# HBioquant/DiffBindFR

Hardware: AMD Instinct MI355X
Metric: poses_per_sec (higher is better)
Workload: dtype f32

## Files before the change

diffbindfr_amd/csrc/api.cpp:

```cpp
#include <cmath>
#include <cstdio>
#include <cstring>
#include <algorithm>
#include <atomic>
#include <map>

#include "common.h"

void launch_conv(const ConvArgs& a, hipStream_t st);
void launch_conv_layer(const ConvArgs* c4, hipStream_t st);
void launch_conv2(const Conv2Args& a, hipStream_t st);
void launch_conv2h(const Conv2Args& a, hipStream_t st);
void launch_convz(const ConvZArgs& a, hipStream_t st);
void launch_reduce_ln(const float* msg, const int* row_start, const int* row_cnt, int N, int D, const LNDesc& ln,
                      const float* old, int D_old, float* out, int ldo, int mode, hipStream_t st, const uint8_t* first = nullptr, unsigned long long sc_lanes = 0);
struct ReduceLayerArgs {
  const float* msg[4]; const int* row_start[4]; const int* row_cnt[4]; LNDesc ln[4];
  int NL, NA, D, D_old;
  const float* old_l; const float* old_a; float* out_l; float* out_a;
  const uint8_t* first[4]; unsigned long long sc_lanes[4];
};
static unsigned long long convz_sc_lanes(const ConvZ& z) {
  unsigned long long m = 0;
  for (int i = 0; i < z.n_io; ++i) m |= 0xfffull << (z.out_off[i] / 4);
  return m;
}
void launch_reduce_ln_layer(const ReduceLayerArgs& a, hipStream_t st);
enum SetKind { SET_LL = 0, SET_AA = 1, SET_AL = 2, SET_LA = 3, SET_TOR = 4, SET_SC = 5, N_SETS = 6 };
struct GraphArgs {
  dbfr_batch b;
  const int* lig_batch; const int* atm_batch; const uint8_t* is_cab; const int* n_cab; const float* tr_sigma;
  float lig_cut2, atom_cut2, cross_cut2;
  int lig_cap, atom_cap, dynamic_cross;
  EdgeSet set[N_SETS];
  int* err;
  int step, lds_nl, lds_na, n_chunk, lanes;
};
void dbfr_edge_form(const dbfr_batch& b, int* n_chunk, int* lanes);
void launch_edges(const GraphArgs& A, bool heads_only, hipStream_t st);
void launch_edge_log(const GraphArgs& A, int* log_row, int stride, hipStream_t st);
void launch_edge_ties(const GraphArgs& A, int* log_row, int stride, float tol, hipStream_t st);
void launch_graph_chunks(const GraphArgs& A, hipStream_t st);
void launch_flat_chunks(const int* tgt, const int* n_edges, int max_edges, int span, int n_span, int* cnt0, int cap, int* chunk_es, int* chunk_gl, hipStream_t st);
void launch_row_absmax(const float* lx, const int* lig_ptr, float* out_l, const float* ax, const int* atm_ptr, float* out_a, int ld, int D, int G, int n_rows_a, hipStream_t st);
void launch_batch_vectors(const dbfr_batch& b, int* lig_batch, int* atm_batch, uint8_t* is_cab, int* n_cab,
                          int* tor_batch, int* sc_batch, hipStream_t st);
void launch_time_embed(const float* t, int G, float emb_scale, float* temb, hipStream_t st);
enum MlpIn { IN_LIGNODE = 0, IN_LIGEDGE = 1, IN_TG = 2, IN_G = 3 };
struct MlpArgs {
  Mlp2 w; int mode; const int* n_rows_dev; int n_rows_max; const float* temb; const int* row_graph_tab; const int* tgt;
  const int* aux; const float* dist; const float* bond_feat; int nfeat; const float* lig_node; int nnode;
  const float* gs_offset; const float* gs_coeff; float* out;
};
void launch_mlp(const MlpArgs& a, hipStream_t st);
struct AtomEncArgs {
  const float* pocket_feat; const int* atm_batch; const float* temb; const float* emb[5]; int dims[5];
  const float* lin_t; int NA; float* out;
};
void launch_atom_encoder(const AtomEncArgs& a, hipStream_t st);
void launch_center_edges(const dbfr_batch& b, int* tgt, int* gth, float* dist, float* sh, int* row_start, int* row_cnt,
                         hipStream_t st);
struct TrRotArgs {
  const float* gp; const float* temb; const float* tr_sigma; const float* rot_norm; Mlp2 tr, rot; int G;
  int scale_by_sigma; float* tr_out; float* rot_out; int* err;
};
void launch_trrot(const TrRotArgs& a, hipStream_t st);
void launch_bond_attr(const float* x, int ldx, const int* b0, const int* b1, const int* bsel, int stride, int n,
                      float* out, hipStream_t st);
void launch_tor_final(const float* feat, const Mlp2& w, const float* norm2, int scale, int n, float* out, hipStream_t st);
struct SdeLigArgs {
  dbfr_batch b; const float* tr_score; const float* rot_score; const float* tor_score; const float* z_tr;
  const float* z_rot; const float* z_tor; float dt, tr_g2, tr_gsdt, rot_g2, rot_gsdt, tor_g2, tor_gsdt; float* traj;
  int* err;
};
void launch_sde_ligand(const SdeLigArgs& a, hipStream_t st);
void launch_sidechain(const dbfr_batch& b, const float* score, const float* z, float dt, float g2, float gsdt,
                      const int* a14_group, float* atom14_out, float* traj14, const int* err, hipStream_t st);
void launch_fill(float* p, float v, int n, hipStream_t st);
void launch_set_int(int* p, int v, hipStream_t st);
void launch_init_poses(const dbfr_batch& b, const dbfr_init_tape& z, const int* a14_group, float* atom14_out, hipStream_t st);
void launch_extract_templates(int n_res, const int* aatype, const float* pos14, float* transl, float* rots, float* frames,
                              float* rigid, float* angle, hipStream_t st);
void launch_select_pocket(int n_prot, int n_res_total, const int* res_ptr, int m, const float* pos, const float* mask, const int* ref_ptr,
                          const float* ref, float cut2, int max_neighbors, float* d2, unsigned char* out, hipStream_t st);
void launch_acc_flops(const int* n_edges, double flops_per_edge, double bytes_per_edge, double fused_bytes_per_edge, double* counter, hipStream_t st);
void launch_acc_executed(const int* n_edges, double flops_per_edge, double* counter, hipStream_t st);
struct AccBatch { const int* n[32]; double coef[32]; double* dst[32]; int count; };
void launch_acc_batch(const AccBatch& b, hipStream_t st);
static inline double fused_bytes(int D_in, int D_out) { return 4.0 * (48 + 9 + 3 + 48 + 48 + D_in + D_out); }

#define RT_TABLE static const
#include "residue_tables.inc"
#undef RT_TABLE

static thread_local std::string g_err;
void dbfr_set_error(const std::string& s) { g_err = s; }
// ... 270 lines not shown
      }
  }
  o->K = K; o->D_in = sp.D_in; o->D_out = sp.D_out; o->n_tiles = n_tiles; o->W = sp.W;
  for (int v = 0; v < 5; ++v) { o->wave_tile0[v] = wave_tile0[v]; o->wave_run0[v] = wave_run0[v]; }
  o->W1p = upload(m, w1p, &rc);
  o->b1 = upload(m, std::vector<float>(B1, B1 + K), &rc);
  o->W2p = upload(m, w2p, &rc);
  o->b2p = upload(m, b2p, &rc);
  o->runs = upload(m, runs, &rc);
  LNDesc& ln = o->ln;
  memset(&ln, 0, sizeof ln);
  ln.nblk = (int)sp.out.size();
  int off = 0;
  for (int i = 0; i < ln.nblk; ++i) {
    ln.mul[i] = sp.out[i].mul; ln.dim[i] = sp.out[i].dim(); ln.off[i] = off;
    ln.is0e[i] = sp.out[i].l == 0 && sp.out[i].p == 1;
    off += ln.mul[i] * ln.dim[i];
  }
  ln.mean_shift = upload(m, std::vector<float>(ms, ms + nirr), &rc);
  ln.weight = upload(m, std::vector<float>(aw, aw + nirr), &rc);
  ln.bias = upload(m, std::vector<float>(ab, ab + std::max(n0e, 0)), &rc);
  return rc;
}

#define CH_TILE_BYTES_HOST 9280
#define F16_ROW_DEPTH_OK 17
static int pack_f16_tiles(const float* frag, const float* bias16, int tile0, int nt, uint16_t* out, int* depth = nullptr, float* rinv = nullptr) {
  constexpr int KT = 9;
  const size_t tile_h = CH_TILE_BYTES_HOST / 2, tail_off = 8192 / 2, bias_off = 9216 / 2;
  auto h16 = [](float v) { const _Float16 h = (_Float16)v; uint16_t u; memcpy(&u, &h, 2); return u; };
  float mx = 0.f;
  for (size_t i = (size_t)tile0 * KT * 256; i < (size_t)(tile0 + nt) * KT * 256; ++i) mx = std::max(mx, fabsf(frag[i]));
  int e = 0;
  if (mx > 0.f) (void)frexpf(mx, &e);
  int k = mx > 0.f ? std::max(-120, std::min(120, 15 - e)) : 0;
  float bmx = 0.f;
  for (int i = 16 * tile0; i < 16 * (tile0 + nt); ++i) bmx = std::max(bmx, fabsf(bias16[i]));
  if (bmx > 0.f) { int eb = 0; (void)frexpf(bmx, &eb); k = std::min(k, 48 - eb); }
  const float sc = ldexpf(1.f, k);
  std::vector<int> rowd((size_t)nt * 16, 0);
  int dmax = 0;
  for (int t = tile0; t < tile0 + nt; ++t)
    for (int row = 0; row < 16; ++row) {
      float rm = 0.f;
      for (int s4 = 0; s4 < KT; ++s4)
        for (int gq = 0; gq < 4; ++gq)
          for (int q = 0; q < 4; ++q) rm = std::max(rm, fabsf(frag[(((size_t)t * KT + s4) * 64 + 16 * gq + row) * 4 + q]));
      if (rm <= 0.f) continue;
      int er = 0;
      (void)frexpf(rm, &er);
      int d = 15 - (er + k);
      if (rinv) {
        int up = std::max(d, 0);
        const float br = fabsf(bias16[16 * t + row]);
        if (br > 0.f) { int eb = 0; (void)frexpf(br, &eb); up = std::max(0, std::min(up, 48 - eb - k)); }
        up = std::min(up, 100);
        rowd[(size_t)(t - tile0) * 16 + row] = up;
        d -= up;
      }
      dmax = std::max(dmax, d);
    }
  if (depth) *depth = dmax;
  if (rinv)
    for (int i = 0; i < nt * 16; ++i) rinv[(size_t)tile0 * 16 + i] = ldexpf(1.f, -rowd[i]);
  for (int t = tile0; t < tile0 + nt; ++t) {
    float b[16];
    for (int i = 0; i < 16; ++i) b[i] = bias16[16 * t + i] * ldexpf(sc, rowd[(size_t)(t - tile0) * 16 + i]);
    memcpy(&out[t * tile_h + bias_off], b, 64);
    for (int s4 = 0; s4 < KT; ++s4)
      for (int lane = 0; lane < 64; ++lane)
        for (int q = 0; q < 4; ++q) {
          const float v = frag[(((size_t)t * KT + s4) * 64 + lane) * 4 + q] * ldexpf(sc, rowd[(size_t)(t - tile0) * 16 + (lane & 15)]);
          const _Float16 hi = (_Float16)v;
          const uint16_t pc[2] = {h16(v), h16(v - (float)hi)};
          for (int i = 0; i < 2; ++i) {
            if (s4 < 8) out[t * tile_h + ((size_t)(i * 4 + (s4 >> 1)) * 64 + lane) * 8 + 4 * (s4 & 1) + q] = pc[i];
            else out[t * tile_h + tail_off + (size_t)lane * 8 + 4 * i + q] = pc[i];
          }
        }
  }
  return k;
}

static int pack_conv2(dbfr_model* m, const TMap& tm, const std::string& name, int kind, const ConvW& base, ConvW2* o, bool vector_only = false) {
  ConvSpec sp = make_conv_spec(kind);
  const int K = sp.K;
  if (K != 144) return fail(DBFR_ERR_ARG, "k_conv2 layout is for the K=144 convs");
  int rc = 0;
  const float* W2 = need(tm, name + ".fc.lin.3.weight", (int64_t)sp.W * K, &rc);
  const float* B2 = need(tm, name + ".fc.lin.3.bias", sp.W, &rc);
  if (rc) return rc;
  const int KT = K / 16;
  struct Pair { int io, w; std::vector<const PathDesc*> paths; };
  std::vector<Pair> pairs;
  for (int io = 0; io < (int)sp.out.size(); ++io)
    for (int w = 0; w < sp.out[io].mul; ++w) {
      if (vector_only && sp.out[io].l == 0) continue;
      Pair pr{io, w, {}};
      for (auto& p : sp.paths) if (p.io == io) pr.paths.push_back(&p);
      std::stable_sort(pr.paths.begin(), pr.paths.end(),
                       [](const PathDesc* a, const PathDesc* b) { return a->type != b->type ? a->type < b->type : a->mul1 > b->mul1; });
      pairs.push_back(pr);
    }
  auto sig = [](const Pair& a) {
    std::string k;
    for (auto* p : a.paths) k += std::to_string(p->type) + ":" + std::to_string(p->mul1) + ":" + std::to_string(p->in_off) + ",";
    return k;
  };
  struct Group { std::vector<int> pair_idx; int tiles; int xph; };
  std::vector<Group> groups;
  {
    std::map<std::string, std::vector<int>> cls;
    std::vector<std::string> order;
    for (int i = 0; i < (int)pairs.size(); ++i) {
      std::string k = sig(pairs[i]);
      if (!cls.count(k)) order.push_back(k);
      cls[k].push_back(i);
    }
    for (auto& k : order) {
      auto& v = cls[k];
      for (size_t i = 0; i < v.size(); i += 4) {
        Group g;
        for (size_t j = i; j < i + 4; ++j) g.pair_idx.push_back(j < v.size() ? v[j] : -1);
        g.tiles = 0;
        bool hi = false, lo = false;
        for (auto* p : pairs[v[i]].paths) {
          if (p->mul1 % 4) return fail(DBFR_ERR_ARG, "input multiplicity not a multiple of 4 in " + name);
          g.tiles += p->mul1 / 4;
          if (p->in_off >= 120) hi = true;
          if (p->in_off < 48) lo = true;
        }
        if (hi && lo) return fail(DBFR_ERR_ARG, "channel group reads both scalar input blocks in " + name);
        g.xph = hi ? 1 : 0;
        groups.push_back(g);
      }
    }
  }
  std::stable_sort(groups.begin(), groups.end(), [](const Group& a, const Group& b) { return a.xph < b.xph; });
  std::vector<int> rows_orig; std::vector<float> rows_scale;
  std::vector<RunDesc> runs;
  std::vector<int> group_run0, group_tiles;
  for (const Group& G : groups) {
    group_run0.push_back((int)runs.size());
    group_tiles.push_back(G.tiles);
    const Pair& lead = pairs[G.pair_idx[0]];
    for (size_t pi = 0; pi < lead.paths.size(); ++pi) {
      const PathDesc* lp = lead.paths[pi];
      RunDesc rd;
      const uint32_t flags = (pi == 0 ? 1u : 0u) | (pi + 1 == lead.paths.size() ? 2u : 0u);
      const uint32_t tile0 = (uint32_t)rows_orig.size() / 16, nt = (uint32_t)lp->mul1 / 4, x_step = 4u * (2 * lp->l1 + 1);
      if (tile0 >= (1u << 20) || nt >= (1u << 12)) return fail(DBFR_ERR_ARG, "conv too large for the run descriptor");
      rd.tile0_n = tile0 | (nt << 20);
      rd.meta = (uint32_t)lp->type | (flags << 4) | ((uint32_t)lp->sh_off << 8) | (x_step << 12) | ((uint32_t)G.xph << 20);
      rd.x_off4 = rd.o_off4 = 0;
      for (int g = 0; g < 4; ++g) {
        const int pidx = G.pair_idx[g];
        const PathDesc* p = pidx >= 0 ? pairs[pidx].paths[pi] : lp;
        if (p->type != lp->type || p->sh_off != lp->sh_off || p->mul1 != lp->mul1 || p->in_off != lp->in_off)
          return fail(DBFR_ERR_ARG, "channel group with non-uniform paths in " + name);
        const int d_o = 2 * p->lo + 1;
        const uint32_t xo = p->in_off >= 120 ? p->in_off - 120 : p->in_off;
        const uint32_t oo = pidx >= 0 ? p->out_off + pairs[pidx].w * d_o : 255u;
        if (xo + 4 * (2 * p->l1 + 1) * (p->mul1 / 4) > 120 || (oo != 255u && (int)oo >= sp.D_out))
          return fail(DBFR_ERR_ARG, "irreps do not fit the k_conv2 row layout in " + name);
        rd.x_off4 |= xo << (8 * g);
        rd.o_off4 |= oo << (8 * g);
      }
      runs.push_back(rd);
      for (int u0 = 0; u0 < lp->mul1; u0 += 4)
        for (int g = 0; g < 4; ++g) {
          const int pidx = G.pair_idx[g];
          const PathDesc* p = pidx >= 0 ? pairs[pidx].paths[pi] : lp;
          for (int r = 0; r < 4; ++r) {
            rows_orig.push_back(pidx >= 0 ? p->w_off + (u0 + r) * p->mulo + pairs[pidx].w : -1);
            rows_scale.push_back(pidx >= 0 ? p->fold : 0.f);
          }
        }
    }
  }
  const int n_tiles = (int)rows_orig.size() / 16;
  std::vector<float> w2q((size_t)n_tiles * KT * 64 * 4), b2q((size_t)n_tiles * 16);
  for (int t = 0; t < n_tiles; ++t) {
    for (int i = 0; i < 16; ++i) { const int ro = rows_orig[16 * t + i]; b2q[16 * t + i] = ro >= 0 ? rows_scale[16 * t + i] * B2[ro] : 0.f; }
    for (int s4 = 0; s4 < KT; ++s4)
      for (int lane = 0; lane < 64; ++lane) {
        const int ro = rows_orig[16 * t + (lane & 15)];
        const float sc = rows_scale[16 * t + (lane & 15)];
        for (int q = 0; q < 4; ++q)
          w2q[(((size_t)t * KT + s4) * 64 + lane) * 4 + q] = ro >= 0 ? sc * W2[(size_t)ro * K + 16 * s4 + 4 * (lane >> 4) + q] : 0.f;
      }
  }
  memset(o, 0, sizeof *o);
  o->D_in = sp.D_in; o->D_out = sp.D_out; o->n_tiles = n_tiles; o->n_runs = (int)runs.size();
  o->W1p = base.W1p; o->b1 = base.b1;
  if (!vector_only) {
  o->W2q = upload(m, w2q, &rc);
  o->b2q = upload(m, b2q, &rc);
  }
  {
    const int rowscale = getenv("DBFR_F16_ROWSCALE") ? atoi(getenv("DBFR_F16_ROWSCALE")) : 1;
    std::vector<uint16_t> w2h((size_t)n_tiles * (CH_TILE_BYTES_HOST / 2) + 512, 0);
    std::vector<float> w2rinv((size_t)std::max(n_tiles, 1) * 16, 1.f);
    int depth_max = 0, depth_run = 0;
    for (int pass = 0; pass < 2; ++pass) {
      const bool rowf = pass == 1;
      if (rowf && !(rowscale == 2 || (rowscale == 1 && depth_max > F16_ROW_DEPTH_OK))) break;
      if (rowf) depth_run = depth_max;
      depth_max = 0;
      for (RunDesc& rd : runs) {
        const int tile0 = rd.tile0_n & 0xfffff, nt = rd.tile0_n >> 20;
        int depth = 0;
        const int k = pack_f16_tiles(w2q.data(), b2q.data(), tile0, nt, w2h.data(), &depth, rowf ? w2rinv.data() : nullptr);
        depth_max = std::max(depth_max, depth);
        rd.meta = (rd.meta & 0x00ffffffu) | ((uint32_t)(k & 0xff) << 24);
      }
      if (!rowf) depth_run = depth_max;
      else o->W2rinv = upload(m, w2rinv, &rc);
    }
    o->W2h = upload(m, w2h, &rc);
    const float* W1 = need(tm, name + ".fc.lin.0.weight", (int64_t)K * K, &rc);
    const float* B1 = need(tm, name + ".fc.lin.0.bias", K, &rc);
    if (rc) return rc;
    std::vector<float> w1q((size_t)KT * KT * 256);
    for (int mt = 0; mt < KT; ++mt)
      for (int s4 = 0; s4 < KT; ++s4)
        for (int lane = 0; lane < 64; ++lane)
          for (int q = 0; q < 4; ++q)
            w1q[(((size_t)mt * KT + s4) * 64 + lane) * 4 + q] = W1[(size_t)(16 * mt + (lane & 15)) * K + 16 * s4 + 4 * (lane >> 4) + q];
    std::vector<uint16_t> w1h((size_t)KT * (CH_TILE_BYTES_HOST / 2) + 512, 0);
    int depth1 = 0;
    o->k1 = pack_f16_tiles(w1q.data(), B1, 0, KT, w1h.data(), &depth1);
    depth_run = std::max(depth_run, depth1);
    if (rowscale == 2 || (rowscale == 1 && depth1 > F16_ROW_DEPTH_OK)) {
      std::vector<float> w1rinv((size_t)KT * 16, 1.f);
      o->k1 = pack_f16_tiles(w1q.data(), B1, 0, KT, w1h.data(), &depth1, w1rinv.data());
      o->W1rinv = upload(m, w1rinv, &rc);
    }
    o->W1h = upload(m, w1h, &rc);
    o->f16_depth = std::max(depth_max, depth1);
    o->f16_depth_run = depth_run;
  }
  o->runs = upload(m, runs, &rc);
  const int n_g = (int)groups.size();
  int total_tiles = 0;
  for (int t : group_tiles) total_tiles += t;
  for (int si = 0; si < 4; ++si) {
    const int S = 1 << si;
    int gi = 0, acc = 0;
    for (int p = 0; p < S; ++p) {
      o->part_run[si][p] = gi < n_g ? group_run0[gi] : (int)runs.size();
      const long target = (long)total_tiles * (p + 1) / S;
      while (gi < n_g && (acc + group_tiles[gi] / 2 < target || p == S - 1)) { acc += group_tiles[gi]; ++gi; }
    }
    for (int p = S; p <= 8; ++p) o->part_run[si][p] = (int)runs.size();
  }
  return rc;
}

static int pack_convz(dbfr_model* m, const TMap& tm, const std::string& name, int kind, const ConvW2& base, ConvZ* o) {
  ConvSpec sp = make_conv_spec(kind);
  const int K = sp.K;
  memset(o, 0, sizeof *o);
  if (K != 144) return fail(DBFR_ERR_ARG, "k_convz is for the K=144 convs");
  int rc = 0;
  const float* W2 = need(tm, name + ".fc.lin.3.weight", (int64_t)sp.W * K, &rc);
  const float* B2 = need(tm, name + ".fc.lin.3.bias", sp.W, &rc);
  if (rc) return rc;
  struct Col { const PathDesc* p; int u; };
  std::vector<std::vector<Col>> cols;
  std::vector<int> ios;
  for (int io = 0; io < (int)sp.out.size(); ++io) {
    if (sp.out[io].l != 0) continue;
    if (sp.out[io].mul != NS) return fail(DBFR_ERR_ARG, "scalar output irrep with a multiplicity other than 48 in " + name);
    std::vector<Col> c;
    for (int pass = 0; pass < 2; ++pass)
      for (auto& p : sp.paths) {
        if (p.io != io || p.l1 != pass) continue;
        if (p.l1 != p.l2 || p.lo != 0 || p.l1 > 1) return fail(DBFR_ERR_ARG, "unsupported scalar-output path in " + name);
        for (int u = 0; u < p.mul1; ++u) c.push_back({&p, u});
      }
    int n_scalar = 0;
    for (auto& q : c) n_scalar += q.p->l1 == 0;
    if (n_scalar % 16) return fail(DBFR_ERR_ARG, "scalar-input columns do not fill whole tiles in " + name);
    while (c.size() % 16) c.push_back({nullptr, 0});
    cols.push_back(c);
    ios.push_back(io);
  }
  if (ios.size() > 2) return fail(DBFR_ERR_ARG, "more than two scalar output irreps in " + name);
  o->n_io = (int)ios.size();
  int nct_total = 0;
  for (int i = 0; i < o->n_io; ++i) {
    o->nct[i] = (int)cols[i].size() / 16;
    for (auto& q : cols[i]) o->nc_valid[i] += q.p != nullptr;
    o->ct0[i] = nct_total;
    nct_total += o->nct[i];
    int off = 0;
    for (int j = 0; j < ios[i]; ++j) off += sp.out[j].mul * sp.out[j].dim();
    o->out_off[i] = off;
  }
  if (nct_total > CZ_MAXCT) return fail(DBFR_ERR_ARG, "too many c tiles in " + name);
  std::vector<uint32_t> cdesc((size_t)std::max(nct_total, 1) * 16, 0u);
  std::vector<float> rowinv((size_t)std::max(o->n_io, 1) * NS, 1.f);
  std::vector<uint16_t> w2z((size_t)nct_total * CZ_NKT * 8 * (CZ_TILE_BYTES / 2) + 512, 0);
  auto h16 = [](float v) { const _Float16 h = (_Float16)v; uint16_t u; memcpy(&u, &h, 2); return u; };
  for (int i = 0; i < o->n_io; ++i) {
    const auto& c = cols[i];
    for (size_t j = 0; j < c.size(); ++j)
      if (c[j].p) cdesc[(size_t)o->ct0[i] * 16 + j] = (uint32_t)(c[j].p->in_off + c[j].u * (2 * c[j].p->l1 + 1)) | ((uint32_t)c[j].p->l1 << 12) |
                                                      ((uint32_t)c[j].p->sh_off << 16) | 0x80000000u;
    auto wval = [&](int cc, int k, int w) -> float {
      if (cc >= (int)c.size() || !c[cc].p || k > K) return 0.f;
      const PathDesc* p = c[cc].p;
      const size_t row = (size_t)p->w_off + (size_t)c[cc].u * p->mulo + w;
      return p->fold * (k < K ? W2[row * K + k] : B2[row]);
    };
    for (int w = 0; w < NS; ++w) {
      float mx = 0.f;
      for (int cc = 0; cc < (int)c.size(); ++cc)
        for (int k = 0; k <= K; ++k) mx = std::max(mx, fabsf(wval(cc, k, w)));
      int s = 0;
      if (mx > 0.f) { int e = 0; (void)frexpf(mx, &e); s = std::max(-100, std::min(100, 15 - e)); }
// ... 85 lines not shown
  if (!m || (log_dev && (n_steps_cap <= 0 || n_graphs_cap <= 0))) return fail(DBFR_ERR_ARG, "dbfr_model_set_edge_log: bad argument");
  m->edge_log = log_dev; m->edge_log_steps = log_dev ? n_steps_cap : 0; m->edge_log_graphs = log_dev ? n_graphs_cap : 0;
  return DBFR_OK;
}

extern "C" int dbfr_model_set_gemm(dbfr_model* m, int32_t mode) {
  if (!m || mode < DBFR_GEMM_F32 || mode > DBFR_GEMM_REDUCE_FIRST || mode == 1 || mode == 2) return fail(DBFR_ERR_ARG, "dbfr_model_set_gemm: bad argument (modes 1 and 2, the three-bf16-piece kernels, were retired with ABI 5 / 4)");
  m->gemm_split = mode;
  return DBFR_OK;
}
extern "C" int dbfr_model_get_gemm(const dbfr_model* m) { return m ? m->gemm_split : DBFR_ERR_ARG; }

extern "C" int dbfr_abi_version(void) { return DBFR_ABI_VERSION; }
#ifndef DBFR_BUILD_ID
#define DBFR_BUILD_ID "unknown"
#endif
extern "C" const char* dbfr_build_id(void) { return DBFR_BUILD_ID; }
extern "C" const char* dbfr_last_error(void) { return g_err.c_str(); }

extern "C" int dbfr_wigner3j(int32_t l1, int32_t l2, int32_t l3, double* out) {
  if (!out || l1 < 0 || l2 < 0 || l3 < 0 || l1 > 4 || l2 > 4 || l3 > 4) return fail(DBFR_ERR_ARG, "bad l");
  std::vector<double> v;
  wigner3j_real(l1, l2, l3, v);
  memcpy(out, v.data(), v.size() * sizeof(double));
  return DBFR_OK;
}

extern "C" int dbfr_conv_paths(int32_t kind, int32_t* t10, int32_t max_paths, int32_t* weight_numel) {
  if (kind < 0 || kind > 5) return fail(DBFR_ERR_ARG, "bad conv kind");
  ConvSpec sp = make_conv_spec(kind);
  if (weight_numel) *weight_numel = sp.W;
  int n = (int)sp.paths.size();
  for (int i = 0; i < n && i < max_paths && t10; ++i) {
    const PathDesc& p = sp.paths[i];
    int32_t* r = t10 + 10 * i;
    r[0] = p.i1; r[1] = p.i2; r[2] = p.io; r[3] = p.l1; r[4] = p.l2; r[5] = p.lo; r[6] = p.mul1; r[7] = p.mulo; r[8] = p.w_off;
    memcpy(&r[9], &p.coeff, 4);
  }
  return n;
}

static int model_create_impl(const dbfr_model_cfg* cfg, const dbfr_tensor* tensors, int32_t n_tensors, dbfr_model** out);
static int f16_depth_ok() { static const int v = getenv("DBFR_F16_DEPTH") ? atoi(getenv("DBFR_F16_DEPTH")) : F16_ROW_DEPTH_OK; return v; }

extern "C" int dbfr_model_create(const dbfr_model_cfg* cfg, const dbfr_tensor* tensors, int32_t n_tensors,
                                 dbfr_model** out) {
  try {
    return model_create_impl(cfg, tensors, n_tensors, out);
  } catch (const std::exception& e) {
    return fail(DBFR_ERR_ARG, std::string("dbfr_model_create: ") + e.what());
  }
}

static int model_create_impl(const dbfr_model_cfg* cfg, const dbfr_tensor* tensors, int32_t n_tensors, dbfr_model** out) {
  if (!cfg || !tensors || !out) return fail(DBFR_ERR_ARG, "null argument");
  if (cfg->ns != NS || cfg->nv != NV || cfg->sh_lmax != 2 || cfg->distance_embed_dim != EMB ||
      cfg->sigma_embed_dim != EMB || cfg->num_conv_layers < 1 || cfg->num_conv_layers > 8)
    return fail(DBFR_ERR_ARG, "unsupported model configuration (need ns=48, nv=12, sh_lmax=2, 32-d embeddings)");
  if (cfg->lig_edge_features + 2 * EMB > 80 || cfg->lig_node_features + EMB > 80)
    return fail(DBFR_ERR_ARG, "ligand feature width too large");
  std::string serr;
  int rc = so3_selftest(serr);
  if (rc) return fail(rc, serr);
  TMap tm;
  for (int i = 0; i < n_tensors; ++i) tm[tensors[i].name] = &tensors[i];
  dbfr_model* m = new dbfr_model();
  m->cfg = *cfg;
  m->profile = 0; m->ev_used = 0; m->flops_dev = nullptr; m->fused_bytes_last = 0; m->executed_last = 0; m->useful_last = 0; m->form_bytes_last = 0; m->conv_ms_acc = 0; m->conv_launches_acc = 0;
  m->streams_ready = false;
  m->edge_log = nullptr; m->edge_log_steps = 0; m->edge_log_graphs = 0; m->layer_fallback = 0;
  m->tie_log = nullptr; m->tie_log_steps = 0; m->tie_log_graphs = 0; m->tie_tol = 0.f;
  m->use_conv2 = getenv("DBFR_CONV2") ? atoi(getenv("DBFR_CONV2")) : -1;
  m->gemm_split = gemm_from_env();
  if (m->gemm_split < 0) rc = fail(DBFR_ERR_ARG, std::string("DBFR_GEMM=") + getenv("DBFR_GEMM") + ": unknown or retired value (f32 | split_f16 | reduce_first)");
  m->conv2_layers = getenv("DBFR_CONV2_LAYERS") ? atoi(getenv("DBFR_CONV2_LAYERS")) : 0;
  m->conv_fuse = getenv("DBFR_CONV_FUSE") ? atoi(getenv("DBFR_CONV_FUSE")) : 1;
  const char* fam[4] = {"lig_conv_layers", "cross_al_conv_layers", "atom_conv_layers", "cross_la_conv_layers"};
  for (int l = 0; l < cfg->num_conv_layers && !rc; ++l)
    for (int f = 0; f < 4 && !rc; ++f)
    {
      rc = pack_conv(m, tm, std::string(fam[f]) + "." + std::to_string(l), std::min(l, 3), &m->layer[l][f]);
      if (!rc) rc = pack_conv2(m, tm, std::string(fam[f]) + "." + std::to_string(l), std::min(l, 3), m->layer[l][f], &m->layer2[l][f]);
      if (!rc && m->layer2[l][f].f16_depth > f16_depth_ok()) { m->layer_fallback |= 1u << l; m->fallback_convs += std::string(fam[f]) + "." + std::to_string(l) + ";"; }
      if (!rc && (m->layer2[l][f].W2rinv || m->layer2[l][f].W1rinv)) m->rowscaled_convs += std::string(fam[f]) + "." + std::to_string(l) + ":" + std::to_string(m->layer2[l][f].f16_depth_run) + ";";
      if (!rc) rc = pack_conv2(m, tm, std::string(fam[f]) + "." + std::to_string(l), std::min(l, 3), m->layer[l][f], &m->layer2v[l][f], true);
      if (!rc) rc = pack_convz(m, tm, std::string(fam[f]) + "." + std::to_string(l), std::min(l, 3), m->layer2[l][f], &m->layerz[l][f]);
    }
  if (!rc) rc = pack_conv(m, tm, "final_conv", 4, &m->final_conv);
  if (!rc) rc = pack_conv(m, tm, "tor_bond_conv", 5, &m->tor_conv);
  if (!rc) rc = pack_conv2(m, tm, "tor_bond_conv", 5, m->tor_conv, &m->tor_conv2);
  if (!rc && m->tor_conv2.f16_depth > f16_depth_ok()) { m->layer_fallback |= 1u << 31; m->fallback_convs += "tor_bond_conv;"; }
  if (!rc && (m->tor_conv2.W2rinv || m->tor_conv2.W1rinv)) m->rowscaled_convs += "tor_bond_conv:" + std::to_string(m->tor_conv2.f16_depth_run) + ";";
  if (!rc) rc = pack_convz(m, tm, "tor_bond_conv", 5, m->tor_conv2, &m->tor_convz);
  if (!rc && !cfg->no_sc_torsion) rc = pack_conv(m, tm, "sc_tor_bond_conv", 5, &m->sc_conv);
  if (!rc && !cfg->no_sc_torsion) rc = pack_conv2(m, tm, "sc_tor_bond_conv", 5, m->sc_conv, &m->sc_conv2);
  if (!rc && !cfg->no_sc_torsion && m->sc_conv2.f16_depth > f16_depth_ok()) { m->layer_fallback |= 1u << 31; m->fallback_convs += "sc_tor_bond_conv;"; }
  if (!rc && !cfg->no_sc_torsion && (m->sc_conv2.W2rinv || m->sc_conv2.W1rinv)) m->rowscaled_convs += "sc_tor_bond_conv:" + std::to_string(m->sc_conv2.f16_depth_run) + ";";
  if (!rc && !cfg->no_sc_torsion) rc = pack_convz(m, tm, "sc_tor_bond_conv", 5, m->sc_conv2, &m->sc_convz);
  if (!rc) rc = pack_mlp(m, tm, "lig_node_embedding", cfg->lig_node_features + EMB, NS, NS, true, &m->lig_node_emb);
  if (!rc) rc = pack_mlp(m, tm, "lig_edge_embedding", cfg->lig_edge_features + 2 * EMB, NS, NS, true, &m->lig_edge_emb);
  if (!rc) rc = pack_mlp(m, tm, "atom_edge_embedding", 2 * EMB, NS, NS, true, &m->atom_edge_emb);
  if (!rc) rc = pack_mlp(m, tm, "la_edge_embedding", 2 * EMB, NS, NS, true, &m->la_edge_emb);
  if (!rc) rc = pack_mlp(m, tm, "center_edge_embedding", 2 * EMB, NS, NS, true, &m->center_edge_emb);
  if (!rc) rc = pack_mlp(m, tm, "tor_edge_embedding", EMB, NS, NS, true, &m->tor_edge_emb);
  if (!rc) rc = pack_mlp(m, tm, "tr_final_layer", 1 + EMB, NS, 1, true, &m->tr_final);
  if (!rc) rc = pack_mlp(m, tm, "rot_final_layer", 1 + EMB, NS, 1, true, &m->rot_final);
  if (!rc) rc = pack_mlp(m, tm, "tor_final_layer", 2 * NS, NS, 1, false, &m->tor_final);
  if (!rc && !cfg->no_sc_torsion) {
    rc = pack_mlp(m, tm, "sc_edge_embedding", EMB, NS, NS, true, &m->sc_edge_emb);
    if (!rc) rc = pack_mlp(m, tm, "sc_tor_final_layer", 2 * NS, NS, 1, false, &m->sc_final);
  }
  const int dims[5] = {37, 22, 4, 21, 2};
  for (int i = 0; i < 5 && !rc; ++i) {
    const float* e = need(tm, "atom_node_embedding.atom_emb_list." + std::to_string(i) + ".weight", (int64_t)dims[i] * NS, &rc);
    if (!rc) { m->atom_emb[i] = upload(m, std::vector<float>(e, e + dims[i] * NS), &rc); m->atom_dims[i] = dims[i]; }
  }
  if (!rc) {
    const float* w = need(tm, "atom_node_embedding.scalar_lin.weight", (int64_t)NS * (NS + EMB), &rc);
    if (!rc) {
      std::vector<float> t((size_t)(NS + EMB) * NS);
      for (int o = 0; o < NS; ++o) for (int i = 0; i < NS + EMB; ++i) t[(size_t)i * NS + o] = w[(size_t)o * (NS + EMB) + i];
      m->atom_lin_t = upload(m, t, &rc);
    }
  }
  struct { const char* n; const float** off; const float** c; } gs[4] = {
      {"lig", &m->gs_lig_off, &m->gs_lig_c}, {"atom", &m->gs_atom_off, &m->gs_atom_c},
      {"cross", &m->gs_cross_off, &m->gs_cross_c}, {"center", &m->gs_center_off, &m->gs_center_c}};
  for (int i = 0; i < 4 && !rc; ++i) {
    const float* off = need(tm, std::string(gs[i].n) + "_distance_expansion.offset", EMB, &rc);
    const float* c = need(tm, std::string(gs[i].n) + "_distance_expansion.coeff", 1, &rc);
    if (!rc) { *gs[i].off = upload(m, std::vector<float>(off, off + EMB), &rc); *gs[i].c = upload(m, std::vector<float>(c, c + 1), &rc); }
  }
  if (!rc) m->a14_group = upload(m, std::vector<int>(kAtom14ToGroup, kAtom14ToGroup + 21 * 14), &rc);
  if (!rc) { m->flops_dev = upload(m, std::vector<double>(6, 0.0), &rc); }
  if (!rc) { m->queue = upload(m, std::vector<int>(4, 0), &rc); }
  if (rc) { dbfr_model_destroy(m); return rc; }
  *out = m;
  return DBFR_OK;
}

extern "C" void dbfr_model_destroy(dbfr_model* m) {
  if (!m) return;
  for (void* p : m->allocs) (void)hipFree(p);
  for (auto e : m->ev) (void)hipEventDestroy(e);
  if (m->streams_ready) {
    for (int i = 0; i < 3; ++i) { (void)hipStreamDestroy(m->side[i]); (void)hipEventDestroy(m->ev_join[i]); }
    (void)hipEventDestroy(m->ev_fork); (void)hipEventDestroy(m->ev_a); (void)hipEventDestroy(m->ev_b);
  }
  delete m;
}

struct WsEntry { std::string name; size_t offset, bytes; };
struct Bump {
  char* base; size_t off; size_t cap;
  std::vector<WsEntry>* log;
  template <typename T> T* take(size_t n, const char* name = nullptr) {
    off = (off + 255) & ~(size_t)255;
    T* p = base ? (T*)(base + off) : nullptr;
    if (log && name) log->push_back({name, off, n * sizeof(T)});
    off += n * sizeof(T);
    return p;
  }
};

struct Ws {
  int* err; int64_t* counters;
  int *lig_batch, *atm_batch, *n_cab, *tor_batch, *sc_batch; uint8_t* is_cab;
  float* temb;
  float *c_t, *c_tr_sigma, *c_rot_norm, *c_tor_n2, *c_sc_n2;
  float *s_tr, *s_rot, *s_tor, *s_sc;
  float *lig_x[2], *atom_x[2];
  EdgeSet set[N_SETS];
  int *c_tgt, *c_gth, *c_row_start, *c_row_cnt, *c_n; float *c_dist, *c_sh, *c_emb;
  float* msg[4]; int multi; int conv2; float* gp; float *tor_attr, *sc_attr, *tor_feat, *sc_feat;
  float *xmax_l, *xmax_a;
  int* n_edges6;
};

static void edge_set_take(Bump& b, EdgeSet& S, int cap, int n_targets, int G, int n_graphs, int* n_edges, const char* nm) {
  S.cap = cap; S.n_edges = n_edges;
  std::string p(nm);
  S.tgt = b.take<int>(cap, (p + ".tgt").c_str()); S.gth = b.take<int>(cap, (p + ".gth").c_str());
  S.aux = b.take<int>(cap, (p + ".aux").c_str());
  S.dist = b.take<float>(cap, (p + ".dist").c_str()); S.sh = b.take<float>((size_t)cap * SH_LD, (p + ".sh").c_str());
  S.emb = b.take<float>((size_t)cap * NS, (p + ".emb").c_str());
  S.row_start = b.take<int>(n_targets, (p + ".row_start").c_str()); S.row_cnt = b.take<int>(n_targets, (p + ".row_cnt").c_str());
  S.g_cnt = b.take<int>(G, (p + ".g_cnt").c_str()); S.g_base = b.take<int>(G, (p + ".g_base").c_str());
  S.chunk0 = b.take<int>(n_graphs + 1, (p + ".chunk0").c_str()); S.gedge0 = b.take<int>(n_graphs + 1, (p + ".gedge0").c_str());
  S.chunk_cap = cap > 0 ? cap / 32 + n_targets / CZ_MAXSEG + n_graphs + 8 : 0;
  S.chunk_es = b.take<int>(std::max(S.chunk_cap, 1), (p + ".chunk_es").c_str()); S.chunk_gl = b.take<int>(std::max(S.chunk_cap, 1), (p + ".chunk_gl").c_str());
  S.seg_first = b.take<uint8_t>(std::max(cap, 1), (p + ".seg_first").c_str());
}

static int plan(const dbfr_model* m, const dbfr_batch* B, const dbfr_limits* lim, char* base, size_t cap, Ws* w,
                size_t* need_bytes, std::vector<WsEntry>* log = nullptr) {
  dbfr_limits L = {24, 64};
  if (lim) { if (lim->aa_avg_neighbors > 0) L.aa_avg_neighbors = lim->aa_avg_neighbors; if (lim->cross_avg_neighbors > 0) L.cross_avg_neighbors = lim->cross_avg_neighbors; }
  Bump b{base, 0, cap, log};
  const int G = B->G, NL = B->NL, NA = B->NA;
  w->err = b.take<int>(16, "err"); w->counters = (int64_t*)b.take<int64_t>(8); w->n_edges6 = b.take<int>(8, "n_edges");
  w->lig_batch = b.take<int>(NL); w->atm_batch = b.take<int>(NA); w->is_cab = b.take<uint8_t>(NA, "is_cab");
  w->n_cab = b.take<int>(G); w->tor_batch = b.take<int>(B->NTOR + 1); w->sc_batch = b.take<int>(B->NSC + 1);
  w->temb = b.take<float>((size_t)G * EMB, "temb");
  w->c_t = b.take<float>(G); w->c_tr_sigma = b.take<float>(G); w->c_rot_norm = b.take<float>(G);
  w->c_tor_n2 = b.take<float>(B->NTOR + 1); w->c_sc_n2 = b.take<float>(B->NSC + 1);
  w->s_tr = b.take<float>(3 * G); w->s_rot = b.take<float>(3 * G); w->s_tor = b.take<float>(B->NTOR + 1); w->s_sc = b.take<float>(B->NSC + 1);
  for (int i = 0; i < 2; ++i) { w->lig_x[i] = b.take<float>((size_t)NL * MAXD, i ? "lig_x1" : "lig_x0"); w->atom_x[i] = b.take<float>((size_t)NA * MAXD, i ? "atom_x1" : "atom_x0"); }
  const int lig_cap = m->cfg.lig_max_neighbors;
  const long cap_ll = (long)NL * std::min(lig_cap + 1, std::max(B->max_nl - 1, 1)) + B->EB;
  const long cap_aa = (long)NA * std::min(L.aa_avg_neighbors, std::max(B->max_na - 1, 1));
  const long cap_x = (long)NL * std::min(B->max_na, 2 * B->max_nr + L.cross_avg_neighbors);
  const long cap_t = (long)B->NTOR * lig_cap, cap_s = m->cfg.no_sc_torsion ? 0 : (long)B->NSC * lig_cap;
  const long caps[N_SETS] = {cap_ll, cap_aa, cap_x, cap_x, cap_t, cap_s};
  const int ntg[N_SETS] = {NL, NA, NL, NA, B->NTOR, B->NSC};
  long maxcap = NL;
  for (int k = 0; k < N_SETS; ++k) {
    if (caps[k] > 0x7fffff00L) return fail(DBFR_ERR_ARG, "batch too large for int32 edge indices; split it");
    static const char* names[N_SETS] = {"ll", "aa", "al", "la", "tor", "sc"};
    edge_set_take(b, w->set[k], (int)caps[k], ntg[k] + 1, G * dbfr_edge_chunks(B->max_na, B->max_nl), G, w->n_edges6 ? w->n_edges6 + k : nullptr, names[k]);
    maxcap = std::max(maxcap, caps[k]);
  }
  w->c_tgt = b.take<int>(NL); w->c_gth = b.take<int>(NL); w->c_dist = b.take<float>(NL); w->c_sh = b.take<float>((size_t)NL * SH_LD, "center.sh");
  w->c_emb = b.take<float>((size_t)NL * NS, "center.emb"); w->c_row_start = b.take<int>(G); w->c_row_cnt = b.take<int>(G);
  w->c_n = w->n_edges6 ? w->n_edges6 + 6 : nullptr;
  static const long multi_edges = getenv("DBFR_MULTI_EDGES") ? atol(getenv("DBFR_MULTI_EDGES")) : 0;
  static const long conv2_edges = getenv("DBFR_CONV2_EDGES") ? atol(getenv("DBFR_CONV2_EDGES")) : 128 * 1024;
  w->multi = maxcap <= multi_edges;
  w->conv2 = m->gemm_split || m->use_conv2 > 0 || (m->use_conv2 < 0 && maxcap <= conv2_edges);
  if (w->conv2 || m->conv2_layers > 0 || (m->conv_fuse && !w->multi)) {
    const bool all_fused = w->conv2 || (m->conv_fuse && !w->multi && m->conv2_layers <= 0);
    const long mc[4] = {all_fused ? std::max({caps[SET_LL], (long)NL, cap_t, cap_s}) : maxcap, std::max(caps[SET_AL], cap_s), caps[SET_AA], caps[SET_LA]};
    for (int i = 0; i < 4; ++i) w->msg[i] = b.take<float>((size_t)std::max(mc[i], 1L) * MAXD, i == 0 ? "msg" : nullptr);
    if (w->conv2) w->multi = 0;
  } else
  for (int i = 0; i < 4; ++i) w->msg[i] = (i == 0 || w->multi) ? b.take<float>((size_t)maxcap * MAXD, i == 0 ? "msg" : nullptr) : nullptr;
  w->gp = b.take<float>((size_t)G * 12, "gp");
  w->xmax_l = b.take<float>(G, "xmax_l"); w->xmax_a = b.take<float>(G, "xmax_a");
  w->tor_attr = b.take<float>((size_t)(B->NTOR + 1) * NS, "tor_attr"); w->sc_attr = b.take<float>((size_t)(B->NSC + 1) * NS);
  w->tor_feat = b.take<float>((size_t)(B->NTOR + 1) * 2 * NS, "tor_feat"); w->sc_feat = b.take<float>((size_t)(B->NSC + 1) * 2 * NS);
  *need_bytes = b.off + 256;
  return DBFR_OK;
}

static int check_batch(const dbfr_model* m, const dbfr_batch* B) {
  if (!m || !B) return fail(DBFR_ERR_ARG, "null argument");
  if (B->G <= 0 || B->NL <= 0 || B->NA <= 0 || B->NR <= 0) return fail(DBFR_ERR_ARG, "empty batch");
  if (B->max_nl > 256) return fail(DBFR_ERR_ARG, "ligand with more than 256 heavy atoms is not supported");
  if (B->max_na > 8192) return fail(DBFR_ERR_ARG, "pocket with more than 8192 heavy atoms is not supported");
  if (B->max_nl <= 0 || B->max_na <= 0 || B->max_nr <= 0) return fail(DBFR_ERR_ARG, "max_nl/max_na/max_nr must be set");
  return DBFR_OK;
}

extern "C" int dbfr_workspace_bytes(const dbfr_model* m, const dbfr_batch* b, const dbfr_limits* lim, size_t* bytes) {
  int rc = check_batch(m, b);
  if (rc) return rc;
  if (!bytes) return fail(DBFR_ERR_ARG, "null argument");
  Ws w; memset(&w, 0, sizeof w);
  return plan(m, b, lim, nullptr, 0, &w, bytes);
}

static void prof_events(dbfr_model* m, hipEvent_t* e0, hipEvent_t* e1) {
  if (m->ev_used + 2 > m->ev.size()) {
    size_t old = m->ev.size();
    m->ev.resize(old + 512);
    for (size_t i = old; i < m->ev.size(); ++i) (void)hipEventCreate(&m->ev[i]);
  }
  *e0 = m->ev[m->ev_used++]; *e1 = m->ev[m->ev_used++];
}

static void conv_call(dbfr_model* m, const ConvW& cw, const int* n_edges, int max_edges, const int* tgt, const int* gth,
                      const float* emb, const float* sh, const float* tab1, int ld1, const int* idx1, const float* tab2,
                      int ld2, const int* idx2, const float* x, int ldx, float* msg, hipStream_t st) {
  ConvArgs a;
  a.n_edges = n_edges; a.max_edges = max_edges; a.tgt = tgt; a.gth = gth; a.emb = emb; a.sh = sh; a.sh_sign = 1.f;
  a.tab1 = tab1; a.ld1 = ld1; a.idx1 = idx1; a.tab2 = tab2; a.ld2 = ld2; a.idx2 = idx2; a.x = x; a.ldx = ldx;
  a.w = cw; a.msg = msg;
  hipEvent_t e0 = nullptr, e1 = nullptr;
  const bool prof = m->profile == 1 && cw.K == 144;
  const bool count = m->profile && cw.K == 144;
  if (prof) {
    prof_events(m, &e0, &e1);
    (void)hipEventRecord(e0, st);
  }
  launch_conv(a, st);
  if (prof) (void)hipEventRecord(e1, st);
  if (count) {
    launch_acc_flops(n_edges, 2.0 * cw.K * ((double)cw.K + cw.W), 4.0 * (cw.W + cw.D_in + 9) + 16.0, fused_bytes(cw.D_in, cw.D_out), m->flops_dev, st);
  }
}

static Conv2Desc conv2_desc(const ConvW2& cw, const int* n_edges, int max_edges, const int* gth, const float* emb, const float* sh,
                            const float* tab1, int ld1, const int* idx1, const float* tab2, int ld2, const int* idx2, const float* x,
                            int ldx, float* msg) {
  Conv2Desc d;
  d.n_edges = n_edges; d.max_edges = max_edges; d.gth = gth; d.emb = emb; d.sh = sh; d.tab1 = tab1; d.ld1 = ld1; d.idx1 = idx1;
  d.tab2 = tab2; d.ld2 = ld2; d.idx2 = idx2; d.x = x; d.ldx = ldx; d.w = cw; d.msg = msg;
  return d;
}

static ConvZDesc convz_desc(const Conv2Desc& d, const ConvZ& z, const int* tgt, int D_out, const int* chunk_es, const int* chunk_gl, const int* n_chunks, int max_chunks,
                            const float* xmax = nullptr) {
  ConvZDesc o;
  o.n_edges = d.n_edges; o.max_edges = d.max_edges; o.tgt = tgt; o.gth = d.gth; o.emb = d.emb; o.sh = d.sh;
  o.tab1 = d.tab1; o.ld1 = d.ld1; o.idx1 = d.idx1; o.tab2 = d.tab2; o.ld2 = d.ld2; o.idx2 = d.idx2; o.x = d.x; o.ldx = d.ldx;
  o.w = z; o.msg = d.msg; o.D_out = D_out; o.chunk_es = chunk_es; o.chunk_gl = chunk_gl; o.n_chunks = n_chunks; o.max_chunks = max_chunks; o.xmax = xmax;
  return o;
}

static void conv2_call(dbfr_model* m, const Conv2Desc* descs, const int* Ws, int n, hipStream_t st, bool f16_fallback = false, const ConvZDesc* z = nullptr) {
  Conv2Args a;
  memset(&a, 0, sizeof a);
  for (int i = 0; i < n; ++i) a.c[i] = descs[i];
  a.n_conv = n; a.queue = m->queue;
  hipEvent_t e0 = nullptr, e1 = nullptr;
  if (m->profile == 1) {
    prof_events(m, &e0, &e1);
    (void)hipEventRecord(e0, st);
  }
  static unsigned long long* trace_dev = nullptr;
  static const char* trace_file = getenv("DBFR_CONV2_TRACE");
  if (trace_file && !trace_dev) {
    if (hipMalloc(&trace_dev, 8 * C2_TRACE_CAP * sizeof(unsigned long long)) != hipSuccess) trace_dev = nullptr;
    else atexit([] {
      std::vector<unsigned long long> h(8 * C2_TRACE_CAP);
      if (hipDeviceSynchronize() == hipSuccess && hipMemcpy(h.data(), trace_dev, h.size() * 8, hipMemcpyDeviceToHost) == hipSuccess) {
        if (FILE* f = fopen(getenv("DBFR_CONV2_TRACE"), "wb")) { fwrite(h.data(), 8, h.size(), f); fclose(f); }
      }
    });
  }
  if (trace_dev) { (void)hipMemsetAsync(trace_dev, 0, 8 * C2_TRACE_CAP * sizeof(unsigned long long), st); a.trace = trace_dev; }
  if (z) {
    Conv2Args v = a;
    v.n_conv = 0;
    for (int i = 0; i < n; ++i)
      if (descs[i].w.n_tiles > 0) v.c[v.n_conv++] = descs[i];
    if (v.n_conv) launch_conv2h(v, st);
    ConvZArgs za;
    memset(&za, 0, sizeof za);
    for (int i = 0; i < n; ++i) za.c[i] = z[i];
    za.n_conv = n;
    za.dbg = nullptr;
    za.executed = m->profile ? m->flops_dev + 3 : nullptr;
    launch_convz(za, st);
  }
  else if (m->gemm_split >= DBFR_GEMM_SPLIT_F16 && !f16_fallback) launch_conv2h(a, st);
  else launch_conv2(a, st);
  if (m->profile == 1) (void)hipEventRecord(e1, st);
  if (m->profile) {
    AccBatch ab; ab.count = 0;
    auto acc = [&](const int* ne, double coef, double* dst) { if (ab.count < 32) { ab.n[ab.count] = ne; ab.coef[ab.count] = coef; ab.dst[ab.count] = dst; ++ab.count; } };
    for (int i = 0; i < n; ++i) {
      acc(descs[i].n_edges, 2.0 * 144 * (144.0 + Ws[i]), m->flops_dev);
      acc(descs[i].n_edges, 4.0 * (Ws[i] + descs[i].w.D_in + 9) + 16.0, m->flops_dev + 1);
      acc(descs[i].n_edges, fused_bytes(descs[i].w.D_in, descs[i].w.D_out), m->flops_dev + 2);
      const double rows = 16.0 * descs[i].w.n_tiles;
      const bool f16 = (m->gemm_split >= DBFR_GEMM_SPLIT_F16 && !f16_fallback) || z;
      const double ex = f16 ? 3.0 * 2.0 * 144 * (144.0 + rows) : 2.0 * 144 * (144.0 + rows);
      if (!z || descs[i].w.n_tiles > 0) acc(descs[i].n_edges, ex, m->flops_dev + 3);
      if (!z) acc(descs[i].n_edges, ex, m->flops_dev + 4);
      else if (descs[i].w.n_tiles > 0) acc(descs[i].n_edges, 3.0 * 2.0 * 144 * rows, m->flops_dev + 4);
      const int D_in = descs[i].w.D_in, D_out = descs[i].w.D_out;
      const double in_bytes = 4.0 * (48 + 9 + 3 + 48 + 48 + D_in);
      if (!z) acc(descs[i].n_edges, fused_bytes(D_in, D_out), m->flops_dev + 5);
      else acc(descs[i].n_edges, in_bytes + 1.0 + (descs[i].w.n_tiles > 0 ? in_bytes + 4.0 * (D_out - 48 * z[i].w.n_io) : 0.0), m->flops_dev + 5);
    }
    launch_acc_batch(ab, st);
  }
}

static int run_score(dbfr_model* m, const dbfr_batch* B, const dbfr_cond* c, const dbfr_scores* out, Ws& w,
                     hipStream_t st, int step = 0) {
  const dbfr_model_cfg& cfg = m->cfg;
  const int G = B->G, NL = B->NL, NA = B->NA;
  launch_time_embed(c->t, G, cfg.emb_scale, w.temb, st);
  GraphArgs ga;
  ga.b = *B; ga.lig_batch = w.lig_batch; ga.atm_batch = w.atm_batch; ga.is_cab = w.is_cab; ga.n_cab = w.n_cab;
  ga.tr_sigma = c->tr_sigma;
  ga.lig_cut2 = cfg.lig_cutoff * cfg.lig_cutoff; ga.atom_cut2 = cfg.atom_cutoff * cfg.atom_cutoff;
  ga.cross_cut2 = cfg.dynamic_max_cross ? 1.0f : cfg.cross_cutoff * cfg.cross_cutoff;
  ga.lig_cap = cfg.lig_max_neighbors; ga.atom_cap = cfg.atom_max_neighbors; ga.dynamic_cross = cfg.dynamic_max_cross;
  for (int k = 0; k < N_SETS; ++k) ga.set[k] = w.set[k];
  ga.err = w.err; ga.step = step; ga.lds_nl = ga.lds_na = 0;
  dbfr_edge_form(*B, &ga.n_chunk, &ga.lanes);
  launch_edges(ga, false, st);
  if (int lrc = take_launch_error()) return lrc;
  if (m->gemm_split == DBFR_GEMM_REDUCE_FIRST) launch_graph_chunks(ga, st);
  if (m->edge_log && step < m->edge_log_steps) launch_edge_log(ga, m->edge_log + (size_t)step * N_SETS * m->edge_log_graphs, m->edge_log_graphs, st);
  if (m->tie_log && step < m->tie_log_steps) launch_edge_ties(ga, m->tie_log + (size_t)step * N_SETS * m->tie_log_graphs, m->tie_log_graphs, m->tie_tol, st);
  {
    MlpArgs a; memset(&a, 0, sizeof a);
    a.w = m->lig_node_emb; a.mode = IN_LIGNODE; a.n_rows_max = NL; a.temb = w.temb; a.row_graph_tab = w.lig_batch;
    a.lig_node = B->lig_node; a.nnode = cfg.lig_node_features; a.out = w.lig_x[0];
    launch_mlp(a, st);
  }
  {
    AtomEncArgs a; a.pocket_feat = B->pocket_feat; a.atm_batch = w.atm_batch; a.temb = w.temb;
    for (int i = 0; i < 5; ++i) { a.emb[i] = m->atom_emb[i]; a.dims[i] = m->atom_dims[i]; }
    a.lin_t = m->atom_lin_t; a.NA = NA; a.out = w.atom_x[0];
    launch_atom_encoder(a, st);
  }
  auto edge_mlp = [&](const Mlp2& mw, int mode, const EdgeSet& S, const int* tab, const float* off, const float* co) {
    MlpArgs a; memset(&a, 0, sizeof a);
    a.w = mw; a.mode = mode; a.n_rows_dev = S.n_edges; a.n_rows_max = S.cap; a.temb = w.temb; a.row_graph_tab = tab;
    a.tgt = S.tgt; a.aux = S.aux; a.dist = S.dist; a.bond_feat = B->bond_feat; a.nfeat = cfg.lig_edge_features;
    a.gs_offset = off; a.gs_coeff = co; a.out = S.emb;
    launch_mlp(a, st);
  };
  edge_mlp(m->lig_edge_emb, IN_LIGEDGE, w.set[SET_LL], w.lig_batch, m->gs_lig_off, m->gs_lig_c);
  edge_mlp(m->atom_edge_emb, IN_TG, w.set[SET_AA], w.atm_batch, m->gs_atom_off, m->gs_atom_c);
  edge_mlp(m->la_edge_emb, IN_TG, w.set[SET_AL], w.lig_batch, m->gs_cross_off, m->gs_cross_c);
  edge_mlp(m->la_edge_emb, IN_TG, w.set[SET_LA], w.atm_batch, m->gs_cross_off, m->gs_cross_c);
  static const int dims[4] = {48, 84, 120, 168};
  int cur = 0;
  for (int l = 0; l < cfg.num_conv_layers; ++l) {
    const int Di = dims[std::min(l, 3)], Do = dims[std::min(l + 1, 3)];
    const float *lx = w.lig_x[cur], *ax = w.atom_x[cur];
    float *lnew = w.lig_x[cur ^ 1], *anew = w.atom_x[cur ^ 1];
    const EdgeSet &LL = w.set[SET_LL], &AA = w.set[SET_AA], &AL = w.set[SET_AL], &LA = w.set[SET_LA];
    if (w.conv2 || l < m->conv2_layers) {
      const bool rf = m->gemm_split == DBFR_GEMM_REDUCE_FIRST && !((m->layer_fallback >> l) & 1u);
      const ConvW2* L2 = rf ? m->layer2v[l] : m->layer2[l];
      const Conv2Desc ds[4] = {
          conv2_desc(L2[0], LL.n_edges, LL.cap, LL.gth, LL.emb, LL.sh, lx, Di, LL.tgt, lx, Di, LL.gth, lx, Di, w.msg[0]),
          conv2_desc(L2[1], AL.n_edges, AL.cap, AL.gth, AL.emb, AL.sh, lx, Di, AL.tgt, ax, Di, AL.gth, ax, Di, w.msg[1]),
          conv2_desc(L2[2], AA.n_edges, AA.cap, AA.gth, AA.emb, AA.sh, ax, Di, AA.tgt, ax, Di, AA.gth, ax, Di, w.msg[2]),
          conv2_desc(L2[3], LA.n_edges, LA.cap, LA.gth, LA.emb, LA.sh, ax, Di, LA.tgt, lx, Di, LA.gth, lx, Di, w.msg[3])};
      const int Ws[4] = {m->layer[l][0].W, m->layer[l][1].W, m->layer[l][2].W, m->layer[l][3].W};
      if (rf) {
        launch_row_absmax(lx, B->lig_ptr, w.xmax_l, ax, B->atm_ptr, w.xmax_a, Di, Di, G, NA, st);
      }
      auto zd = [&](int i, const EdgeSet& S, const float* xmax) { return convz_desc(ds[i], m->layerz[l][i], S.tgt, Do, S.chunk_es, S.chunk_gl, S.chunk0 + G, S.chunk_cap, xmax); };
      const ConvZDesc zs[4] = {zd(0, LL, w.xmax_l), zd(1, AL, w.xmax_a), zd(2, AA, w.xmax_a), zd(3, LA, w.xmax_l)};
      conv2_call(m, ds, Ws, 4, st, (m->layer_fallback >> l) & 1u, rf ? zs : nullptr);
      ReduceLayerArgs ra;
      const EdgeSet* es[4] = {&LL, &AL, &AA, &LA};
      for (int i = 0; i < 4; ++i) {
        ra.msg[i] = w.msg[i]; ra.row_start[i] = es[i]->row_start; ra.row_cnt[i] = es[i]->row_cnt; ra.ln[i] = m->layer[l][i].ln;
        ra.first[i] = rf ? es[i]->seg_first : nullptr; ra.sc_lanes[i] = rf ? convz_sc_lanes(m->layerz[l][i]) : 0;
      }
      ra.NL = NL; ra.NA = NA; ra.D = Do; ra.D_old = Di; ra.old_l = lx; ra.old_a = ax; ra.out_l = lnew; ra.out_a = anew;
      launch_reduce_ln_layer(ra, st);
    } else if (m->conv_fuse && !w.multi) {
      auto mk = [&](const ConvW& cw, const EdgeSet& S, const float* tab1, const int* idx1, const float* tab2, const int* idx2, const float* x, float* msg) {
        ConvArgs a;
        a.n_edges = S.n_edges; a.max_edges = S.cap; a.tgt = S.tgt; a.gth = S.gth; a.emb = S.emb; a.sh = S.sh; a.sh_sign = 1.f;
        a.tab1 = tab1; a.ld1 = Di; a.idx1 = idx1; a.tab2 = tab2; a.ld2 = Di; a.idx2 = idx2; a.x = x; a.ldx = Di; a.w = cw; a.msg = msg; a.trace = nullptr;
        return a;
      };
      const ConvArgs c4[4] = {mk(m->layer[l][0], LL, lx, LL.tgt, lx, LL.gth, lx, w.msg[0]), mk(m->layer[l][1], AL, lx, AL.tgt, ax, AL.gth, ax, w.msg[1]),
                              mk(m->layer[l][2], AA, ax, AA.tgt, ax, AA.gth, ax, w.msg[2]), mk(m->layer[l][3], LA, ax, LA.tgt, lx, LA.gth, lx, w.msg[3])};
      hipEvent_t e0 = nullptr, e1 = nullptr;
      if (m->profile == 1) {
        prof_events(m, &e0, &e1);
        (void)hipEventRecord(e0, st);
      }
      launch_conv_layer(c4, st);
      if (m->profile == 1) (void)hipEventRecord(e1, st);
      if (m->profile)
        for (int i = 0; i < 4; ++i)
          launch_acc_flops(c4[i].n_edges, 2.0 * 144 * (144.0 + m->layer[l][i].W), 4.0 * (m->layer[l][i].W + Di + 9) + 16.0, fused_bytes(Di, Do), m->flops_dev, st);
      ReduceLayerArgs ra;
      const EdgeSet* es[4] = {&LL, &AL, &AA, &LA};
      for (int i = 0; i < 4; ++i) { ra.msg[i] = w.msg[i]; ra.row_start[i] = es[i]->row_start; ra.row_cnt[i] = es[i]->row_cnt; ra.ln[i] = m->layer[l][i].ln; ra.first[i] = nullptr; ra.sc_lanes[i] = 0; }
      ra.NL = NL; ra.NA = NA; ra.D = Do; ra.D_old = Di; ra.old_l = lx; ra.old_a = ax; ra.out_l = lnew; ra.out_a = anew;
      launch_reduce_ln_layer(ra, st);
    } else if (!w.multi || m->profile == 1) {
      conv_call(m, m->layer[l][0], LL.n_edges, LL.cap, LL.tgt, LL.gth, LL.emb, LL.sh, lx, Di, LL.tgt, lx, Di, LL.gth, lx, Di, w.msg[0], st);
      launch_reduce_ln(w.msg[0], LL.row_start, LL.row_cnt, NL, Do, m->layer[l][0].ln, lx, Di, lnew, Do, 0, st);
      conv_call(m, m->layer[l][1], AL.n_edges, AL.cap, AL.tgt, AL.gth, AL.emb, AL.sh, lx, Di, AL.tgt, ax, Di, AL.gth, ax, Di, w.msg[0], st);
      launch_reduce_ln(w.msg[0], AL.row_start, AL.row_cnt, NL, Do, m->layer[l][1].ln, nullptr, 0, lnew, Do, 1, st);
      conv_call(m, m->layer[l][2], AA.n_edges, AA.cap, AA.tgt, AA.gth, AA.emb, AA.sh, ax, Di, AA.tgt, ax, Di, AA.gth, ax, Di, w.msg[0], st);
      launch_reduce_ln(w.msg[0], AA.row_start, AA.row_cnt, NA, Do, m->layer[l][2].ln, ax, Di, anew, Do, 0, st);
      conv_call(m, m->layer[l][3], LA.n_edges, LA.cap, LA.tgt, LA.gth, LA.emb, LA.sh, ax, Di, LA.tgt, lx, Di, LA.gth, lx, Di, w.msg[0], st);
      launch_reduce_ln(w.msg[0], LA.row_start, LA.row_cnt, NA, Do, m->layer[l][3].ln, nullptr, 0, anew, Do, 1, st);
    } else {
      hipStream_t s0 = m->side[0], s1 = m->side[1], s2 = m->side[2];
      HIPCHECK(hipEventRecord(m->ev_fork, st));
      for (int i = 0; i < 3; ++i) HIPCHECK(hipStreamWaitEvent(m->side[i], m->ev_fork, 0));
      conv_call(m, m->layer[l][0], LL.n_edges, LL.cap, LL.tgt, LL.gth, LL.emb, LL.sh, lx, Di, LL.tgt, lx, Di, LL.gth, lx, Di, w.msg[0], st);
      conv_call(m, m->layer[l][1], AL.n_edges, AL.cap, AL.tgt, AL.gth, AL.emb, AL.sh, lx, Di, AL.tgt, ax, Di, AL.gth, ax, Di, w.msg[1], s0);
      conv_call(m, m->layer[l][2], AA.n_edges, AA.cap, AA.tgt, AA.gth, AA.emb, AA.sh, ax, Di, AA.tgt, ax, Di, AA.gth, ax, Di, w.msg[2], s1);
      conv_call(m, m->layer[l][3], LA.n_edges, LA.cap, LA.tgt, LA.gth, LA.emb, LA.sh, ax, Di, LA.tgt, lx, Di, LA.gth, lx, Di, w.msg[3], s2);
      launch_reduce_ln(w.msg[0], LL.row_start, LL.row_cnt, NL, Do, m->layer[l][0].ln, lx, Di, lnew, Do, 0, st);
      HIPCHECK(hipEventRecord(m->ev_a, st));
      HIPCHECK(hipStreamWaitEvent(s0, m->ev_a, 0));
      launch_reduce_ln(w.msg[1], AL.row_start, AL.row_cnt, NL, Do, m->layer[l][1].ln, nullptr, 0, lnew, Do, 1, s0);
      launch_reduce_ln(w.msg[2], AA.row_start, AA.row_cnt, NA, Do, m->layer[l][2].ln, ax, Di, anew, Do, 0, s1);
      HIPCHECK(hipEventRecord(m->ev_b, s1));
      HIPCHECK(hipStreamWaitEvent(s2, m->ev_b, 0));
      launch_reduce_ln(w.msg[3], LA.row_start, LA.row_cnt, NA, Do, m->layer[l][3].ln, nullptr, 0, anew, Do, 1, s2);
      HIPCHECK(hipEventRecord(m->ev_join[0], s0));
      HIPCHECK(hipEventRecord(m->ev_join[2], s2));
      HIPCHECK(hipStreamWaitEvent(st, m->ev_join[0], 0));
      HIPCHECK(hipStreamWaitEvent(st, m->ev_join[2], 0));
    }
    cur ^= 1;
  }
  const int D = dims[std::min(cfg.num_conv_layers, 3)];
  if (D != MAXD) return fail(DBFR_ERR_ARG, "heads need num_conv_layers >= 3");
  const float *lx = w.lig_x[cur], *ax = w.atom_x[cur];
  const bool fork_heads = w.multi && m->profile != 1 && !w.conv2;
  hipStream_t s_tor = fork_heads ? m->side[0] : st, s_sc = fork_heads ? m->side[1] : st;
  float* msg_tor = fork_heads ? w.msg[1] : w.msg[0];
  float* msg_sc = fork_heads ? w.msg[2] : w.msg[0];
  if (fork_heads) {
    HIPCHECK(hipEventRecord(m->ev_fork, st));
    HIPCHECK(hipStreamWaitEvent(s_tor, m->ev_fork, 0));
    HIPCHECK(hipStreamWaitEvent(s_sc, m->ev_fork, 0));
  }
  launch_center_edges(*B, w.c_tgt, w.c_gth, w.c_dist, w.c_sh, w.c_row_start, w.c_row_cnt, st);
  {
    MlpArgs a; memset(&a, 0, sizeof a);
    a.w = m->center_edge_emb; a.mode = IN_TG; a.n_rows_max = NL; a.temb = w.temb; a.row_graph_tab = w.lig_batch;
    a.dist = w.c_dist; a.gs_offset = m->gs_center_off; a.gs_coeff = m->gs_center_c; a.out = w.c_emb;
    launch_mlp(a, st);
  }
  conv_call(m, m->final_conv, w.n_edges6 + 7, NL, w.c_tgt, w.c_gth, w.c_emb, w.c_sh, lx, D, w.c_gth, nullptr, 0, w.c_gth, lx, D, w.msg[0], st);
  launch_reduce_ln(w.msg[0], w.c_row_start, w.c_row_cnt, G, 12, m->final_conv.ln, nullptr, 0, w.gp, 12, 2, st);
  {
    TrRotArgs a; a.gp = w.gp; a.temb = w.temb; a.tr_sigma = c->tr_sigma; a.rot_norm = c->rot_score_norm;
    a.tr = m->tr_final; a.rot = m->rot_final; a.G = G; a.scale_by_sigma = cfg.scale_by_sigma; a.tr_out = out->tr;
    a.rot_out = out->rot; a.err = w.err;
    launch_trrot(a, st);
  }
  if (w.conv2) {
    const EdgeSet& T = w.set[SET_TOR];
    const EdgeSet& S = w.set[SET_SC];
    const bool do_t = B->NTOR > 0, do_s = !cfg.no_sc_torsion && B->NSC > 0;
    const bool rf = m->gemm_split == DBFR_GEMM_REDUCE_FIRST && !((m->layer_fallback >> 31) & 1u);
    Conv2Desc ds[2]; ConvZDesc zs[2]; int Ws[2]; int nd = 0;
    if (rf) {
      launch_row_absmax(lx, B->lig_ptr, w.xmax_l, ax, B->atm_ptr, w.xmax_a, D, D, G, NA, st);
    }
    if (do_t) {
      launch_bond_attr(lx, D, B->bond_src, B->bond_dst, B->tor_bond, 0, B->NTOR, w.tor_attr, st);
      MlpArgs a; memset(&a, 0, sizeof a);
      a.w = m->tor_edge_emb; a.mode = IN_G; a.n_rows_dev = T.n_edges; a.n_rows_max = T.cap; a.dist = T.dist;
      a.gs_offset = m->gs_lig_off; a.gs_coeff = m->gs_lig_c; a.out = T.emb;
      launch_mlp(a, st);
      ds[nd] = conv2_desc(m->tor_conv2, T.n_edges, T.cap, T.gth, T.emb, T.sh, lx, D, T.gth, w.tor_attr, NS, T.tgt, lx, D, w.msg[0]);
      if (rf) { ds[nd].w.n_tiles = 0; zs[nd] = convz_desc(ds[nd], m->tor_convz, T.tgt, 2 * NS, T.chunk_es, T.chunk_gl, T.chunk0 + G, T.chunk_cap, w.xmax_l); }
      Ws[nd++] = m->tor_conv.W;
    }
    if (do_s) {
      launch_bond_attr(ax, D, B->sc_bond, nullptr, nullptr, 2, B->NSC, w.sc_attr, st);
      MlpArgs a; memset(&a, 0, sizeof a);
      a.w = m->sc_edge_emb; a.mode = IN_G; a.n_rows_dev = S.n_edges; a.n_rows_max = S.cap; a.dist = S.dist;
      a.gs_offset = m->gs_atom_off; a.gs_coeff = m->gs_atom_c; a.out = S.emb;
      launch_mlp(a, st);
      ds[nd] = conv2_desc(m->sc_conv2, S.n_edges, S.cap, S.gth, S.emb, S.sh, ax, D, S.gth, w.sc_attr, NS, S.tgt, ax, D, w.msg[1]);
      if (rf) { ds[nd].w.n_tiles = 0; zs[nd] = convz_desc(ds[nd], m->sc_convz, S.tgt, 2 * NS, S.chunk_es, S.chunk_gl, S.chunk0 + G, S.chunk_cap, w.xmax_a); }
      Ws[nd++] = m->sc_conv.W;
    }
    if (nd) conv2_call(m, ds, Ws, nd, st, (m->layer_fallback >> 31) & 1u, rf ? zs : nullptr);
    if (do_t) {
      launch_reduce_ln(w.msg[0], T.row_start, T.row_cnt, B->NTOR, 2 * NS, m->tor_conv.ln, nullptr, 0, w.tor_feat, 2 * NS, 2, st, rf ? T.seg_first : nullptr, rf ? convz_sc_lanes(m->tor_convz) : 0);
      launch_tor_final(w.tor_feat, m->tor_final, c->tor_score_norm2, cfg.scale_by_sigma, B->NTOR, out->tor, st);
    }
    if (do_s) {
      launch_reduce_ln(w.msg[1], S.row_start, S.row_cnt, B->NSC, 2 * NS, m->sc_conv.ln, nullptr, 0, w.sc_feat, 2 * NS, 2, st, rf ? S.seg_first : nullptr, rf ? convz_sc_lanes(m->sc_convz) : 0);
      launch_tor_final(w.sc_feat, m->sc_final, c->sc_tor_score_norm2, cfg.scale_by_sigma, B->NSC, out->sc_tor, st);
    }
    return DBFR_OK;
  }
  if (B->NTOR > 0) {
    const EdgeSet& T = w.set[SET_TOR];
    launch_bond_attr(lx, D, B->bond_src, B->bond_dst, B->tor_bond, 0, B->NTOR, w.tor_attr, s_tor);
    {
      MlpArgs a; memset(&a, 0, sizeof a);
      a.w = m->tor_edge_emb; a.mode = IN_G; a.n_rows_dev = T.n_edges; a.n_rows_max = T.cap; a.dist = T.dist;
      a.gs_offset = m->gs_lig_off; a.gs_coeff = m->gs_lig_c; a.out = T.emb;
      launch_mlp(a, s_tor);
    }
    conv_call(m, m->tor_conv, T.n_edges, T.cap, T.tgt, T.gth, T.emb, T.sh, lx, D, T.gth, w.tor_attr, NS, T.tgt, lx, D, msg_tor, s_tor);
    launch_reduce_ln(msg_tor, T.row_start, T.row_cnt, B->NTOR, 2 * NS, m->tor_conv.ln, nullptr, 0, w.tor_feat, 2 * NS, 2, s_tor);
    launch_tor_final(w.tor_feat, m->tor_final, c->tor_score_norm2, cfg.scale_by_sigma, B->NTOR, out->tor, s_tor);
  }
  if (!cfg.no_sc_torsion && B->NSC > 0) {
    const EdgeSet& S = w.set[SET_SC];
    launch_bond_attr(ax, D, B->sc_bond, nullptr, nullptr, 2, B->NSC, w.sc_attr, s_sc);
    {
      MlpArgs a; memset(&a, 0, sizeof a);
      a.w = m->sc_edge_emb; a.mode = IN_G; a.n_rows_dev = S.n_edges; a.n_rows_max = S.cap; a.dist = S.dist;
      a.gs_offset = m->gs_atom_off; a.gs_coeff = m->gs_atom_c; a.out = S.emb;
      launch_mlp(a, s_sc);
    }
    conv_call(m, m->sc_conv, S.n_edges, S.cap, S.tgt, S.gth, S.emb, S.sh, ax, D, S.gth, w.sc_attr, NS, S.tgt, ax, D, msg_sc, s_sc);
    launch_reduce_ln(msg_sc, S.row_start, S.row_cnt, B->NSC, 2 * NS, m->sc_conv.ln, nullptr, 0, w.sc_feat, 2 * NS, 2, s_sc);
    launch_tor_final(w.sc_feat, m->sc_final, c->sc_tor_score_norm2, cfg.scale_by_sigma, B->NSC, out->sc_tor, s_sc);
  }
  if (fork_heads) {
    HIPCHECK(hipEventRecord(m->ev_join[0], s_tor));
    HIPCHECK(hipEventRecord(m->ev_join[1], s_sc));
    HIPCHECK(hipStreamWaitEvent(st, m->ev_join[0], 0));
    HIPCHECK(hipStreamWaitEvent(st, m->ev_join[1], 0));
  }
  return DBFR_OK;
}

static int begin(dbfr_model* m, const dbfr_batch* B, void* workspace, size_t wbytes, const dbfr_limits* lim, Ws* w,
                 hipStream_t st) {
  g_launch_err = false;
  int rc = check_batch(m, B);
  if (rc) return rc;
  rc = check_logs(m, B->G);
  if (rc) return rc;
  if (!workspace) return fail(DBFR_ERR_ARG, "null workspace");
  size_t needb = 0;
  memset(w, 0, sizeof *w);
  rc = plan(m, B, lim, (char*)workspace, wbytes, w, &needb);
  if (rc) return rc;
  if (needb > wbytes) return fail(DBFR_ERR_ARG, "workspace too small: need " + std::to_string(needb) + " bytes");
  if (w->multi && !m->streams_ready) {
    for (int i = 0; i < 3; ++i) {
      HIPCHECK(hipStreamCreateWithFlags(&m->side[i], hipStreamNonBlocking));
      HIPCHECK(hipEventCreateWithFlags(&m->ev_join[i], hipEventDisableTiming));
    }
    HIPCHECK(hipEventCreateWithFlags(&m->ev_fork, hipEventDisableTiming));
    HIPCHECK(hipEventCreateWithFlags(&m->ev_a, hipEventDisableTiming));
    HIPCHECK(hipEventCreateWithFlags(&m->ev_b, hipEventDisableTiming));
    m->streams_ready = true;
  }
  HIPCHECK(hipMemsetAsync(workspace, 0, 1024, st));
  if (w->conv2 || m->gemm_split || m->conv2_layers > 0) HIPCHECK(hipMemsetAsync(m->queue, 0, 16, st));
  launch_set_int(w->n_edges6 + 7, B->NL, st);
  launch_batch_vectors(*B, w->lig_batch, w->atm_batch, w->is_cab, w->n_cab, w->tor_batch, w->sc_batch, st);
  return DBFR_OK;
}

extern "C" int dbfr_score(dbfr_model* m, const dbfr_batch* b, const dbfr_cond* cond, const dbfr_scores* out,
                          void* workspace, size_t workspace_bytes, const dbfr_limits* lim, void* hip_stream) {
  if (!cond || !out) return fail(DBFR_ERR_ARG, "null argument");
  hipStream_t st = (hipStream_t)hip_stream;
// ... 138 lines not shown
    float ms = 0;
    if (hipEventElapsedTime(&ms, m->ev[i], m->ev[i + 1]) == hipSuccess) { m->conv_ms_acc += ms; m->conv_launches_acc++; }
  }
  m->ev_used = 0;
  double fl[6] = {0, 0, 0, 0, 0, 0};
  HIPCHECK(hipMemcpy(fl, m->flops_dev, sizeof fl, hipMemcpyDeviceToHost));
  m->fused_bytes_last = fl[2];
  m->executed_last = fl[3];
  m->useful_last = fl[4];
  m->form_bytes_last = fl[5];
  if (conv_ms) *conv_ms = m->conv_ms_acc;
  if (conv_launches) *conv_launches = m->conv_launches_acc;
  if (conv_flops) *conv_flops = fl[0];
  if (ref_form_bytes) *ref_form_bytes = fl[1];
  if (reset) { m->conv_ms_acc = 0; m->conv_launches_acc = 0; HIPCHECK(hipMemset(m->flops_dev, 0, 6 * sizeof(double))); }
  return DBFR_OK;
}

extern "C" int dbfr_profile_executed_flops(const dbfr_model* m, double* executed_flops) {
  if (!m || !executed_flops) return fail(DBFR_ERR_ARG, "null argument");
  *executed_flops = m->executed_last;
  return DBFR_OK;
}

extern "C" int dbfr_profile_useful_flops(const dbfr_model* m, double* useful_flops, double* form_bytes) {
  if (!m || (!useful_flops && !form_bytes)) return fail(DBFR_ERR_ARG, "null argument");
  if (useful_flops) *useful_flops = m->useful_last;
  if (form_bytes) *form_bytes = m->form_bytes_last;
  return DBFR_OK;
}

extern "C" int dbfr_profile_fused_bytes(const dbfr_model* m, double* fused_form_bytes) {
  if (!m || !fused_form_bytes) return fail(DBFR_ERR_ARG, "null argument");
  *fused_form_bytes = m->fused_bytes_last;
  return DBFR_OK;
}

extern "C" int dbfr_workspace_layout(const dbfr_model* m, const dbfr_batch* b, const dbfr_limits* lim, char* names,
                                     size_t names_cap, size_t* offsets, size_t* bytes, int32_t max_entries) {
  int rc = check_batch(m, b);
  if (rc) return rc;
  std::vector<WsEntry> log;
  Ws w; memset(&w, 0, sizeof w);
  size_t nb = 0;
  rc = plan(m, b, lim, nullptr, 0, &w, &nb, &log);
  if (rc) return rc;
  size_t pos = 0;
  int n = 0;
  for (auto& e : log) {
    if (n >= max_entries || pos + e.name.size() + 2 > names_cap) break;
    memcpy(names + pos, e.name.c_str(), e.name.size());
    pos += e.name.size();
    names[pos++] = ';';
    offsets[n] = e.offset; bytes[n] = e.bytes;
    ++n;
  }
  names[pos] = 0;
  return n;
}

static const ConvW* pick_conv(const dbfr_model* m, int layer, int family) {
  if (layer >= 0 && layer < m->cfg.num_conv_layers && family >= 0 && family < 4) return &m->layer[layer][family];
  if (layer == -1) return &m->final_conv;
  if (layer == -2) return &m->tor_conv;
  if (layer == -3 && !m->cfg.no_sc_torsion) return &m->sc_conv;
  return nullptr;
}

static int test_conv_impl(dbfr_model* m, bool conv2, int32_t layer, int32_t family, int32_t n_edges, const int32_t* n_edges_dev,
                          const int32_t* tgt, const int32_t* gth, const float* emb, const float* sh, const float* tab1, int32_t ld1,
                          const int32_t* idx1, const float* tab2, int32_t ld2, const int32_t* idx2, const float* x, int32_t ldx,
                          float* msg, void* hip_stream) {
  if (!m) return fail(DBFR_ERR_ARG, "null model");
  g_launch_err = false;
  const ConvW* cw = pick_conv(m, layer, family);
  if (!cw) return fail(DBFR_ERR_ARG, "no such conv");
  if (conv2) {
    if (cw->K != 144) return fail(DBFR_ERR_ARG, "k_conv2 serves the K=144 convs");
    const ConvW2* cw2 = layer >= 0 ? &m->layer2[layer][family] : layer == -2 ? &m->tor_conv2 : &m->sc_conv2;
    const bool deep = cw2->f16_depth > f16_depth_ok();
    const bool rf = m->gemm_split == DBFR_GEMM_REDUCE_FIRST && !deep;
    Conv2Desc d = conv2_desc(rf && layer >= 0 ? m->layer2v[layer][family] : *cw2, n_edges_dev, n_edges, gth, emb, sh, tab1, ld1, idx1, tab2, ld2, idx2, x, ldx, msg);
    if (rf && layer < 0) d.w.n_tiles = 0;
    static int* scratch_dev[16] = {nullptr}; static size_t scratch_dev_ints[16] = {0};
    int dev_id = 0;
    HIPCHECK(hipGetDevice(&dev_id));
    if (dev_id < 0 || dev_id >= 16) return fail(DBFR_ERR_ARG, "test hook: device index beyond 15");
    int*& scratch = scratch_dev[dev_id]; size_t& scratch_ints = scratch_dev_ints[dev_id];
    const int span = 2048, n_span = std::max((n_edges + span - 1) / span, 1), ccap = n_edges / 32 + n_edges / CZ_MAXSEG + n_span + 8;
    if (rf) {
      const size_t need = (size_t)n_span + 1 + 2 * (size_t)ccap;
      if (need > scratch_ints) {
        if (scratch) HIPCHECK(hipFree(scratch));
        scratch = nullptr; scratch_ints = 0;
        HIPCHECK(hipMalloc(&scratch, need * sizeof(int)));
        scratch_ints = need;
      }
      launch_flat_chunks(tgt, n_edges_dev, n_edges, span, n_span, scratch, ccap, scratch + n_span + 1, scratch + n_span + 1 + ccap, (hipStream_t)hip_stream);
    }
    const ConvZDesc z = convz_desc(d, layer >= 0 ? m->layerz[layer][family] : layer == -2 ? m->tor_convz : m->sc_convz, tgt, cw->D_out,
                                   scratch ? scratch + n_span + 1 : nullptr, scratch ? scratch + n_span + 1 + ccap : nullptr, scratch ? scratch + n_span : nullptr, ccap);
    const int W = cw->W;
    if (rf) HIPCHECK(hipMemsetAsync(msg, 0, (size_t)n_edges * cw->D_out * sizeof(float), (hipStream_t)hip_stream));
    conv2_call(m, &d, &W, 1, (hipStream_t)hip_stream, deep, rf ? &z : nullptr);
  } else {
    conv_call(m, *cw, n_edges_dev, n_edges, tgt, gth, emb, sh, tab1, ld1, idx1, tab2, ld2, idx2, x, ldx, msg, (hipStream_t)hip_stream);
  }
  HIPCHECK(hipGetLastError());
  return take_launch_error();
}

extern "C" int dbfr_test_sde_step(const dbfr_model* m, const dbfr_batch* b, const dbfr_step* step, const dbfr_scores* scores,
                                  const dbfr_noise* z, float* atom14_out, int32_t* err_word_out, void* hip_stream) {
  int rc = check_batch(m, b);
  if (rc) return rc;
  if (!step || !scores || !z || !err_word_out) return fail(DBFR_ERR_ARG, "dbfr_test_sde_step: null argument");
  if (!scores->tr || !scores->rot || !z->z_tr || !z->z_rot || (b->NTOR > 0 && (!scores->tor || !z->z_tor)) ||
      (!m->cfg.no_sc_torsion && b->NSC > 0 && (!scores->sc_tor || !z->z_sc)))
    return fail(DBFR_ERR_ARG, "dbfr_test_sde_step: null score or noise array");
  hipStream_t st = (hipStream_t)hip_stream;
  HIPCHECK(hipMemsetAsync(err_word_out, 0, sizeof(int32_t), st));
  pose_update(m, b, *step, *scores, z->z_tr, z->z_rot, z->z_tor, z->z_sc, nullptr, atom14_out, nullptr, err_word_out, st);
  HIPCHECK(hipGetLastError());
  return DBFR_OK;
}

extern "C" int dbfr_test_chunk_table(const int32_t* tgt, const int32_t* n_edges_dev, int32_t max_edges, int32_t span, int32_t* scratch, int32_t cap,
                                     int32_t* chunk_es, int32_t* chunk_gl, void* hip_stream) {
  if (!tgt || !n_edges_dev || !scratch || !chunk_es || !chunk_gl || span <= 0 || max_edges < 0 || cap <= 0) return fail(DBFR_ERR_ARG, "dbfr_test_chunk_table: bad argument");
  g_launch_err = false;
  const int n_span = std::max((max_edges + span - 1) / span, 1);
  launch_flat_chunks(tgt, n_edges_dev, max_edges, span, n_span, scratch, cap, chunk_es, chunk_gl, (hipStream_t)hip_stream);
  HIPCHECK(hipGetLastError());
  return take_launch_error();
}

extern "C" int dbfr_test_conv(dbfr_model* m, int32_t layer, int32_t family, int32_t n_edges, const int32_t* n_edges_dev,
                              const int32_t* tgt, const int32_t* gth, const float* emb, const float* sh,
                              const float* tab1, int32_t ld1, const int32_t* idx1, const float* tab2, int32_t ld2,
                              const int32_t* idx2, const float* x, int32_t ldx, float* msg, void* hip_stream) {
  return test_conv_impl(m, false, layer, family, n_edges, n_edges_dev, tgt, gth, emb, sh, tab1, ld1, idx1, tab2, ld2, idx2, x, ldx,
                        msg, hip_stream);
}

extern "C" int dbfr_test_conv2(dbfr_model* m, int32_t layer, int32_t family, int32_t n_edges, const int32_t* n_edges_dev,
                               const int32_t* tgt, const int32_t* gth, const float* emb, const float* sh,
                               const float* tab1, int32_t ld1, const int32_t* idx1, const float* tab2, int32_t ld2,
                               const int32_t* idx2, const float* x, int32_t ldx, float* msg, void* hip_stream) {
  return test_conv_impl(m, true, layer, family, n_edges, n_edges_dev, tgt, gth, emb, sh, tab1, ld1, idx1, tab2, ld2, idx2, x, ldx,
                        msg, hip_stream);
}

extern "C" int dbfr_test_reduce_ln2(dbfr_model* m, int32_t layer, int32_t family, const float* msg, const int32_t* row_start, const int32_t* row_cnt,
                                    int32_t n_nodes, const float* old, int32_t d_old, float* out, int32_t mode, const uint8_t* seg_first, void* hip_stream) {
  if (!m) return fail(DBFR_ERR_ARG, "null model");
  const ConvW* cw = pick_conv(m, layer, family);
  if (!cw) return fail(DBFR_ERR_ARG, "no such conv");
  unsigned long long lanes = 0;
  if (seg_first) {
    if (layer == -1 || cw->K != 144) return fail(DBFR_ERR_ARG, "dbfr_test_reduce_ln2: seg_first with a conv that has no reduce-first form");
    lanes = convz_sc_lanes(layer >= 0 ? m->layerz[layer][family] : layer == -2 ? m->tor_convz : m->sc_convz);
  }
  launch_reduce_ln(msg, row_start, row_cnt, n_nodes, cw->D_out, cw->ln, old, d_old, out, cw->D_out, mode, (hipStream_t)hip_stream, seg_first, lanes);
  HIPCHECK(hipGetLastError());
  return DBFR_OK;
}
// ... 13 lines not shown
```

diffbindfr_amd/csrc/common.h:

```cpp
#pragma once
#include <hip/hip_runtime.h>
#include <stdint.h>
#include <string.h>
#include <string>
#include <vector>

#include "../../include/dbfr.h"

#define NS 48
#define NV 12
#define SH_LD 9
#define EMB 32
#define MAXD 168
#define EDGE_CHUNK 64
int dbfr_edge_chunks(int max_na, int max_nl);

enum PathType { PT_SS = 0, PT_SV = 1, PT_VS = 2, PT_VVS = 3, PT_VVV = 4, PT_VTV = 5 };

struct Irr { int mul, l, p; int dim() const { return 2 * l + 1; } };

struct PathDesc {
  int i1, i2, io, l1, l2, lo, mul1, mulo, w_off;
  float coeff;
  int type;
  int in_off, sh_off, out_off;
  float fold;
};

struct ConvSpec {
  std::vector<Irr> in, sh, out;
  std::vector<PathDesc> paths;
  int K;
  int W;
  int D_in, D_out;
};

ConvSpec make_conv_spec(int kind);
void wigner3j_real(int l1, int l2, int l3, std::vector<double>& out);
int so3_selftest(std::string& err);

struct LNDesc {
  int nblk;
  int mul[4], dim[4], off[4], is0e[4];
  const float* mean_shift;
  const float* weight;
  const float* bias;
};

struct RunDesc {
  uint32_t tile0_n;
  uint32_t meta;
  uint32_t x_off4;
  uint32_t o_off4;
};

struct ConvW {
  int K, D_in, D_out, n_tiles, W;
  int wave_tile0[5];
  const float* W1p;
  const float* b1;
  const float* W2p;
  const float* b2p;
  const RunDesc* runs;
  int wave_run0[5];
  LNDesc ln;
};

struct ConvW2 {
  int D_in, D_out, n_tiles, n_runs;
  const float* W1p;
  const float* b1;
  const float* W2q;
  const float* b2q;
  const void* W1h;
  int k1;
  int f16_depth;
  int f16_depth_run;
  const float* W2rinv;
  const float* W1rinv;
  const void* W2h;
  const RunDesc* runs;
  int part_run[4][9];
};

struct Conv2Desc {
  const int* n_edges; int max_edges;
  const int* gth;
  const float* emb;
  const float* sh;
  const float* tab1; int ld1; const int* idx1;
  const float* tab2; int ld2; const int* idx2;
  const float* x; int ldx;
  ConvW2 w;
  float* msg;
};

struct Conv2Args {
  Conv2Desc c[4];
  int n_conv;
  int* queue;
  int run_barrier, no_split;
  int skew;
  unsigned long long* trace;
};
#define C2_TRACE_CAP 4096

#define CZ_NKT 10
#define CZ_MAXCT 12
#define CZ_MAXSEG 4
#define CZ_TILE_BYTES 6144
struct ConvZ {
  int n_io;
  int nct[2];
  int ct0[2];
  int out_off[2];
  int nc_valid[2];
  const uint32_t* cdesc;
  const void* W2z;
  const float* rowinv;
  const void* W1h; int k1;
  const float* W1rinv;
};
struct ConvZDesc {
  const int* n_edges; int max_edges;
  const int* tgt;
  const int* gth;
  const float* emb; const float* sh;
  const float* tab1; int ld1; const int* idx1;
  const float* tab2; int ld2; const int* idx2;
  const float* x; int ldx;
  ConvZ w;
  float* msg; int D_out;
  const int* chunk_es;
  const int* chunk_gl;
  const int* n_chunks;
  int max_chunks;
  const float* xmax;
};
struct ConvZArgs { ConvZDesc c[4]; int n_conv; float* dbg; double* executed; int dbg_sel; };

static inline uint16_t dbfr_bf16_rne(float x) {
  uint32_t u;
  memcpy(&u, &x, 4);
  u += 0x7fffu + ((u >> 16) & 1u);
  return (uint16_t)(u >> 16);
}
static inline float dbfr_bf16_to_f32(uint16_t b) {
  const uint32_t u = (uint32_t)b << 16;
  float f;
  memcpy(&f, &u, 4);
  return f;
}

struct Mlp2 {
  int in, hid, out;
  const float* w0t;
  const float* b0;
  const float* w1t;
  const float* b1;
};

struct EdgeSet {
  int cap;
  int* n_edges;
  int* tgt;
  int* gth;
  int* aux;
  float* dist;
  float* sh;
  float* emb;
  int* row_start;
  int* row_cnt;
  int* g_cnt;
  int* g_base;
  int* chunk0;
  int* gedge0;
  int* chunk_es;
  int* chunk_gl;
// ... 33 lines not shown
```

diffbindfr_amd/csrc/conv2h.hip:

```cpp
#include <cstdio>
#include <cstdlib>
#include <type_traits>

#include "common.h"

typedef float f32x4 __attribute__((ext_vector_type(4)));
typedef float f32x2 __attribute__((ext_vector_type(2)));
typedef _Float16 f16x8 __attribute__((ext_vector_type(8)));
typedef _Float16 f16x4 __attribute__((ext_vector_type(4)));
typedef _Float16 f16x2 __attribute__((ext_vector_type(2)));
typedef unsigned u32x4 __attribute__((ext_vector_type(4)));
typedef unsigned u32x2 __attribute__((ext_vector_type(2)));

#define CH_TILE_BYTES 9280
#define CH_TAIL_OFF 8192
#define CH_BIAS_OFF 9216
#define CH_RING_BYTES 10240

__device__ __forceinline__ void split2x2(float x0, float x1, unsigned& hi, unsigned& lo) {
  const f16x2 h = __builtin_convertvector((f32x2){x0, x1}, f16x2);
  const f16x2 l = __builtin_convertvector((f32x2){x0 - (float)h[0], x1 - (float)h[1]}, f16x2);
  hi = __builtin_bit_cast(unsigned, h);
  lo = __builtin_bit_cast(unsigned, l);
}

__device__ __forceinline__ void scale4(f32x4& o, const f32x4& v, float s) { o[0] = v[0] * s; o[1] = v[1] * s; o[2] = v[2] * s; o[3] = v[3] * s; }
__device__ __forceinline__ void sum4(f32x4& o, const f32x4& a, const f32x4& b) { o[0] = a[0] + b[0]; o[1] = a[1] + b[1]; o[2] = a[2] + b[2]; o[3] = a[3] + b[3]; }

#define C2_XLD 124
#define C2_WAVE_FLOATS (32 * C2_XLD + 32 * 10 + 32 * 8 + 32)

template <int NW, int ABL = 0>
__global__ __launch_bounds__(64 * NW, 2) void k_conv2h(Conv2Args a) {
  constexpr int K = 144, KT = 9;
  constexpr bool ROWF = (ABL & 1024) != 0;
  constexpr int EPB = 32 * NW;
  extern __shared__ __attribute__((aligned(16))) float lds[];
  const int tid = threadIdx.x, lane = tid & 63, wave = tid >> 6;
  const int n = lane & 15, g = lane >> 4;
  if (wave >= NW / 2) __builtin_amdgcn_s_setprio(1);
  const char* ring = reinterpret_cast<const char*>(lds);
  float* xs = lds + CH_RING_BYTES / 4 + wave * C2_WAVE_FLOATS;
  float* shs = xs + 32 * C2_XLD;
  float* ms = shs + 32 * 10;
  int* s_gth = reinterpret_cast<int*>(ms + 32 * 8);

  if (a.trace && blockIdx.x == 0 && tid == 0) { a.trace[0] = __builtin_readcyclecounter(); a.trace[1] = __builtin_amdgcn_s_memrealtime(); }
  int nb0 = 0, nb1 = 0, nb2 = 0, nb3 = 0;
  {
    auto blocks = [&](int c) { return c < a.n_conv ? (min(*a.c[c].n_edges, a.c[c].max_edges) + EPB - 1) / EPB : 0; };
    nb0 = blocks(0); nb1 = blocks(1); nb2 = blocks(2); nb3 = blocks(3);
  }
  const int N = nb0 + nb1 + nb2 + nb3;
  const int n_wg = gridDim.x;
  const int full = (N / n_wg) * n_wg, rem = N - full;
  int si = 0;
  if (rem > 0 && !a.no_split) {
    int best = 0x7fffffff;
#pragma unroll
    for (int c = 0; c < 4; ++c) {
      const int cost = (((rem << c) + n_wg - 1) / n_wg) * ((128 >> c) + 6);
      if (cost < best) { best = cost; si = c; }
    }
  }
  const int total = full + (rem << si);

  for (int it = 0;; ++it) {
    asm volatile("s_waitcnt vmcnt(0) lgkmcnt(0)" ::: "memory");
    __syncthreads();
    const int u = (int)blockIdx.x + it * n_wg;
    if (u >= total) break;
    int blk, part = 0, psi = 0;
    if (u < full) blk = u;
    else { const int v = u - full; blk = full + (v >> si); part = v & ((1 << si) - 1); psi = si; }
    int c = 0;
    if (blk >= nb0) { blk -= nb0; c = 1; if (blk >= nb1) { blk -= nb1; c = 2; if (blk >= nb2) { blk -= nb2; c = 3; } } }
    const Conv2Desc& d = a.c[c];
    const int E = min(*d.n_edges, d.max_edges);
    const int e0 = blk * EPB + 32 * wave;
    const int D_in = d.w.D_in, D_out = d.w.D_out;
    const int vW = lane * 16, vB = g * 16;
    const int wv = __builtin_amdgcn_readfirstlane(wave);
    const int r_begin = d.w.part_run[psi][part], r_end = d.w.part_run[psi][part + 1];
    int t_last = 0, t_first = 0;
    if (r_begin < r_end) {
      const RunDesc rl = d.w.runs[r_end - 1];
      t_last = (rl.tile0_n & 0xfffff) + (rl.tile0_n >> 20) - 1;
      t_first = d.w.runs[r_begin].tile0_n & 0xfffff;
    }
    const __amdgpu_buffer_rsrc_t rW = __builtin_amdgcn_make_buffer_rsrc((void*)d.w.W2h, 0, d.w.n_tiles * CH_TILE_BYTES, 0x00020000);
    const int shA = wv & 7, shB = wv % 6;
    const int offA = shA < 6 ? ((shA / 3) * 4 + shA % 3) * 1024 : CH_BIAS_OFF;
    const int offB = shB < 4 ? ((shB >> 1) * 4 + 3) * 1024 + (shB & 1) * 512 : CH_TAIL_OFF + (shB - 4) * 512;
    const int vA = (shA < 6 || lane < 4) ? lane * 16 : 0x40000000;
    char* ringw = const_cast<char*>(ring);
    u32x4 stgA = {0u, 0u, 0u, 0u};
    u32x2 stgB = {0u, 0u};
    auto fetchA = [&](int tile) { if (!(ABL & (4 | 16))) stgA = __builtin_bit_cast(u32x4, __builtin_amdgcn_raw_buffer_load_b128(rW, vA, ((ABL & 512) ? (tile & 7) : tile) * CH_TILE_BYTES + offA, 0)); };
    auto fetchB = [&](int tile) { if (!(ABL & (4 | 16))) stgB = __builtin_bit_cast(u32x2, __builtin_amdgcn_raw_buffer_load_b64(rW, lane * 8, ((ABL & 512) ? (tile & 7) : tile) * CH_TILE_BYTES + offB, 0)); };
    auto putA = [&] { if (!(ABL & (4 | 8))) *reinterpret_cast<u32x4*>(ringw + offA + vW) = stgA; };
    auto putB = [&] { if (!(ABL & (4 | 8))) *reinterpret_cast<u32x2*>(ringw + offB + lane * 8) = stgB; };
    using I0 = std::integral_constant<int, 0>; using I1 = std::integral_constant<int, 1>;
    using I2 = std::integral_constant<int, 2>; using I3 = std::integral_constant<int, 3>;
    if (r_begin < r_end) {
      fetchA(t_first); fetchB(t_first);
    }

    int ev[2], gthv[2];
    const float* r0[2]; const float* r1[2]; const float* r2[2];
#pragma unroll
    for (int b = 0; b < 2; ++b) {
      const int e = e0 + 16 * b + n;
      ev[b] = min(e, E - 1);
      gthv[b] = d.gth[ev[b]];
      r0[b] = d.emb + (size_t)ev[b] * NS;
      r1[b] = d.tab1 + (size_t)d.idx1[ev[b]] * d.ld1;
      r2[b] = d.tab2 + (size_t)d.idx2[ev[b]] * d.ld2;
    }
    if (g == 0) { s_gth[n] = gthv[0]; s_gth[16 + n] = gthv[1]; }
    if (lane < 32) {
      const int e = min(e0 + lane, E - 1);
      const float* sp = d.sh + (size_t)e * SH_LD;
      float s[9];
#pragma unroll
      for (int k = 0; k < 9; ++k) { s[k] = sp[k]; shs[lane * 10 + k] = s[k]; }
      const float r3 = 1.7320508075688772f;
      float* m = ms + lane * 8;
      m[0] = -s[6] - r3 * s[8]; m[1] = r3 * s[5]; m[2] = r3 * s[4]; m[3] = 2.f * s[6]; m[4] = r3 * s[7]; m[5] = -s[6] + r3 * s[8];
    }
    u32x4 Bh[2][2][4];
    u32x4 Btc[2];
    float se[2], ue[2];
    {
      const __amdgpu_buffer_rsrc_t rW1 = __builtin_amdgcn_make_buffer_rsrc((void*)d.w.W1h, 0, KT * CH_TILE_BYTES, 0x00020000);
      u32x4 Ah[2][2][4];
      u32x4 Atc[2];
      float sa[2];
      int ja[2];
#pragma unroll
      for (int b = 0; b < 2; ++b) {
        f32x4 Ba[KT];
        float amx = 0.f;
#pragma unroll
        for (int s4 = 0; s4 < KT; ++s4) {
          const float* src = s4 < 3 ? r0[b] : s4 < 6 ? r1[b] : r2[b];
          Ba[s4] = *reinterpret_cast<const f32x4*>(src + 16 * (s4 % 3) + 4 * g);
#pragma unroll
          for (int q = 0; q < 4; ++q) amx = fmaxf(amx, fabsf(Ba[s4][q]));
        }
        amx = fmaxf(amx, __shfl_xor(amx, 16));
        amx = fmaxf(amx, __shfl_xor(amx, 32));
        ja[b] = max(-14, __builtin_amdgcn_frexp_expf(amx));
        sa[b] = __builtin_amdgcn_ldexpf(1.f, 15 - ja[b]);
#pragma unroll
        for (int s4 = 0; s4 < KT; ++s4) {
          unsigned hi0, lo0, hi1, lo1;
          split2x2(Ba[s4][0] * sa[b], Ba[s4][1] * sa[b], hi0, lo0);
          split2x2(Ba[s4][2] * sa[b], Ba[s4][3] * sa[b], hi1, lo1);
          if (s4 < 8) {
            Ah[b][0][s4 >> 1][2 * (s4 & 1)] = hi0; Ah[b][0][s4 >> 1][2 * (s4 & 1) + 1] = hi1;
            Ah[b][1][s4 >> 1][2 * (s4 & 1)] = lo0; Ah[b][1][s4 >> 1][2 * (s4 & 1) + 1] = lo1;
          } else {
            Atc[b] = (u32x4){lo0, lo1, hi0, hi1};
          }
        }
      }
      constexpr int NST = KT * 4;
      u32x4 F[3][2];
      u32x4 Ft;
      f32x4 bb;
      auto ld_step = [&](int i, u32x4 (&f)[2]) {
#pragma unroll
        for (int p = 0; p < 2; ++p) f[p] = __builtin_bit_cast(u32x4, __builtin_amdgcn_raw_buffer_load_b128(rW1, vW, (i >> 2) * CH_TILE_BYTES + (p * 4 + (i & 3)) * 1024, 0));
      };
      auto ld_tail = [&](int m) {
        Ft = __builtin_bit_cast(u32x4, __builtin_amdgcn_raw_buffer_load_b128(rW1, vW, m * CH_TILE_BYTES + CH_TAIL_OFF, 0));
        bb = __builtin_bit_cast(f32x4, __builtin_amdgcn_raw_buffer_load_b128(rW1, vB, m * CH_TILE_BYTES + CH_BIAS_OFF, 0));
      };
      ld_step(0, F[0]); ld_step(1, F[1]); ld_tail(0);
      float H[2][KT][4];
      float mx[2] = {0.f, 0.f};
      const f32x4 zero = {0.f, 0.f, 0.f, 0.f};
#define AHB(b, p, s) __builtin_bit_cast(f16x8, Ah[b][p][s])
#define FW(i, p) __builtin_bit_cast(f16x8, F[(i) % 3][p])
#pragma unroll
      for (int m = 0; m < KT; ++m) {
        f32x4 aS[2], aB[2];
        scale4(aS[0], bb, sa[0]); scale4(aS[1], bb, sa[1]);
        aB[0] = zero; aB[1] = zero;
#pragma unroll
        for (int s = 0; s < 4; ++s) {
          const int i = m * 4 + s;
          aS[0] = __builtin_amdgcn_mfma_f32_16x16x32_f16(FW(i, 0), AHB(0, 1, s), aS[0], 0, 0, 0);
          aS[1] = __builtin_amdgcn_mfma_f32_16x16x32_f16(FW(i, 0), AHB(1, 1, s), aS[1], 0, 0, 0);
          aS[0] = __builtin_amdgcn_mfma_f32_16x16x32_f16(FW(i, 1), AHB(0, 0, s), aS[0], 0, 0, 0);
          aS[1] = __builtin_amdgcn_mfma_f32_16x16x32_f16(FW(i, 1), AHB(1, 0, s), aS[1], 0, 0, 0);
          aB[0] = __builtin_amdgcn_mfma_f32_16x16x32_f16(FW(i, 0), AHB(0, 0, s), aB[0], 0, 0, 0);
          aB[1] = __builtin_amdgcn_mfma_f32_16x16x32_f16(FW(i, 0), AHB(1, 0, s), aB[1], 0, 0, 0);
          __builtin_amdgcn_sched_barrier(0);
          if (i + 2 < NST) ld_step(i + 2, F[(i + 2) % 3]);
        }
        {
          const f16x8 fw = __builtin_bit_cast(f16x8, Ft);
          const f16x4 fh = __builtin_bit_cast(f16x4, (u32x2){Ft[0], Ft[1]});
          aS[0] = __builtin_amdgcn_mfma_f32_16x16x32_f16(fw, __builtin_bit_cast(f16x8, Atc[0]), aS[0], 0, 0, 0);
          aS[1] = __builtin_amdgcn_mfma_f32_16x16x32_f16(fw, __builtin_bit_cast(f16x8, Atc[1]), aS[1], 0, 0, 0);
          aB[0] = __builtin_amdgcn_mfma_f32_16x16x16f16(fh, __builtin_bit_cast(f16x4, (u32x2){Atc[0][2], Atc[0][3]}), aB[0], 0, 0, 0);
          aB[1] = __builtin_amdgcn_mfma_f32_16x16x16f16(fh, __builtin_bit_cast(f16x4, (u32x2){Atc[1][2], Atc[1][3]}), aB[1], 0, 0, 0);
          __builtin_amdgcn_sched_barrier(0);
          if (m + 1 < KT) ld_tail(m + 1);
        }
        f32x4 rv = {1.f, 1.f, 1.f, 1.f};
        if constexpr (ROWF) if (d.w.W1rinv) rv = *reinterpret_cast<const f32x4*>(d.w.W1rinv + 16 * m + 4 * g);
#pragma unroll
        for (int b = 0; b < 2; ++b)
#pragma unroll
          for (int r = 0; r < 4; ++r) { H[b][m][r] = fmaxf(aS[b][r] + aB[b][r], 0.f); if constexpr (ROWF) H[b][m][r] *= rv[r]; mx[b] = fmaxf(mx[b], H[b][m][r]); }
      }
#undef AHB
#undef FW
      const int k1 = d.w.k1;
#pragma unroll
      for (int b = 0; b < 2; ++b) {
        float m2 = fmaxf(mx[b], __shfl_xor(mx[b], 16));
        m2 = fmaxf(m2, __shfl_xor(m2, 32));
        const int j = __builtin_amdgcn_frexp_expf(m2);
        const int tot = max(-120, min(64, 15 - j + k1 + 15 - ja[b]));
        const float t = __builtin_amdgcn_ldexpf(1.f, tot - k1 - 15 + ja[b]);
        se[b] = __builtin_amdgcn_ldexpf(1.f, tot);
        ue[b] = __builtin_amdgcn_ldexpf(1.f, -tot);
#pragma unroll
        for (int m = 0; m < KT; ++m) {
          unsigned hi0, lo0, hi1, lo1;
          split2x2(H[b][m][0] * t, H[b][m][1] * t, hi0, lo0);
          split2x2(H[b][m][2] * t, H[b][m][3] * t, hi1, lo1);
          if (m < 8) {
            Bh[b][0][m >> 1][2 * (m & 1)] = hi0; Bh[b][0][m >> 1][2 * (m & 1) + 1] = hi1;
            Bh[b][1][m >> 1][2 * (m & 1)] = lo0; Bh[b][1][m >> 1][2 * (m & 1) + 1] = lo1;
          } else {
            Btc[b] = (u32x4){lo0, lo1, hi0, hi1};
          }
        }
      }
    }
    __builtin_amdgcn_wave_barrier();
    {
      const int d4 = min(D_in, 120) >> 2;
      const float* xsrc = d.x + (size_t)s_gth[lane & 31] * d.ldx;
      float* xdst = xs + (lane & 31) * C2_XLD;
      f32x4 v[15];
#pragma unroll
      for (int j = 0; j < 15; ++j) v[j] = *reinterpret_cast<const f32x4*>(xsrc + 4 * min(2 * j + (lane >> 5), d4 - 1));
#pragma unroll
      for (int j = 0; j < 15; ++j) *reinterpret_cast<f32x4*>(xdst + 4 * min(2 * j + (lane >> 5), d4 - 1)) = v[j];
    }
    __builtin_amdgcn_wave_barrier();

    if (ABL & 64) {
      asm volatile("" ::"v"(Bh[0][0][0]), "v"(Bh[1][1][3]), "v"(Btc[1]));
      continue;
    }
    float oacc[2][3];
#pragma unroll
    for (int b = 0; b < 2; ++b) oacc[b][0] = oacc[b][1] = oacc[b][2] = 0.f;
    const float* xs_lane = xs + n * C2_XLD;
    const float* sh_lane = shs + n * 10;
    f16x8 FA[2], FB[2];
    f16x8 FT;
    f32x4 bias_n;
    f32x4 accN[2];
    f32x4 accS[2], accB[2];
    f32x4 accp[2];
    f32x4 rinv_c = {1.f, 1.f, 1.f, 1.f}, rinv_n = {1.f, 1.f, 1.f, 1.f};
    const float* rinv_base = ROWF && d.w.W2rinv ? d.w.W2rinv + 4 * g : nullptr;
    auto sumr4 = [&](f32x4& o, const f32x4& x, const f32x4& y) {
      if constexpr (ROWF) { o[0] = (x[0] + y[0]) * rinv_c[0]; o[1] = (x[1] + y[1]) * rinv_c[1]; o[2] = (x[2] + y[2]) * rinv_c[2]; o[3] = (x[3] + y[3]) * rinv_c[3]; }
      else sum4(o, x, y);
    };
    auto rd_step = [&](auto jc, f16x8 (&F)[2]) {
      constexpr int j = decltype(jc)::value;
#pragma unroll
      for (int i = 0; i < 2; ++i) F[i] = *reinterpret_cast<const f16x8*>(ring + (i * 4 + j) * 1024 + vW);
    };
    auto ring_barrier = [&] {
      __builtin_amdgcn_sched_barrier(0);
      asm volatile("s_waitcnt lgkmcnt(0)" ::: "memory");
      if (!(ABL & 2)) __builtin_amdgcn_s_barrier();
      __builtin_amdgcn_sched_barrier(0);
    };
#define HB(b, p, s) __builtin_bit_cast(f16x8, Bh[b][p][s])
#define M32(C, wp, b, hp, F, s) __builtin_amdgcn_mfma_f32_16x16x32_f16(F[wp], HB(b, hp, s), C, 0, 0, 0)
#define MT32(C, b) __builtin_amdgcn_mfma_f32_16x16x32_f16(FT, __builtin_bit_cast(f16x8, Btc[b]), C, 0, 0, 0)
#define MT16(C, b) __builtin_amdgcn_mfma_f32_16x16x16f16(__builtin_shufflevector(FT, FT, 0, 1, 2, 3), __builtin_bit_cast(f16x4, (u32x2){Btc[b][2], Btc[b][3]}), C, 0, 0, 0)
#define SLOT(m) do { op(std::integral_constant<int, (m)>{}); __builtin_amdgcn_sched_barrier(0); } while (0)
    auto tile = [&](int t, auto&& op) {
      const f32x4 zero = {0.f, 0.f, 0.f, 0.f};
      accS[0] = M32(accN[0], 0, 0, 1, FA, 0); if (ABL & 256) putB(); SLOT(0);
      accS[1] = M32(accN[1], 0, 1, 1, FA, 0); if (ABL & 256) fetchB(min(t + 1, t_last)); SLOT(1);
      accS[0] = M32(accS[0], 1, 0, 0, FA, 0); rd_step(I1{}, FB); SLOT(2);
      accS[1] = M32(accS[1], 1, 1, 0, FA, 0); SLOT(3);
      accB[0] = M32(zero, 0, 0, 0, FA, 0); SLOT(4);
      accB[1] = M32(zero, 0, 1, 0, FA, 0); SLOT(5);
      accS[0] = M32(accS[0], 0, 0, 1, FB, 1); SLOT(6);
      accS[1] = M32(accS[1], 0, 1, 1, FB, 1); SLOT(7);
      accS[0] = M32(accS[0], 1, 0, 0, FB, 1); rd_step(I2{}, FA); SLOT(8);
      accS[1] = M32(accS[1], 1, 1, 0, FB, 1); if (!(ABL & 256)) putB(); SLOT(9);
      accB[0] = M32(accB[0], 0, 0, 0, FB, 1); if (!(ABL & (256 | 32))) fetchB(min(t + 1, t_last)); SLOT(10);
      accB[1] = M32(accB[1], 0, 1, 0, FB, 1); SLOT(11);
      ring_barrier();
      accS[0] = M32(accS[0], 0, 0, 1, FA, 2); if (ABL & 256) putA(); SLOT(12);
      accS[1] = M32(accS[1], 0, 1, 1, FA, 2); if (ABL & 256) fetchA(min(t + 2, t_last)); SLOT(13);
      accS[0] = M32(accS[0], 1, 0, 0, FA, 2); rd_step(I3{}, FB); SLOT(14);
      accS[1] = M32(accS[1], 1, 1, 0, FA, 2); SLOT(15);
// ... 112 lines not shown
          else if (TYPE == PT_VS) { oacc[b][0] += cz0 * S[b][0]; oacc[b][1] += cz1 * S[b][0]; oacc[b][2] += cz2 * S[b][0]; }
          else if (TYPE == PT_VVS) { oacc[b][0] += cz0 * S[b][0]; oacc[b][0] += cz1 * S[b][1]; oacc[b][0] += cz2 * S[b][2]; }
          else if (TYPE == PT_VVV) {
            oacc[b][0] += cz1 * S[b][2]; oacc[b][1] += cz2 * S[b][0]; oacc[b][2] += cz0 * S[b][1];
            oacc[b][0] -= cz2 * S[b][1]; oacc[b][1] -= cz0 * S[b][2]; oacc[b][2] -= cz1 * S[b][0];
          } else {
            oacc[b][0] += Mv[b][0] * cz0; oacc[b][1] += Mv[b][1] * cz0; oacc[b][2] += Mv[b][2] * cz0;
            oacc[b][0] += Mv[b][1] * cz1; oacc[b][1] += Mv[b][3] * cz1; oacc[b][2] += Mv[b][4] * cz1;
            oacc[b][0] += Mv[b][2] * cz2; oacc[b][1] += Mv[b][4] * cz2; oacc[b][2] += Mv[b][5] * cz2;
          }
        };
        using B0 = std::integral_constant<int, 0>;
        using B1 = std::integral_constant<int, 1>;
        auto travel = [&](auto mc, const float* xp) {
          constexpr int m = decltype(mc)::value;
          if constexpr (m == 0) cop(B0{}, std::integral_constant<int, 0>{}, xp);
          if constexpr (m >= 3 && m <= 14) cop(B0{}, std::integral_constant<int, m - 2>{}, xp);
          if constexpr (m == 12) cop(B1{}, std::integral_constant<int, 0>{}, xp);
          if constexpr (m >= 15 && m <= 26) cop(B1{}, std::integral_constant<int, m - 14>{}, xp);
          if constexpr (m == 26) scale4(accN[0], bias_n, se[0]);
          if constexpr (m == 27) { scale4(accN[1], bias_n, se[1]); sumr4(accp[0], accS[0], accB[0]); }
        };
        const float* xp = xs_lane + xo;
        accp[0] = (f32x4){0.f, 0.f, 0.f, 0.f}; accp[1] = (f32x4){0.f, 0.f, 0.f, 0.f};
        for (int i = 0; i < nt; ++i) {
          tile(tile0 + i, [&](auto mc) { travel(mc, xp); });
          if (i) xp += x_step;
        }
        __builtin_amdgcn_sched_barrier(0);
#define COPS(b) cop(b, std::integral_constant<int, 0>{}, xp); cop(b, std::integral_constant<int, 1>{}, xp); cop(b, std::integral_constant<int, 2>{}, xp); \
        cop(b, std::integral_constant<int, 3>{}, xp); cop(b, std::integral_constant<int, 4>{}, xp); cop(b, std::integral_constant<int, 5>{}, xp); \
        cop(b, std::integral_constant<int, 6>{}, xp); cop(b, std::integral_constant<int, 7>{}, xp); cop(b, std::integral_constant<int, 8>{}, xp); \
        cop(b, std::integral_constant<int, 9>{}, xp); cop(b, std::integral_constant<int, 10>{}, xp); cop(b, std::integral_constant<int, 11>{}, xp); \
        cop(b, std::integral_constant<int, 12>{}, xp); finish(b);
        COPS(B0{}) COPS(B1{})
#undef COPS
        if (flags & 2) {
          if (oo < D_out) {
#pragma unroll
            for (int b = 0; b < 2; ++b)
              if (e0 + 16 * b + n < E) {
                float* op = d.msg + (size_t)(e0 + 16 * b + n) * D_out + oo;
                op[0] = oacc[b][0] * ue[b];
                if (VOUT) { op[1] = oacc[b][1] * ue[b]; op[2] = oacc[b][2] * ue[b]; }
              }
          }
        }
      };
      switch (type) {
        case PT_SS: run(std::integral_constant<int, PT_SS>{}); break;
        case PT_SV: run(std::integral_constant<int, PT_SV>{}); break;
        case PT_VS: run(std::integral_constant<int, PT_VS>{}); break;
        case PT_VVS: run(std::integral_constant<int, PT_VVS>{}); break;
        case PT_VVV: run(std::integral_constant<int, PT_VVV>{}); break;
        default: run(std::integral_constant<int, PT_VTV>{}); break;
      }
    }
#undef M32
#undef MT32
#undef MT16
#undef HB
#undef TB
  }
  if (a.trace && blockIdx.x == 0 && tid == 0) { a.trace[2] = __builtin_readcyclecounter(); a.trace[3] = __builtin_amdgcn_s_memrealtime(); }
}

void launch_conv2h(const Conv2Args& a, hipStream_t st) {
  static int no_split = getenv("DBFR_CONV2_NOSPLIT") ? atoi(getenv("DBFR_CONV2_NOSPLIT")) : 0;
  constexpr int NW = 8;
  const size_t lds = CH_RING_BYTES + (size_t)NW * C2_WAVE_FLOATS * sizeof(float);
  const int n_cu = dbfr_current_cu_count();
  Conv2Args b = a;
  b.skew = 0;
  b.run_barrier = 0;
  b.no_split = no_split;
#define V(x) { if (dbfr_launch_check(hipFuncSetAttribute(reinterpret_cast<const void*>(&k_conv2h<NW, x>), hipFuncAttributeMaxDynamicSharedMemorySize, (int)lds), "k_conv2h: hipFuncSetAttribute(MaxDynamicSharedMemorySize)")) return; \
               hipLaunchKernelGGL((k_conv2h<NW, x>), dim3(n_cu), dim3(64 * NW), lds, st, b); return; }
#ifdef DBFR_DEV_VARIANTS
  static int abl = getenv("DBFR_CONV2H_ABL") ? atoi(getenv("DBFR_CONV2H_ABL")) : 0;
  if (abl == 1) V(1) if (abl == 2) V(2) if (abl == 3) V(3) if (abl == 4) V(4) if (abl == 7) V(7) if (abl == 8) V(8) if (abl == 16) V(16)
  if (abl == 32) V(32) if (abl == 64) V(64) if (abl == 256) V(256) if (abl == 512) V(512)
#endif
  for (int i = 0; i < a.n_conv; ++i)
    if (a.c[i].w.W2rinv || a.c[i].w.W1rinv) V(1024)
  V(0)
#undef V
}
```

diffbindfr_amd/csrc/convz.hip:

```cpp
#include <cstdio>
#include <cstdlib>
#include <type_traits>

#include "common.h"

typedef float f32x4 __attribute__((ext_vector_type(4)));
typedef float f32x2 __attribute__((ext_vector_type(2)));
typedef _Float16 f16x8 __attribute__((ext_vector_type(8)));
typedef _Float16 f16x4 __attribute__((ext_vector_type(4)));
typedef _Float16 f16x2 __attribute__((ext_vector_type(2)));
typedef unsigned u32x4 __attribute__((ext_vector_type(4)));
typedef unsigned u32x2 __attribute__((ext_vector_type(2)));

#define CH_TILE_BYTES 9280
#define CH_TAIL_OFF 8192
#define CH_BIAS_OFF 9216

#define CZ_VSTRIDE 2064
#define CZ_CB (8 * CZ_VSTRIDE)
#define CZ_NCB 2
#define CZ_TILE (CZ_NCB * CZ_CB)
#define CZ_KPB 1
#define CZ_BUF (CZ_KPB * CZ_TILE)
#define CZ_ZBYTES (2 * CZ_BUF)
// ... 517 lines not shown
              if constexpr (kt == CZ_PF_KT) if (ct + 1 < W.nct[io]) prefetch_x(ct + 1);
            } else
              tile9(ct);
            stamp(12);
            ++gq;
            if (!(ABL & 2)) __syncthreads();
            stamp(13);
          });
        }
      };
      if (ncb > 1) run_tiles(K2{}); else run_tiles(K1{});
#undef YM
#undef MF
#undef SL
      float* red = reinterpret_cast<float*>(zb) + wave * (12 * CZ_NCB * 64);
#pragma unroll
      for (int wt = 0; wt < 3; ++wt)
#pragma unroll
        for (int cb = 0; cb < CZ_NCB; ++cb)
#pragma unroll
          for (int q = 0; q < 4; ++q) red[((wt * CZ_NCB + cb) * 4 + q) * 64 + lane] = acc[wt][cb][q];
      __syncthreads();
      for (int idx = tid; idx < 16 * ncb * 48; idx += 64 * NW) {
        const int col = idx / 48, w = idx - 48 * col;
        const int e = b_col_edge[col];
        if (e >= 0) {
          const int r = w & 15;
          const float* rp = reinterpret_cast<const float*>(zb) + (((w >> 4) * CZ_NCB + (col >> 4)) * 4 + (r & 3)) * 64 + 16 * (r >> 2) + (col & 15);
          float s = 0.f;
#pragma unroll
          for (int v = 0; v < NW; ++v) s += rp[v * (12 * CZ_NCB * 64)];
          d.msg[(size_t)e * d.D_out + W.out_off[io] + w] = s * b_col_inv[col] * W.rowinv[io * 48 + w];
        }
      }
      __syncthreads();
    }
    if (a.executed && lane == 0) atomicAdd(a.executed, 16384.0 * (double)n_mfma);
  }
}

__global__ void k_convz_useful(ConvZArgs a) {
  for (int c = 0; c < a.n_conv; ++c) {
    const ConvZDesc& d = a.c[c];
    const ConvZ& W = d.w;
    const int nch = min(*d.n_chunks, d.max_chunks), E = min(*d.n_edges, d.max_edges);
    double useful = 0.0, bytes = 0.0;
    for (int ch = blockIdx.x * blockDim.x + threadIdx.x; ch < nch; ch += gridDim.x * blockDim.x) {
      const int es = d.chunk_es[ch], len = min(min(d.chunk_gl[ch] & 63, 32), max(E - es, 0));
      int nseg = 0;
      for (int i = 0; i < len; ++i) nseg += (i == 0 || d.tgt[es + i] != d.tgt[es + i - 1]);
      nseg = min(nseg, CZ_MAXSEG);
      double u = 144.0 * 144.0 * len;
      for (int io = 0; io < W.n_io; ++io) u += (double)W.nc_valid[io] * 145.0 * ((double)len + 48.0 * nseg);
      useful += 6.0 * u;
      bytes += 4.0 * 48.0 * W.n_io * nseg;
    }
    if (useful > 0.0) { atomicAdd(a.executed + 1, useful); atomicAdd(a.executed + 2, bytes); }
  }
}

size_t convz_lds_bytes() { return CZ_ZBYTES + 8 * CZ_WAVE_FLOATS * sizeof(float) + (8 + 2 * 16 * CZ_NCB + CZ_MAXCT * 16) * sizeof(int); }

void launch_convz(const ConvZArgs& a0, hipStream_t st) {
  constexpr int NW = 8;
  ConvZArgs a = a0;
  static float* dbg_dev = nullptr;
  static const char* dbg_file = getenv("DBFR_CONVZ_DEBUG");
  if (dbg_file && !dbg_dev) {
    if (hipMalloc(&dbg_dev, 8 * 1024 * 8) != hipSuccess || hipMemset(dbg_dev, 0, 8 * 1024 * 8) != hipSuccess) dbg_dev = nullptr;
    else atexit([] {
      std::vector<float> h(8 * 1024 * 2);
      if (hipDeviceSynchronize() == hipSuccess && hipMemcpy(h.data(), dbg_dev, h.size() * 4, hipMemcpyDeviceToHost) == hipSuccess)
        if (FILE* f = fopen(getenv("DBFR_CONVZ_DEBUG"), "wb")) { fwrite(h.data(), 4, h.size(), f); fclose(f); }
    });
  }
  a.dbg = dbg_dev;
  const size_t lds = convz_lds_bytes();
#define V(x) { if (dbfr_launch_check(hipFuncSetAttribute(reinterpret_cast<const void*>(&k_convz<NW, x>), hipFuncAttributeMaxDynamicSharedMemorySize, (int)lds), "k_convz: hipFuncSetAttribute(MaxDynamicSharedMemorySize)")) return; \
               hipLaunchKernelGGL((k_convz<NW, x>), dim3(dbfr_current_cu_count()), dim3(64 * NW), lds, st, a); return; }
#ifdef DBFR_DEV_VARIANTS
  static int abl = getenv("DBFR_CONVZ_ABL") ? atoi(getenv("DBFR_CONVZ_ABL")) : 0;
  if (abl == 1) V(1) if (abl == 2) V(2) if (abl == 4) V(4) if (abl == 8) V(8) if (abl == 16) V(16) if (abl == 32) V(32) if (abl == 12) V(12) if (abl == 5) V(5) if (abl == 64) V(64) if (abl == 128) V(128)
#endif
  if (a.executed) hipLaunchKernelGGL(k_convz_useful, dim3(64), dim3(256), 0, st, a);
  V(0)
#undef V
}
```

diffbindfr_amd/lib.py:

```python
import ctypes as C
import os

HERE = os.path.dirname(os.path.abspath(__file__))
LIB_PATH = os.environ.get("DBFR_LIB") or os.path.join(HERE, "libdbfr.so")

DBFR_OK = 0
DBFR_ERR_CAPACITY = -3
ERRORS = {-1: "DBFR_ERR_ARG", -2: "DBFR_ERR_HIP", -3: "DBFR_ERR_CAPACITY", -4: "DBFR_ERR_SELFTEST",
          -5: "DBFR_ERR_NUMERIC"}

i32, f32, vp = C.c_int32, C.c_float, C.c_void_p


class ModelCfg(C.Structure):
    _fields_ = [(n, i32) for n in ("ns", "nv", "sh_lmax", "num_conv_layers", "lig_node_features",
                                   "lig_edge_features", "distance_embed_dim", "sigma_embed_dim")] + \
               [(n, f32) for n in ("emb_scale", "lig_cutoff", "atom_cutoff", "cross_cutoff", "center_max_distance")] + \
               [(n, i32) for n in ("atom_max_neighbors", "lig_max_neighbors", "dynamic_max_cross", "scale_by_sigma",
                                   "no_sc_torsion")]


class Tensor(C.Structure):
    _fields_ = [("name", C.c_char_p), ("data", vp), ("numel", C.c_int64)]

# ... 56 lines not shown
    _fields_ = [(n, C.c_int32) for n in ("B", "NL", "EL", "NR", "EP")] + [(n, C.c_void_p) for n in _MDN_PTRS] + \
               [("dist_threshold", C.c_float)]


class SdfTemplate(C.Structure):
    _fields_ = [("n_atoms", C.c_int32), ("header", C.c_char_p), ("atom_tail", C.POINTER(C.c_char_p)), ("trailer", C.c_char_p)]


class PdbTopology(C.Structure):
    _fields_ = [("n_res", C.c_int32), ("aatype", C.c_void_p), ("atom37_pos", C.c_void_p), ("atom37_mask", C.c_void_p),
                ("residue_index", C.c_void_p), ("chain_index", C.c_void_p), ("b_factors", C.c_void_p),
                ("remark", C.c_char_p)]


class VinaIn(C.Structure):
    _fields_ = [("batch", C.c_void_p), ("lig_type", C.c_void_p), ("rec_type", C.c_void_p), ("pair_ptr", C.c_void_p),
                ("pair_ij", C.c_void_p), ("n_pairs", C.c_int32), ("ext_ptr", C.c_void_p), ("ext_pos", C.c_void_p),
                ("ext_type", C.c_void_p), ("max_tor", C.c_int32), ("max_ext", C.c_int32)]


class VinaOpts(C.Structure):
    _fields_ = [("max_iters", C.c_int32), ("grad_tol", C.c_float), ("margin", C.c_float)]


class PoseRmsdIn(C.Structure):
    _fields_ = [("n_group", C.c_int32), ("pose_ptr", C.c_void_p), ("atom_ptr", C.c_void_p), ("perm_ptr", C.c_void_p),
                ("pos", C.c_void_p), ("perms", C.c_void_p), ("heavy_mask", C.c_void_p), ("max_pose", C.c_int32),
                ("max_atom", C.c_int32), ("path", C.c_int32), ("tile_rows", C.c_int32)]


class ModesOpts(C.Structure):
    _fields_ = [("num_modes", C.c_int32), ("higher_is_better", C.c_int32), ("min_rmsd", C.c_float), ("cluster_rmsd", C.c_float),
                ("energy_range", C.c_float)]


class PoseCheckIn(C.Structure):
    _fields_ = [("n_group", C.c_int32), ("n_frame", C.c_int32)] + \
               [(n, C.c_void_p) for n in ("frame_ptr", "lig_ptr", "lig_pos_off", "lig_pos", "lig_rad", "pocket_ptr", "pocket_pos_off",
                                          "pocket_pos", "pocket_rad", "static_ptr", "static_pos", "static_rad", "pair_ptr", "pair_ij",
                                          "flat_ptr", "flat_atoms", "stereo_ptr", "stereo_atoms", "stereo_sign")] + \
               [(n, C.c_int32) for n in ("max_lig", "max_pair", "max_flat", "max_stereo", "cand_cap")]


class PoseCheckOpts(C.Structure):
    _fields_ = [(n, C.c_float) for n in ("clash_ratio", "max_distance", "vol_scale", "vol_overlap", "internal_ratio", "flat_tol", "grid")]


class PoseCheckOut(C.Structure):
    _fields_ = [(n, C.c_void_p) for n in ("min_dist", "min_ratio", "n_clash", "vol_lig", "vol_overlap", "int_min_ratio", "n_int_clash",
                                          "flat_dev", "n_stereo_flip", "passed")]


class PdbLigand(C.Structure):
    _fields_ = [("n_atoms", i32), ("head", C.c_char_p), ("atom_line", C.POINTER(C.c_char_p)), ("tail", C.c_char_p)]


class XtcIn(C.Structure):
    _fields_ = [(n, i32) for n in ("n_frame", "n_file", "n_src", "n_lig", "n_res", "n_static", "n_map", "max_atoms")] + \
               [(n, vp) for n in ("lig", "pos14", "center", "static_pos", "map_ptr", "atom_map", "file_map", "frame_file",
                                  "frame_src", "frame_step")]


class XtcOpts(C.Structure):
    _fields_ = [("precision", f32), ("dt", f32), ("first_step", i32), ("box", f32 * 9)]


class SitesOpts(C.Structure):
    _fields_ = [(n, f32) for n in ("spacing", "probe", "ray_length", "lining_cutoff")] + \
               [(n, i32) for n in ("min_buried", "min_points", "max_sites")]


class SitesIn(C.Structure):
    _fields_ = [("n_prot", i32), ("n_res", i32), ("max_points", C.c_int64)] + \
               [(n, vp) for n in ("res_ptr", "aatype", "atom37_pos", "atom37_mask", "radius")]


class SitesOut(C.Structure):
    _fields_ = [(n, vp) for n in ("n_sites", "label", "n_points", "score", "idx_sum", "centre", "lining", "grid", "occupancy",
                                  "burial", "labels")]


SYMBOLS = ["dbfr_model_create", "dbfr_model_destroy", "dbfr_model_set_edge_log", "dbfr_model_set_tie_log", "dbfr_model_fallback_convs", "dbfr_model_rowscaled_convs", "dbfr_model_set_gemm", "dbfr_model_get_gemm", "dbfr_workspace_bytes", "dbfr_score", "dbfr_sample",
           "dbfr_sample_range", "dbfr_capacity_report",
           "dbfr_init_poses", "dbfr_extract_templates", "dbfr_status_sync", "dbfr_abi_version", "dbfr_build_id", "dbfr_last_error", "dbfr_wigner3j", "dbfr_conv_paths", "dbfr_test_pack_f16_tiles", "dbfr_test_pack_f16_rows", "dbfr_test_chunk_table", "dbfr_test_pack_f16_depth", "dbfr_probe_mfma_f16",
           "dbfr_profile_enable", "dbfr_profile_read", "dbfr_profile_fused_bytes", "dbfr_profile_executed_flops", "dbfr_profile_useful_flops", "dbfr_workspace_layout", "dbfr_test_conv", "dbfr_test_conv2", "dbfr_test_reduce_ln", "dbfr_test_reduce_ln2", "dbfr_test_sde_step",
           "dbfr_pose_metrics", "dbfr_pdb_format", "dbfr_pdb_write_files", "dbfr_select_pocket", "dbfr_sdf_format",
           "dbfr_sdf_write_files", "dbfr_mdn_model_create", "dbfr_mdn_model_destroy", "dbfr_mdn_workspace_bytes", "dbfr_mdn_forward", "dbfr_mdn_pocket_features",
           "dbfr_vina_workspace_bytes", "dbfr_vina_score", "dbfr_vina_score_at", "dbfr_vina_minimize",
           "dbfr_pose_rmsd_matrix", "dbfr_select_modes", "dbfr_pose_check",
           "dbfr_pdb_atom_map", "dbfr_complex_pdb_format", "dbfr_complex_pdb_write_files", "dbfr_xtc_workspace_bytes", "dbfr_xtc_encode",
           "dbfr_sites_workspace_bytes", "dbfr_find_sites"]

_lib = None


class DbfrError(RuntimeError):
    pass


def load():
    global _lib
    if _lib is not None:
        return _lib
    if not os.path.exists(LIB_PATH):
        raise DbfrError(f"{LIB_PATH} is missing: build the HIP library first "
                        f"(python -m diffbindfr_amd.build). There is no CPU fallback.")
    lib = C.CDLL(LIB_PATH)
    lib.dbfr_last_error.restype = C.c_char_p
    lib.dbfr_build_id.restype = C.c_char_p
    lib.dbfr_model_create.argtypes = [C.POINTER(ModelCfg), C.POINTER(Tensor), i32, C.POINTER(vp)]
    lib.dbfr_model_destroy.argtypes = [vp]
    lib.dbfr_model_destroy.restype = None
    lib.dbfr_model_set_edge_log.argtypes = [vp, vp, i32, i32]
    lib.dbfr_model_set_tie_log.argtypes = [vp, vp, i32, i32, C.c_float]
    lib.dbfr_model_fallback_convs.argtypes = [vp, C.c_char_p, C.c_size_t]
    lib.dbfr_model_rowscaled_convs.argtypes = [vp, C.c_char_p, C.c_size_t]
    lib.dbfr_model_set_gemm.argtypes = [vp, i32]
    lib.dbfr_model_get_gemm.argtypes = [vp]
    lib.dbfr_workspace_bytes.argtypes = [vp, C.POINTER(Batch), C.POINTER(Limits), C.POINTER(C.c_size_t)]
    lib.dbfr_score.argtypes = [vp, C.POINTER(Batch), C.POINTER(Cond), C.POINTER(Scores), vp, C.c_size_t,
                               C.POINTER(Limits), vp]
    lib.dbfr_sample.argtypes = [vp, C.POINTER(Batch), C.POINTER(Step), i32, C.POINTER(Noise), vp, vp, vp, vp,
                                C.c_size_t, C.POINTER(Limits), vp]
    lib.dbfr_sample_range.argtypes = [vp, C.POINTER(Batch), C.POINTER(Step), i32, i32, C.POINTER(Noise), vp, vp, vp, vp,
                                      C.c_size_t, C.POINTER(Limits), vp]
    lib.dbfr_capacity_report.argtypes = [vp, vp, C.POINTER(i32), C.POINTER(C.c_int64)]
    lib.dbfr_init_poses.argtypes = [vp, C.POINTER(Batch), C.POINTER(InitTape), vp, vp]
    lib.dbfr_extract_templates.argtypes = [i32, vp, vp, vp, vp, vp, vp, vp, vp]
    lib.dbfr_status_sync.argtypes = [vp, vp, C.POINTER(C.c_int64)]
    lib.dbfr_wigner3j.argtypes = [i32, i32, i32, C.POINTER(C.c_double)]
    lib.dbfr_conv_paths.argtypes = [i32, C.POINTER(i32), i32, C.POINTER(i32)]
    lib.dbfr_test_pack_f16_tiles.argtypes = [vp, vp, i32, vp, C.POINTER(i32)]
    lib.dbfr_test_pack_f16_depth.argtypes = [vp, vp, i32, C.POINTER(i32), C.POINTER(i32)]
    lib.dbfr_test_pack_f16_rows.argtypes = [vp, vp, i32, vp, C.POINTER(i32), vp, C.POINTER(i32)]
    lib.dbfr_test_chunk_table.argtypes = [vp, vp, i32, i32, vp, i32, vp, vp, vp]
    lib.dbfr_probe_mfma_f16.argtypes = [C.c_double, C.POINTER(C.c_double), vp]
    lib.dbfr_profile_enable.argtypes = [vp, i32]
    lib.dbfr_profile_fused_bytes.argtypes = [vp, C.POINTER(C.c_double)]
    lib.dbfr_profile_executed_flops.argtypes = [vp, C.POINTER(C.c_double)]
    lib.dbfr_profile_useful_flops.argtypes = [vp, C.POINTER(C.c_double), C.POINTER(C.c_double)]
    lib.dbfr_profile_read.argtypes = [vp, C.POINTER(C.c_double), C.POINTER(C.c_int64), C.POINTER(C.c_double),
                                      C.POINTER(C.c_double), i32]
    lib.dbfr_workspace_layout.argtypes = [vp, C.POINTER(Batch), C.POINTER(Limits), C.c_char_p, C.c_size_t,
                                          C.POINTER(C.c_size_t), C.POINTER(C.c_size_t), i32]
    lib.dbfr_test_conv.argtypes = [vp, i32, i32, i32, vp, vp, vp, vp, vp, vp, i32, vp, vp, i32, vp, vp, i32, vp, vp]
    lib.dbfr_test_conv2.argtypes = lib.dbfr_test_conv.argtypes
    lib.dbfr_test_reduce_ln.argtypes = [vp, i32, i32, vp, vp, vp, i32, vp, i32, vp, i32, vp]
    lib.dbfr_test_reduce_ln2.argtypes = [vp, i32, i32, vp, vp, vp, i32, vp, i32, vp, i32, vp, vp]
    lib.dbfr_test_sde_step.argtypes = [vp, C.POINTER(Batch), C.POINTER(Step), C.POINTER(Scores), C.POINTER(Noise), vp, vp, vp]
    lib.dbfr_select_pocket.argtypes = [i32, i32, vp, i32, vp, vp, vp, vp, C.c_double, i32, vp, vp, vp]
    lib.dbfr_pose_metrics.argtypes = [C.POINTER(PoseMetricsIn), C.POINTER(PoseMetricsOut), vp]
    lib.dbfr_pdb_format.argtypes = [C.POINTER(PdbTopology), i32, vp, vp, i32, i32, vp, C.c_int64]
    lib.dbfr_pdb_format.restype = C.c_int64
    lib.dbfr_pdb_write_files.argtypes = [C.POINTER(PdbTopology), i32, vp, vp, i32, C.POINTER(C.c_char_p), i32]
    lib.dbfr_sdf_format.argtypes = [C.POINTER(SdfTemplate), vp, vp, C.c_int64]
    lib.dbfr_sdf_format.restype = C.c_int64
    lib.dbfr_sdf_write_files.argtypes = [C.POINTER(SdfTemplate), vp, i32, C.POINTER(C.c_char_p), i32]
    lib.dbfr_mdn_model_create.argtypes = [C.POINTER(Tensor), i32, C.POINTER(vp)]
    lib.dbfr_mdn_model_destroy.argtypes = [vp]
    lib.dbfr_mdn_model_destroy.restype = None
    lib.dbfr_mdn_workspace_bytes.argtypes = [C.POINTER(MdnBatch), C.POINTER(C.c_size_t)]
    lib.dbfr_mdn_pocket_features.argtypes = [i32, i32, vp, vp, vp, vp, i32, vp, vp, vp, vp, vp, vp, vp, vp]
    lib.dbfr_mdn_forward.argtypes = [vp, C.POINTER(MdnBatch), vp, vp, vp, vp, C.c_size_t, vp]
    lib.dbfr_vina_workspace_bytes.argtypes = [C.POINTER(VinaIn), C.POINTER(C.c_size_t)]
    lib.dbfr_vina_score.argtypes = [C.POINTER(VinaIn), vp, vp, vp, vp, C.c_size_t, vp]
    lib.dbfr_vina_score_at.argtypes = [C.POINTER(VinaIn), vp, vp, vp, vp, vp, vp, vp, C.c_size_t, vp]
    lib.dbfr_vina_minimize.argtypes = [C.POINTER(VinaIn), C.POINTER(VinaOpts), vp, vp, vp, vp, C.c_size_t, vp]
    lib.dbfr_pose_rmsd_matrix.argtypes = [C.POINTER(PoseRmsdIn), vp, vp]
    lib.dbfr_select_modes.argtypes = [C.POINTER(PoseRmsdIn), vp, vp, C.POINTER(ModesOpts), vp, vp, vp, vp]
    lib.dbfr_pose_check.argtypes = [C.POINTER(PoseCheckIn), C.POINTER(PoseCheckOpts), C.POINTER(PoseCheckOut), vp]
    lib.dbfr_pdb_atom_map.argtypes = [C.POINTER(PdbTopology), i32, vp, vp, vp, C.c_int64, C.POINTER(C.c_int64)]
    lib.dbfr_pdb_atom_map.restype = C.c_int64
    lib.dbfr_complex_pdb_format.argtypes = [C.POINTER(PdbTopology), i32, vp, vp, C.POINTER(PdbLigand), vp, vp, C.c_int64]
    lib.dbfr_complex_pdb_format.restype = C.c_int64
    lib.dbfr_complex_pdb_write_files.argtypes = [C.POINTER(PdbTopology), i32, vp, vp, C.POINTER(PdbLigand), vp, i32,
                                                 C.POINTER(C.c_char_p), i32]
    lib.dbfr_xtc_workspace_bytes.argtypes = [C.POINTER(XtcIn), C.POINTER(C.c_size_t), C.POINTER(C.c_int64)]
    lib.dbfr_xtc_encode.argtypes = [C.POINTER(XtcIn), C.POINTER(XtcOpts), vp, C.c_int64, vp, vp, C.c_size_t, vp]
    lib.dbfr_sites_workspace_bytes.argtypes = [C.POINTER(SitesIn), C.POINTER(C.c_size_t)]
    lib.dbfr_find_sites.argtypes = [C.POINTER(SitesIn), C.POINTER(SitesOpts), C.POINTER(SitesOut), vp, C.c_size_t, vp]
    if lib.dbfr_abi_version() != 7:
        raise DbfrError("libdbfr ABI version mismatch")
    _lib = lib
    return lib


def check(rc):
    if rc != DBFR_OK:
        msg = load().dbfr_last_error().decode()
        raise DbfrError(f"{ERRORS.get(rc, rc)}: {msg}")


def workspace_views(model_handle, batch_c, limits, ws):
    lib = load()
    names = C.create_string_buffer(8192)
    offs = (C.c_size_t * 128)()
    nbytes = (C.c_size_t * 128)()
    n = lib.dbfr_workspace_layout(model_handle, C.byref(batch_c), C.byref(limits), names, 8192, offs, nbytes, 128)
    if n < 0:
        check(n)
    out = {}
    for i, nm in enumerate(names.value.decode().split(";")[:n]):
        out[nm] = ws[offs[i]:offs[i] + nbytes[i]]
    return out
```

include/dbfr.h:

```cpp
#ifndef DBFR_H
#define DBFR_H

#include <stddef.h>
#include <stdint.h>

#ifdef __cplusplus
extern "C" {
#endif

#define DBFR_ABI_VERSION 7

typedef enum {
  DBFR_OK = 0,
  DBFR_ERR_ARG = -1,
  DBFR_ERR_HIP = -2,
  DBFR_ERR_CAPACITY = -3,
  DBFR_ERR_SELFTEST = -4,
  DBFR_ERR_NUMERIC = -5
} dbfr_status;

typedef struct dbfr_model dbfr_model;

typedef struct {
  int32_t ns, nv, sh_lmax;
// ... 357 lines not shown
  int32_t        max_atoms;
  const float*   lig;
  const float*   pos14;
  const float*   center;
  const float*   static_pos;
  const int32_t* map_ptr;
  const int32_t* atom_map;
  const int32_t* file_map;
  const int32_t* frame_file;
  const int32_t* frame_src;
  const int32_t* frame_step;
} dbfr_xtc_in;

typedef struct {
  float   precision;
  float   dt;
  int32_t first_step;
  float   box[9];
} dbfr_xtc_opts;

int dbfr_xtc_workspace_bytes(const dbfr_xtc_in* in, size_t* bytes, int64_t* out_cap);
int dbfr_xtc_encode(const dbfr_xtc_in* in, const dbfr_xtc_opts* opts, uint8_t* out, int64_t out_cap, int64_t* offsets,
                    void* workspace, size_t workspace_bytes, void* hip_stream);

typedef struct {
  float   spacing;
  float   probe;
  float   ray_length;
  float   lining_cutoff;
  int32_t min_buried;
  int32_t min_points;
  int32_t max_sites;
} dbfr_sites_opts;

typedef struct {
  int32_t        n_prot;
  int32_t        n_res;
  int64_t        max_points;
  const int32_t* res_ptr;
  const int32_t* aatype;
  const float*   atom37_pos;
  const float*   atom37_mask;
  const float*   radius;
} dbfr_sites_in;

typedef struct {
  int32_t* n_sites;
  int32_t* label;
  int32_t* n_points;
  int32_t* score;
  int64_t* idx_sum;
  double*  centre;
  uint8_t* lining;
  int32_t* grid;
  uint8_t* occupancy;
  uint8_t* burial;
  int32_t* labels;
} dbfr_sites_out;

int dbfr_sites_workspace_bytes(const dbfr_sites_in* in, size_t* bytes);
int dbfr_find_sites(const dbfr_sites_in* in, const dbfr_sites_opts* opts, const dbfr_sites_out* out, void* workspace,
                    size_t workspace_bytes, void* hip_stream);

int dbfr_status_sync(void* workspace, void* hip_stream, int64_t* counters);

#define DBFR_GEMM_F32 0
#define DBFR_GEMM_SPLIT_F16 3
#define DBFR_GEMM_REDUCE_FIRST 4
#define DBFR_GEMM_DEFAULT DBFR_GEMM_REDUCE_FIRST
int dbfr_model_set_gemm(dbfr_model* model, int32_t mode);
int dbfr_model_rowscaled_convs(const dbfr_model* model, char* names, size_t names_cap);
int dbfr_model_fallback_convs(const dbfr_model* model, char* names, size_t names_cap);
int dbfr_model_get_gemm(const dbfr_model* model);

int         dbfr_abi_version(void);
const char* dbfr_build_id(void);
const char* dbfr_last_error(void);
int dbfr_wigner3j(int32_t l1, int32_t l2, int32_t l3, double* out);
int dbfr_conv_paths(int32_t kind, int32_t* table10, int32_t max_paths, int32_t* weight_numel);
int dbfr_test_chunk_table(const int32_t* tgt, const int32_t* n_edges_dev, int32_t max_edges, int32_t span, int32_t* scratch, int32_t cap,
                          int32_t* chunk_es, int32_t* chunk_gl, void* hip_stream);
int dbfr_test_pack_f16_tiles(const float* frag, const float* bias, int32_t n_tiles, void* out, int32_t* k_out);
int dbfr_test_pack_f16_rows(const float* frag, const float* bias, int32_t n_tiles, void* out, int32_t* k_out, float* rinv_out, int32_t* depth_out);
int dbfr_test_pack_f16_depth(const float* frag, const float* bias, int32_t n_tiles, int32_t* depth_out, int32_t* depth_ok_out);
int dbfr_profile_enable(dbfr_model* m, int32_t on);
int dbfr_profile_read(dbfr_model* m, double* conv_ms, int64_t* conv_launches, double* conv_flops,
                      double* ref_form_bytes, int32_t reset);
int dbfr_profile_fused_bytes(const dbfr_model* m, double* fused_form_bytes);
int dbfr_profile_executed_flops(const dbfr_model* m, double* executed_flops);
int dbfr_profile_useful_flops(const dbfr_model* m, double* useful_flops, double* form_bytes);

int dbfr_probe_mfma_f16(double seconds, double* tflops, void* hip_stream);

int dbfr_workspace_layout(const dbfr_model* m, const dbfr_batch* b, const dbfr_limits* lim, char* names,
                          size_t names_cap, size_t* offsets, size_t* bytes, int32_t max_entries);

int dbfr_test_conv(dbfr_model* m, int32_t layer, int32_t family, int32_t n_edges, const int32_t* n_edges_dev,
                   const int32_t* tgt, const int32_t* gth, const float* emb, const float* sh, const float* tab1,
                   int32_t ld1, const int32_t* idx1, const float* tab2, int32_t ld2, const int32_t* idx2,
                   const float* x, int32_t ldx, float* msg, void* hip_stream);
int dbfr_test_conv2(dbfr_model* m, int32_t layer, int32_t family, int32_t n_edges, const int32_t* n_edges_dev,
                    const int32_t* tgt, const int32_t* gth, const float* emb, const float* sh, const float* tab1,
                    int32_t ld1, const int32_t* idx1, const float* tab2, int32_t ld2, const int32_t* idx2,
                    const float* x, int32_t ldx, float* msg, void* hip_stream);
int dbfr_test_reduce_ln(dbfr_model* m, int32_t layer, int32_t family, const float* msg, const int32_t* row_start,
                        const int32_t* row_cnt, int32_t n_nodes, const float* old, int32_t d_old, float* out,
                        int32_t mode, void* hip_stream);
int dbfr_test_reduce_ln2(dbfr_model* m, int32_t layer, int32_t family, const float* msg, const int32_t* row_start,
                         const int32_t* row_cnt, int32_t n_nodes, const float* old, int32_t d_old, float* out,
                         int32_t mode, const uint8_t* seg_first, void* hip_stream);

int dbfr_test_sde_step(const dbfr_model* m, const dbfr_batch* b, const dbfr_step* step, const dbfr_scores* scores,
                       const dbfr_noise* z, float* atom14_out, int32_t* err_word_out, void* hip_stream);

#ifdef __cplusplus
}
#endif
#endif
```

Measured before the change: 493.6.

## Factor first conv MLP layer into per-row precomputed terms plus edge-only MFMA

The first fc layer's K=144 input splits into an edge-embedding part (48 columns) and two node-feature parts. The node-feature parts become per-node row terms computed once by a new k_row_terms kernel and stored in workspace buffers P, so the per-edge split-f16 MFMA only covers the 48 edge columns. This removes redundant per-edge work on node features, at the cost of an extra kernel launch, extra workspace, and gathers of the precomputed row terms. Separately, the convz useful-flops profiling launch is split out and the f16 tile loads are double-buffered.

```diff
diff --git a/diffbindfr_amd/csrc/api.cpp b/diffbindfr_amd/csrc/api.cpp
--- a/diffbindfr_amd/csrc/api.cpp
+++ b/diffbindfr_amd/csrc/api.cpp
@@ -11,7 +11,9 @@
 void launch_conv_layer(const ConvArgs* c4, hipStream_t st);
 void launch_conv2(const Conv2Args& a, hipStream_t st);
 void launch_conv2h(const Conv2Args& a, hipStream_t st);
+void launch_row_terms(const RowTermArgs& a, hipStream_t st);
 void launch_convz(const ConvZArgs& a, hipStream_t st);
+void launch_convz_useful(const ConvZArgs& a, hipStream_t st);
 void launch_reduce_ln(const float* msg, const int* row_start, const int* row_cnt, int N, int D, const LNDesc& ln,
                       const float* old, int D_old, float* out, int ldo, int mode, hipStream_t st, const uint8_t* first = nullptr, unsigned long long sc_lanes = 0);
 struct ReduceLayerArgs {
@@ -448,6 +450,60 @@
   return k;
 }
 
+#define W1A_TILE_BYTES_HOST 3072
+static int pack_w1_factored(const float* W1, uint16_t* w1a, float* rinv, float* w1bt, float* w1ct, int* depth) {
+  constexpr int K = 144, KT = 9, KE = NS;
+  auto h16 = [](float v) { const _Float16 h = (_Float16)v; uint16_t u; memcpy(&u, &h, 2); return u; };
+  float mx = 0.f;
+  for (int u = 0; u < K; ++u)
+    for (int k = 0; k < KE; ++k) mx = std::max(mx, fabsf(W1[(size_t)u * K + k]));
+  int e = 0;
+  if (mx > 0.f) (void)frexpf(mx, &e);
+  const int k1a = mx > 0.f ? std::max(-120, std::min(120, 15 - e)) : 0;
+  int dmax = 0;
+  for (int u = 0; u < K; ++u) {
+    float rm = 0.f;
+    for (int k = 0; k < KE; ++k) rm = std::max(rm, fabsf(W1[(size_t)u * K + k]));
+    int up = 0;
+    if (rm > 0.f) {
+      int er = 0;
+      (void)frexpf(rm, &er);
+      int d = 15 - (er + k1a);
+      if (rinv) { up = std::min(std::max(d, 0), 100); d -= up; }
+      dmax = std::max(dmax, d);
+    }
+    if (rinv) rinv[u] = ldexpf(1.f, -up);
+    const float sc = ldexpf(1.f, k1a + up);
+    const int mt = u >> 4, row = u & 15;
+    uint16_t* tile = w1a + (size_t)mt * (W1A_TILE_BYTES_HOST / 2);
+    for (int k = 0; k < KE; ++k) {
+      const float v = W1[(size_t)u * K + k] * sc;
+      const _Float16 hi = (_Float16)v;
+      const uint16_t pc[2] = {h16(v), h16(v - (float)hi)};
+      const int s4 = k >> 4, lane = 16 * ((k >> 2) & 3) + row, q = k & 3;
+      for (int i = 0; i < 2; ++i) {
+        if (s4 < 2) tile[((size_t)i * 64 + lane) * 8 + 4 * s4 + q] = pc[i];
+        else tile[1024 + (size_t)lane * 8 + 4 * i + q] = pc[i];
+      }
+    }
+    for (int k = 0; k < NS; ++k) {
+      w1bt[(size_t)k * K + u] = W1[(size_t)u * K + KE + k];
+      w1ct[(size_t)k * K + u] = W1[(size_t)u * K + KE + NS + k];
+    }
+  }
+  if (depth) *depth = dmax;
+  return k1a;
+}
+
+extern "C" int dbfr_test_pack_w1_factored(const float* W1, int32_t per_row, void* w1a_out, int32_t* k1a_out, float* rinv_out, float* w1bt_out, float* w1ct_out,
+                                          int32_t* depth_out) {
+  if (!W1 || !w1a_out || !k1a_out || !w1bt_out || !w1ct_out || (per_row && !rinv_out)) return fail(DBFR_ERR_ARG, "dbfr_test_pack_w1_factored: bad argument");
+  int depth = 0;
+  *k1a_out = pack_w1_factored(W1, (uint16_t*)w1a_out, per_row ? rinv_out : nullptr, w1bt_out, w1ct_out, &depth);
+  if (depth_out) *depth_out = depth;
+  return DBFR_OK;
+}
+
 static int pack_conv2(dbfr_model* m, const TMap& tm, const std::string& name, int kind, const ConvW& base, ConvW2* o, bool vector_only = false) {
   ConvSpec sp = make_conv_spec(kind);
   const int K = sp.K;
@@ -603,6 +659,22 @@
       o->W1rinv = upload(m, w1rinv, &rc);
     }
     o->W1h = upload(m, w1h, &rc);
+    {
+      std::vector<uint16_t> w1a((size_t)KT * (W1A_TILE_BYTES_HOST / 2) + 512, 0);
+      std::vector<float> w1bt((size_t)NS * K), w1ct((size_t)NS * K), w1arinv(K, 1.f);
+      int deptha = 0;
+      o->k1a = pack_w1_factored(W1, w1a.data(), nullptr, w1bt.data(), w1ct.data(), &deptha);
+      depth_run = std::max(depth_run, deptha);
+      if (rowscale == 2 || (rowscale == 1 && deptha > F16_ROW_DEPTH_OK)) {
+        o->k1a = pack_w1_factored(W1, w1a.data(), w1arinv.data(), w1bt.data(), w1ct.data(), &deptha);
+        o->W1arinv = upload(m, w1arinv, &rc);
+      }
+      o->W1aru = o->W1arinv ? o->W1arinv : upload(m, w1arinv, &rc);
+      depth1 = std::max(depth1, deptha);
+      o->W1a = upload(m, w1a, &rc);
+      o->W1bt = upload(m, w1bt, &rc);
+      o->W1ct = upload(m, w1ct, &rc);
+    }
     o->f16_depth = std::max(depth_max, depth1);
     o->f16_depth_run = depth_run;
   }
@@ -854,7 +926,7 @@
       rc = pack_conv(m, tm, std::string(fam[f]) + "." + std::to_string(l), std::min(l, 3), &m->layer[l][f]);
       if (!rc) rc = pack_conv2(m, tm, std::string(fam[f]) + "." + std::to_string(l), std::min(l, 3), m->layer[l][f], &m->layer2[l][f]);
       if (!rc && m->layer2[l][f].f16_depth > f16_depth_ok()) { m->layer_fallback |= 1u << l; m->fallback_convs += std::string(fam[f]) + "." + std::to_string(l) + ";"; }
-      if (!rc && (m->layer2[l][f].W2rinv || m->layer2[l][f].W1rinv)) m->rowscaled_convs += std::string(fam[f]) + "." + std::to_string(l) + ":" + std::to_string(m->layer2[l][f].f16_depth_run) + ";";
+      if (!rc && (m->layer2[l][f].W2rinv || m->layer2[l][f].W1rinv || m->layer2[l][f].W1arinv)) m->rowscaled_convs += std::string(fam[f]) + "." + std::to_string(l) + ":" + std::to_string(m->layer2[l][f].f16_depth_run) + ";";
       if (!rc) rc = pack_conv2(m, tm, std::string(fam[f]) + "." + std::to_string(l), std::min(l, 3), m->layer[l][f], &m->layer2v[l][f], true);
       if (!rc) rc = pack_convz(m, tm, std::string(fam[f]) + "." + std::to_string(l), std::min(l, 3), m->layer2[l][f], &m->layerz[l][f]);
     }
@@ -862,12 +934,12 @@
   if (!rc) rc = pack_conv(m, tm, "tor_bond_conv", 5, &m->tor_conv);
   if (!rc) rc = pack_conv2(m, tm, "tor_bond_conv", 5, m->tor_conv, &m->tor_conv2);
   if (!rc && m->tor_conv2.f16_depth > f16_depth_ok()) { m->layer_fallback |= 1u << 31; m->fallback_convs += "tor_bond_conv;"; }
-  if (!rc && (m->tor_conv2.W2rinv || m->tor_conv2.W1rinv)) m->rowscaled_convs += "tor_bond_conv:" + std::to_string(m->tor_conv2.f16_depth_run) + ";";
+  if (!rc && (m->tor_conv2.W2rinv || m->tor_conv2.W1rinv || m->tor_conv2.W1arinv)) m->rowscaled_convs += "tor_bond_conv:" + std::to_string(m->tor_conv2.f16_depth_run) + ";";
   if (!rc) rc = pack_convz(m, tm, "tor_bond_conv", 5, m->tor_conv2, &m->tor_convz);
   if (!rc && !cfg->no_sc_torsion) rc = pack_conv(m, tm, "sc_tor_bond_conv", 5, &m->sc_conv);
   if (!rc && !cfg->no_sc_torsion) rc = pack_conv2(m, tm, "sc_tor_bond_conv", 5, m->sc_conv, &m->sc_conv2);
   if (!rc && !cfg->no_sc_torsion && m->sc_conv2.f16_depth > f16_depth_ok()) { m->layer_fallback |= 1u << 31; m->fallback_convs += "sc_tor_bond_conv;"; }
-  if (!rc && !cfg->no_sc_torsion && (m->sc_conv2.W2rinv || m->sc_conv2.W1rinv)) m->rowscaled_convs += "sc_tor_bond_conv:" + std::to_string(m->sc_conv2.f16_depth_run) + ";";
+  if (!rc && !cfg->no_sc_torsion && (m->sc_conv2.W2rinv || m->sc_conv2.W1rinv || m->sc_conv2.W1arinv)) m->rowscaled_convs += "sc_tor_bond_conv:" + std::to_string(m->sc_conv2.f16_depth_run) + ";";
   if (!rc && !cfg->no_sc_torsion) rc = pack_convz(m, tm, "sc_tor_bond_conv", 5, m->sc_conv2, &m->sc_convz);
   if (!rc) rc = pack_mlp(m, tm, "lig_node_embedding", cfg->lig_node_features + EMB, NS, NS, true, &m->lig_node_emb);
   if (!rc) rc = pack_mlp(m, tm, "lig_edge_embedding", cfg->lig_edge_features + 2 * EMB, NS, NS, true, &m->lig_edge_emb);
@@ -945,6 +1017,7 @@
   EdgeSet set[N_SETS];
   int *c_tgt, *c_gth, *c_row_start, *c_row_cnt, *c_n; float *c_dist, *c_sh, *c_emb;
   float* msg[4]; int multi; int conv2; float* gp; float *tor_attr, *sc_attr, *tor_feat, *sc_feat;
+  float* P[8];
   float *xmax_l, *xmax_a;
   int* n_edges6;
 };
@@ -1008,6 +1081,11 @@
   for (int i = 0; i < 4; ++i) w->msg[i] = (i == 0 || w->multi) ? b.take<float>((size_t)maxcap * MAXD, i == 0 ? "msg" : nullptr) : nullptr;
   w->gp = b.take<float>((size_t)G * 12, "gp");
   w->xmax_l = b.take<float>(G, "xmax_l"); w->xmax_a = b.take<float>(G, "xmax_a");
+  for (int i = 0; i < 8; ++i) w->P[i] = nullptr;
+  if ((w->conv2 || m->conv2_layers > 0) && m->gemm_split >= DBFR_GEMM_SPLIT_F16) {
+    const long pr[8] = {NL, std::max(NL, B->NTOR), std::max(NL, NA), std::max(NA, B->NSC), NA, NA, NA, NL};
+    for (int i = 0; i < 8; ++i) w->P[i] = b.take<float>((size_t)std::max(pr[i], 1L) * P_LD, i == 0 ? "row_terms" : nullptr);
+  }
   w->tor_attr = b.take<float>((size_t)(B->NTOR + 1) * NS, "tor_attr"); w->sc_attr = b.take<float>((size_t)(B->NSC + 1) * NS);
   w->tor_feat = b.take<float>((size_t)(B->NTOR + 1) * 2 * NS, "tor_feat"); w->sc_feat = b.take<float>((size_t)(B->NSC + 1) * 2 * NS);
   *need_bytes = b.off + 256;
@@ -1067,6 +1145,7 @@
   Conv2Desc d;
   d.n_edges = n_edges; d.max_edges = max_edges; d.gth = gth; d.emb = emb; d.sh = sh; d.tab1 = tab1; d.ld1 = ld1; d.idx1 = idx1;
   d.tab2 = tab2; d.ld2 = ld2; d.idx2 = idx2; d.x = x; d.ldx = ldx; d.w = cw; d.msg = msg;
+  d.P1 = d.P2 = nullptr; d.rows1 = d.rows2 = 0;
   return d;
 }
 
@@ -1077,6 +1156,30 @@
   o.tab1 = d.tab1; o.ld1 = d.ld1; o.idx1 = d.idx1; o.tab2 = d.tab2; o.ld2 = d.ld2; o.idx2 = d.idx2; o.x = d.x; o.ldx = d.ldx;
   o.w = z; o.msg = d.msg; o.D_out = D_out; o.chunk_es = chunk_es; o.chunk_gl = chunk_gl; o.n_chunks = n_chunks; o.max_chunks = max_chunks; o.xmax = xmax;
   return o;
+}
+
+static void with_row_terms(Conv2Desc& d, float* P1, int rows1, float* P2, int rows2) { d.P1 = P1; d.rows1 = rows1; d.P2 = P2; d.rows2 = rows2; }
+
+static void row_terms_call(const Conv2Desc* ds, int n, hipStream_t st) {
+  RowTermArgs ra;
+  memset(&ra, 0, sizeof ra);
+  auto add = [&](const float* tab, int ld, int rows, const float* Wt, const float* b, float* P) {
+    if (rows <= 0) return;
+    RowTermSet* s = nullptr;
+    for (int i = 0; i < ra.n_set; ++i)
+      if (ra.s[i].tab == tab && ra.s[i].ld == ld && ra.s[i].n_rows == rows && ra.s[i].n_tab < 4) s = &ra.s[i];
+    if (!s) {
+      if (ra.n_set == 4) { launch_row_terms(ra, st); memset(&ra, 0, sizeof ra); }
+      s = &ra.s[ra.n_set++];
+      s->tab = tab; s->ld = ld; s->n_rows = rows;
+    }
+    s->Wt[s->n_tab] = Wt; s->b[s->n_tab] = b; s->P[s->n_tab] = P; ++s->n_tab;
+  };
+  for (int i = 0; i < n; ++i) {
+    add(ds[i].tab1, ds[i].ld1, ds[i].rows1, ds[i].w.W1bt, nullptr, ds[i].P1);
+    add(ds[i].tab2, ds[i].ld2, ds[i].rows2, ds[i].w.W1ct, ds[i].w.b1, ds[i].P2);
+  }
+  if (ra.n_set) launch_row_terms(ra, st);
 }
 
 static void conv2_call(dbfr_model* m, const Conv2Desc* descs, const int* Ws, int n, hipStream_t st, bool f16_fallback = false, const ConvZDesc* z = nullptr) {
@@ -1106,7 +1209,7 @@
     v.n_conv = 0;
     for (int i = 0; i < n; ++i)
       if (descs[i].w.n_tiles > 0) v.c[v.n_conv++] = descs[i];
-    if (v.n_conv) launch_conv2h(v, st);
+    if (v.n_conv) { row_terms_call(v.c, v.n_conv, st); launch_conv2h(v, st); }
     ConvZArgs za;
     memset(&za, 0, sizeof za);
     for (int i = 0; i < n; ++i) za.c[i] = z[i];
@@ -1114,10 +1217,12 @@
     za.dbg = nullptr;
     za.executed = m->profile ? m->flops_dev + 3 : nullptr;
     launch_convz(za, st);
-  }
-  else if (m->gemm_split >= DBFR_GEMM_SPLIT_F16 && !f16_fallback) launch_conv2h(a, st);
+    if (m->profile == 1) { (void)hipEventRecord(e1, st); e1 = nullptr; }
+    if (za.executed) launch_convz_useful(za, st);
+  }
+  else if (m->gemm_split >= DBFR_GEMM_SPLIT_F16 && !f16_fallback) { row_terms_call(a.c, n, st); launch_conv2h(a, st); }
   else launch_conv2(a, st);
-  if (m->profile == 1) (void)hipEventRecord(e1, st);
+  if (m->profile == 1 && e1) (void)hipEventRecord(e1, st);
   if (m->profile) {
     AccBatch ab; ab.count = 0;
     auto acc = [&](const int* ne, double coef, double* dst) { if (ab.count < 32) { ab.n[ab.count] = ne; ab.coef[ab.count] = coef; ab.dst[ab.count] = dst; ++ab.count; } };
@@ -1127,14 +1232,14 @@
       acc(descs[i].n_edges, fused_bytes(descs[i].w.D_in, descs[i].w.D_out), m->flops_dev + 2);
       const double rows = 16.0 * descs[i].w.n_tiles;
       const bool f16 = (m->gemm_split >= DBFR_GEMM_SPLIT_F16 && !f16_fallback) || z;
-      const double ex = f16 ? 3.0 * 2.0 * 144 * (144.0 + rows) : 2.0 * 144 * (144.0 + rows);
+      const double ex = f16 ? 3.0 * 2.0 * 144 * (48.0 + rows) : 2.0 * 144 * (144.0 + rows);
       if (!z || descs[i].w.n_tiles > 0) acc(descs[i].n_edges, ex, m->flops_dev + 3);
       if (!z) acc(descs[i].n_edges, ex, m->flops_dev + 4);
       else if (descs[i].w.n_tiles > 0) acc(descs[i].n_edges, 3.0 * 2.0 * 144 * rows, m->flops_dev + 4);
       const int D_in = descs[i].w.D_in, D_out = descs[i].w.D_out;
       const double in_bytes = 4.0 * (48 + 9 + 3 + 48 + 48 + D_in);
       if (!z) acc(descs[i].n_edges, fused_bytes(D_in, D_out), m->flops_dev + 5);
-      else acc(descs[i].n_edges, in_bytes + 1.0 + (descs[i].w.n_tiles > 0 ? in_bytes + 4.0 * (D_out - 48 * z[i].w.n_io) : 0.0), m->flops_dev + 5);
+      else acc(descs[i].n_edges, in_bytes + 1.0 + (descs[i].w.n_tiles > 0 ? in_bytes + 4.0 * 2 * (P_LD - 48) + 4.0 * (D_out - 48 * z[i].w.n_io) : 0.0), m->flops_dev + 5);
     }
     launch_acc_batch(ab, st);
   }
@@ -1192,11 +1297,15 @@
     if (w.conv2 || l < m->conv2_layers) {
       const bool rf = m->gemm_split == DBFR_GEMM_REDUCE_FIRST && !((m->layer_fallback >> l) & 1u);
       const ConvW2* L2 = rf ? m->layer2v[l] : m->layer2[l];
-      const Conv2Desc ds[4] = {
+      Conv2Desc ds[4] = {
           conv2_desc(L2[0], LL.n_edges, LL.cap, LL.gth, LL.emb, LL.sh, lx, Di, LL.tgt, lx, Di, LL.gth, lx, Di, w.msg[0]),
           conv2_desc(L2[1], AL.n_edges, AL.cap, AL.gth, AL.emb, AL.sh, lx, Di, AL.tgt, ax, Di, AL.gth, ax, Di, w.msg[1]),
           conv2_desc(L2[2], AA.n_edges, AA.cap, AA.gth, AA.emb, AA.sh, ax, Di, AA.tgt, ax, Di, AA.gth, ax, Di, w.msg[2]),
           conv2_desc(L2[3], LA.n_edges, LA.cap, LA.gth, LA.emb, LA.sh, ax, Di, LA.tgt, lx, Di, LA.gth, lx, Di, w.msg[3])};
+      if (w.P[0]) {
+        with_row_terms(ds[0], w.P[0], NL, w.P[1], NL); with_row_terms(ds[1], w.P[2], NL, w.P[3], NA);
+        with_row_terms(ds[2], w.P[4], NA, w.P[5], NA); with_row_terms(ds[3], w.P[6], NA, w.P[7], NL);
+      }
       const int Ws[4] = {m->layer[l][0].W, m->layer[l][1].W, m->layer[l][2].W, m->layer[l][3].W};
       if (rf) {
         launch_row_absmax(lx, B->lig_ptr, w.xmax_l, ax, B->atm_ptr, w.xmax_a, Di, Di, G, NA, st);
@@ -1311,6 +1420,7 @@
       a.gs_offset = m->gs_lig_off; a.gs_coeff = m->gs_lig_c; a.out = T.emb;
       launch_mlp(a, st);
       ds[nd] = conv2_desc(m->tor_conv2, T.n_edges, T.cap, T.gth, T.emb, T.sh, lx, D, T.gth, w.tor_attr, NS, T.tgt, lx, D, w.msg[0]);
+      if (w.P[0]) with_row_terms(ds[nd], w.P[0], NL, w.P[1], B->NTOR);
       if (rf) { ds[nd].w.n_tiles = 0; zs[nd] = convz_desc(ds[nd], m->tor_convz, T.tgt, 2 * NS, T.chunk_es, T.chunk_gl, T.chunk0 + G, T.chunk_cap, w.xmax_l); }
       Ws[nd++] = m->tor_conv.W;
     }
@@ -1321,6 +1431,7 @@
       a.gs_offset = m->gs_atom_off; a.gs_coeff = m->gs_atom_c; a.out = S.emb;
       launch_mlp(a, st);
       ds[nd] = conv2_desc(m->sc_conv2, S.n_edges, S.cap, S.gth, S.emb, S.sh, ax, D, S.gth, w.sc_attr, NS, S.tgt, ax, D, w.msg[1]);
+      if (w.P[0]) with_row_terms(ds[nd], w.P[2], NA, w.P[3], B->NSC);
       if (rf) { ds[nd].w.n_tiles = 0; zs[nd] = convz_desc(ds[nd], m->sc_convz, S.tgt, 2 * NS, S.chunk_es, S.chunk_gl, S.chunk0 + G, S.chunk_cap, w.xmax_a); }
       Ws[nd++] = m->sc_conv.W;
     }
@@ -1625,6 +1736,35 @@
     const bool rf = m->gemm_split == DBFR_GEMM_REDUCE_FIRST && !deep;
     Conv2Desc d = conv2_desc(rf && layer >= 0 ? m->layer2v[layer][family] : *cw2, n_edges_dev, n_edges, gth, emb, sh, tab1, ld1, idx1, tab2, ld2, idx2, x, ldx, msg);
     if (rf && layer < 0) d.w.n_tiles = 0;
+    static float* pterm_dev[16] = {nullptr}; static size_t pterm_floats[16] = {0};
+    if (m->gemm_split >= DBFR_GEMM_SPLIT_F16 && !deep && d.w.n_tiles > 0) {
+      int dev = 0;
+      HIPCHECK(hipGetDevice(&dev));
+      if (dev < 0 || dev >= 16) return fail(DBFR_ERR_ARG, "test hook: device index beyond 15");
+      hipStream_t hs = (hipStream_t)hip_stream;
+      int E = 0;
+      HIPCHECK(hipMemcpyAsync(&E, n_edges_dev, sizeof(int), hipMemcpyDeviceToHost, hs));
+      HIPCHECK(hipStreamSynchronize(hs));
+      E = std::max(0, std::min(E, n_edges));
+      int rows[2] = {0, 0};
+      std::vector<int> h((size_t)std::max(E, 1));
+      for (int t = 0; t < 2 && E > 0; ++t) {
+        HIPCHECK(hipMemcpyAsync(h.data(), t ? idx2 : idx1, (size_t)E * sizeof(int), hipMemcpyDeviceToHost, hs));
+        HIPCHECK(hipStreamSynchronize(hs));
+        for (int i = 0; i < E; ++i) {
+          if (h[i] < 0) return fail(DBFR_ERR_ARG, "test hook: negative table index");
+          rows[t] = std::max(rows[t], h[i] + 1);
+        }
+      }
+      const size_t need = ((size_t)rows[0] + rows[1] + 1) * P_LD;
+      if (need > pterm_floats[dev]) {
+        if (pterm_dev[dev]) HIPCHECK(hipFree(pterm_dev[dev]));
+        pterm_dev[dev] = nullptr; pterm_floats[dev] = 0;
+        HIPCHECK(hipMalloc(&pterm_dev[dev], need * sizeof(float)));
+        pterm_floats[dev] = need;
+      }
+      with_row_terms(d, pterm_dev[dev], rows[0], pterm_dev[dev] + (size_t)rows[0] * P_LD, rows[1]);
+    }
     static int* scratch_dev[16] = {nullptr}; static size_t scratch_dev_ints[16] = {0};
     int dev_id = 0;
     HIPCHECK(hipGetDevice(&dev_id));
diff --git a/diffbindfr_amd/csrc/common.h b/diffbindfr_amd/csrc/common.h
--- a/diffbindfr_amd/csrc/common.h
+++ b/diffbindfr_amd/csrc/common.h
@@ -78,6 +78,12 @@
   int f16_depth_run;
   const float* W2rinv;
   const float* W1rinv;
+  const void* W1a;
+  int k1a;
+  const float* W1arinv;
+  const float* W1aru;
+  const float* W1bt;
+  const float* W1ct;
   const void* W2h;
   const RunDesc* runs;
   int part_run[4][9];
@@ -93,7 +99,20 @@
   const float* x; int ldx;
   ConvW2 w;
   float* msg;
-};
+  float* P1; float* P2; int rows1, rows2;
+};
+
+#define W1A_TILE_BYTES 3072
+#define P_LD 144
+
+struct RowTermSet {
+  const float* tab; int ld; int n_rows; int blk0;
+  int n_tab;
+  const float* Wt[4];
+  const float* b[4];
+  float* P[4];
+};
+struct RowTermArgs { RowTermSet s[4]; int n_set, rows_per_blk; };
 
 struct Conv2Args {
   Conv2Desc c[4];
diff --git a/diffbindfr_amd/csrc/conv2h.hip b/diffbindfr_amd/csrc/conv2h.hip
--- a/diffbindfr_amd/csrc/conv2h.hip
+++ b/diffbindfr_amd/csrc/conv2h.hip
@@ -1,3 +1,4 @@
+#include <algorithm>
 #include <cstdio>
 #include <cstdlib>
 #include <type_traits>
@@ -114,8 +115,8 @@
       ev[b] = min(e, E - 1);
       gthv[b] = d.gth[ev[b]];
       r0[b] = d.emb + (size_t)ev[b] * NS;
-      r1[b] = d.tab1 + (size_t)d.idx1[ev[b]] * d.ld1;
-      r2[b] = d.tab2 + (size_t)d.idx2[ev[b]] * d.ld2;
+      r1[b] = d.P1 + (size_t)d.idx1[ev[b]] * P_LD;
+      r2[b] = d.P2 + (size_t)d.idx2[ev[b]] * P_LD;
     }
     if (g == 0) { s_gth[n] = gthv[0]; s_gth[16 + n] = gthv[1]; }
     if (lane < 32) {
@@ -132,74 +133,62 @@
     u32x4 Btc[2];
     float se[2], ue[2];
     {
-      const __amdgpu_buffer_rsrc_t rW1 = __builtin_amdgcn_make_buffer_rsrc((void*)d.w.W1h, 0, KT * CH_TILE_BYTES, 0x00020000);
-      u32x4 Ah[2][2][4];
+      const __amdgpu_buffer_rsrc_t rW1 = __builtin_amdgcn_make_buffer_rsrc((void*)d.w.W1a, 0, KT * W1A_TILE_BYTES, 0x00020000);
+      u32x4 Ah[2][2];
       u32x4 Atc[2];
-      float sa[2];
-      int ja[2];
+      float fa[2];
+      float H[2][KT][4];
 #pragma unroll
       for (int b = 0; b < 2; ++b) {
-        f32x4 Ba[KT];
+        f32x4 Ba[3];
         float amx = 0.f;
 #pragma unroll
-        for (int s4 = 0; s4 < KT; ++s4) {
-          const float* src = s4 < 3 ? r0[b] : s4 < 6 ? r1[b] : r2[b];
-          Ba[s4] = *reinterpret_cast<const f32x4*>(src + 16 * (s4 % 3) + 4 * g);
+        for (int s4 = 0; s4 < 3; ++s4) {
+          Ba[s4] = *reinterpret_cast<const f32x4*>(r0[b] + 16 * s4 + 4 * g);
 #pragma unroll
           for (int q = 0; q < 4; ++q) amx = fmaxf(amx, fabsf(Ba[s4][q]));
+        }
+#pragma unroll
+        for (int m = 0; m < KT; ++m) {
+          const f32x4 p1 = *reinterpret_cast<const f32x4*>(r1[b] + 16 * m + 4 * g);
+          const f32x4 p2 = *reinterpret_cast<const f32x4*>(r2[b] + 16 * m + 4 * g);
+#pragma unroll
+          for (int r = 0; r < 4; ++r) H[b][m][r] = p1[r] + p2[r];
         }
         amx = fmaxf(amx, __shfl_xor(amx, 16));
         amx = fmaxf(amx, __shfl_xor(amx, 32));
-        ja[b] = max(-14, __builtin_amdgcn_frexp_expf(amx));
-        sa[b] = __builtin_amdgcn_ldexpf(1.f, 15 - ja[b]);
-#pragma unroll
-        for (int s4 = 0; s4 < KT; ++s4) {
-          unsigned hi0, lo0, hi1, lo1;
-          split2x2(Ba[s4][0] * sa[b], Ba[s4][1] * sa[b], hi0, lo0);
-          split2x2(Ba[s4][2] * sa[b], Ba[s4][3] * sa[b], hi1, lo1);
-          if (s4 < 8) {
-            Ah[b][0][s4 >> 1][2 * (s4 & 1)] = hi0; Ah[b][0][s4 >> 1][2 * (s4 & 1) + 1] = hi1;
-            Ah[b][1][s4 >> 1][2 * (s4 & 1)] = lo0; Ah[b][1][s4 >> 1][2 * (s4 & 1) + 1] = lo1;
-          } else {
-            Atc[b] = (u32x4){lo0, lo1, hi0, hi1};
-          }
-        }
-      }
-      constexpr int NST = KT * 4;
-      u32x4 F[3][2];
-      u32x4 Ft;
-      f32x4 bb;
-      auto ld_step = [&](int i, u32x4 (&f)[2]) {
-#pragma unroll
-        for (int p = 0; p < 2; ++p) f[p] = __builtin_bit_cast(u32x4, __builtin_amdgcn_raw_buffer_load_b128(rW1, vW, (i >> 2) * CH_TILE_BYTES + (p * 4 + (i & 3)) * 1024, 0));
+        const int ja = max(-14, __builtin_amdgcn_frexp_expf(amx));
+        const float sa = __builtin_amdgcn_ldexpf(1.f, 15 - ja);
+        fa[b] = __builtin_amdgcn_ldexpf(1.f, ja - 15 - d.w.k1a);
+        unsigned hi[3][2], lo[3][2];
+#pragma unroll
+        for (int s4 = 0; s4 < 3; ++s4) {
+          split2x2(Ba[s4][0] * sa, Ba[s4][1] * sa, hi[s4][0], lo[s4][0]);
+          split2x2(Ba[s4][2] * sa, Ba[s4][3] * sa, hi[s4][1], lo[s4][1]);
+        }
+        Ah[b][0] = (u32x4){hi[0][0], hi[0][1], hi[1][0], hi[1][1]};
+        Ah[b][1] = (u32x4){lo[0][0], lo[0][1], lo[1][0], lo[1][1]};
+        Atc[b] = (u32x4){lo[2][0], lo[2][1], hi[2][0], hi[2][1]};
+      }
+      u32x4 F[3][3];
+      auto ld_tile = [&](int m, u32x4 (&f)[3]) {
+#pragma unroll
+        for (int p = 0; p < 3; ++p) f[p] = __builtin_bit_cast(u32x4, __builtin_amdgcn_raw_buffer_load_b128(rW1, vW, m * W1A_TILE_BYTES + p * 1024, 0));
       };
-      auto ld_tail = [&](int m) {
-        Ft = __builtin_bit_cast(u32x4, __builtin_amdgcn_raw_buffer_load_b128(rW1, vW, m * CH_TILE_BYTES + CH_TAIL_OFF, 0));
-        bb = __builtin_bit_cast(f32x4, __builtin_amdgcn_raw_buffer_load_b128(rW1, vB, m * CH_TILE_BYTES + CH_BIAS_OFF, 0));
-      };
-      ld_step(0, F[0]); ld_step(1, F[1]); ld_tail(0);
-      float H[2][KT][4];
+      ld_tile(0, F[0]); ld_tile(1, F[1]);
       float mx[2] = {0.f, 0.f};
       const f32x4 zero = {0.f, 0.f, 0.f, 0.f};
-#define AHB(b, p, s) __builtin_bit_cast(f16x8, Ah[b][p][s])
-#define FW(i, p) __builtin_bit_cast(f16x8, F[(i) % 3][p])
 #pragma unroll
       for (int m = 0; m < KT; ++m) {
         f32x4 aS[2], aB[2];
-        scale4(aS[0], bb, sa[0]); scale4(aS[1], bb, sa[1]);
-        aB[0] = zero; aB[1] = zero;
-#pragma unroll
-        for (int s = 0; s < 4; ++s) {
-          const int i = m * 4 + s;
-          aS[0] = __builtin_amdgcn_mfma_f32_16x16x32_f16(FW(i, 0), AHB(0, 1, s), aS[0], 0, 0, 0);
-          aS[1] = __builtin_amdgcn_mfma_f32_16x16x32_f16(FW(i, 0), AHB(1, 1, s), aS[1], 0, 0, 0);
-          aS[0] = __builtin_amdgcn_mfma_f32_16x16x32_f16(FW(i, 1), AHB(0, 0, s), aS[0], 0, 0, 0);
-          aS[1] = __builtin_amdgcn_mfma_f32_16x16x32_f16(FW(i, 1), AHB(1, 0, s), aS[1], 0, 0, 0);
-          aB[0] = __builtin_amdgcn_mfma_f32_16x16x32_f16(FW(i, 0), AHB(0, 0, s), aB[0], 0, 0, 0);
-          aB[1] = __builtin_amdgcn_mfma_f32_16x16x32_f16(FW(i, 0), AHB(1, 0, s), aB[1], 0, 0, 0);
-          __builtin_amdgcn_sched_barrier(0);
-          if (i + 2 < NST) ld_step(i + 2, F[(i + 2) % 3]);
-        }
+        const f16x8 whi = __builtin_bit_cast(f16x8, F[m % 3][0]), wlo = __builtin_bit_cast(f16x8, F[m % 3][1]);
+        const u32x4 Ft = F[m % 3][2];
+        aS[0] = __builtin_amdgcn_mfma_f32_16x16x32_f16(whi, __builtin_bit_cast(f16x8, Ah[0][1]), zero, 0, 0, 0);
+        aS[1] = __builtin_amdgcn_mfma_f32_16x16x32_f16(whi, __builtin_bit_cast(f16x8, Ah[1][1]), zero, 0, 0, 0);
+        aS[0] = __builtin_amdgcn_mfma_f32_16x16x32_f16(wlo, __builtin_bit_cast(f16x8, Ah[0][0]), aS[0], 0, 0, 0);
+        aS[1] = __builtin_amdgcn_mfma_f32_16x16x32_f16(wlo, __builtin_bit_cast(f16x8, Ah[1][0]), aS[1], 0, 0, 0);
+        aB[0] = __builtin_amdgcn_mfma_f32_16x16x32_f16(whi, __builtin_bit_cast(f16x8, Ah[0][0]), zero, 0, 0, 0);
+        aB[1] = __builtin_amdgcn_mfma_f32_16x16x32_f16(whi, __builtin_bit_cast(f16x8, Ah[1][0]), zero, 0, 0, 0);
         {
           const f16x8 fw = __builtin_bit_cast(f16x8, Ft);
           const f16x4 fh = __builtin_bit_cast(f16x4, (u32x2){Ft[0], Ft[1]});
@@ -207,28 +196,29 @@
           aS[1] = __builtin_amdgcn_mfma_f32_16x16x32_f16(fw, __builtin_bit_cast(f16x8, Atc[1]), aS[1], 0, 0, 0);
           aB[0] = __builtin_amdgcn_mfma_f32_16x16x16f16(fh, __builtin_bit_cast(f16x4, (u32x2){Atc[0][2], Atc[0][3]}), aB[0], 0, 0, 0);
           aB[1] = __builtin_amdgcn_mfma_f32_16x16x16f16(fh, __builtin_bit_cast(f16x4, (u32x2){Atc[1][2], Atc[1][3]}), aB[1], 0, 0, 0);
-          __builtin_amdgcn_sched_barrier(0);
-          if (m + 1 < KT) ld_tail(m + 1);
-        }
+        }
+        __builtin_amdgcn_sched_barrier(0);
+        if (m + 2 < KT) ld_tile(m + 2, F[(m + 2) % 3]);
         f32x4 rv = {1.f, 1.f, 1.f, 1.f};
-        if constexpr (ROWF) if (d.w.W1rinv) rv = *reinterpret_cast<const f32x4*>(d.w.W1rinv + 16 * m + 4 * g);
+        if constexpr (ROWF) rv = *reinterpret_cast<const f32x4*>(d.w.W1aru + 16 * m + 4 * g);
 #pragma unroll
         for (int b = 0; b < 2; ++b)
 #pragma unroll
-          for (int r = 0; r < 4; ++r) { H[b][m][r] = fmaxf(aS[b][r] + aB[b][r], 0.f); if constexpr (ROWF) H[b][m][r] *= rv[r]; mx[b] = fmaxf(mx[b], H[b][m][r]); }
-      }
-#undef AHB
-#undef FW
-      const int k1 = d.w.k1;
+          for (int r = 0; r < 4; ++r) {
+            const float f = ROWF ? fa[b] * rv[r] : fa[b];
+            H[b][m][r] = fmaxf(__builtin_fmaf(aS[b][r] + aB[b][r], f, H[b][m][r]), 0.f);
+            mx[b] = fmaxf(mx[b], H[b][m][r]);
+          }
+      }
 #pragma unroll
       for (int b = 0; b < 2; ++b) {
         float m2 = fmaxf(mx[b], __shfl_xor(mx[b], 16));
         m2 = fmaxf(m2, __shfl_xor(m2, 32));
         const int j = __builtin_amdgcn_frexp_expf(m2);
-        const int tot = max(-120, min(64, 15 - j + k1 + 15 - ja[b]));
-        const float t = __builtin_amdgcn_ldexpf(1.f, tot - k1 - 15 + ja[b]);
+        const int tot = max(-120, min(64, 15 - j));
         se[b] = __builtin_amdgcn_ldexpf(1.f, tot);
         ue[b] = __builtin_amdgcn_ldexpf(1.f, -tot);
+        const float t = se[b];
 #pragma unroll
         for (int m = 0; m < KT; ++m) {
           unsigned hi0, lo0, hi1, lo1;
@@ -507,7 +497,65 @@
   if (abl == 32) V(32) if (abl == 64) V(64) if (abl == 256) V(256) if (abl == 512) V(512)
 #endif
   for (int i = 0; i < a.n_conv; ++i)
-    if (a.c[i].w.W2rinv || a.c[i].w.W1rinv) V(1024)
+    if (a.c[i].w.W2rinv || a.c[i].w.W1arinv) V(1024)
   V(0)
 #undef V
 }
+
+#define RT_CHUNK 32
+__global__ __launch_bounds__(192) void k_row_terms(RowTermArgs a) {
+  __shared__ __attribute__((aligned(16))) float xs[RT_CHUNK * NS];
+  int si = 0;
+  while (si + 1 < a.n_set && (int)blockIdx.x >= a.s[si + 1].blk0) ++si;
+  const RowTermSet& s = a.s[si];
+  const int row0 = ((int)blockIdx.x - s.blk0) * a.rows_per_blk, row1 = min(row0 + a.rows_per_blk, s.n_rows);
+  float w[3][NS], c[3];
+  float* out[3];
+#pragma unroll
+  for (int j = 0; j < 3; ++j) {
+    const int o = (int)threadIdx.x + 192 * j, t = o / 144, u = o - 144 * t;
+    const bool live = t < s.n_tab;
+    const float* Wt = s.Wt[live ? t : 0];
+#pragma unroll
+    for (int k = 0; k < NS; ++k) w[j][k] = Wt[k * 144 + u];
+    c[j] = live && s.b[t] ? s.b[t][u] : 0.f;
+    out[j] = live ? s.P[t] + u : nullptr;
+  }
+  const int lr = (int)threadIdx.x / 6, lp = ((int)threadIdx.x % 6) * 8;
+  for (int r0 = row0; r0 < row1; r0 += RT_CHUNK) {
+    const int nr = min(RT_CHUNK, row1 - r0);
+    __syncthreads();
+    if (lr < nr) {
+      const f32x4* src = reinterpret_cast<const f32x4*>(s.tab + (size_t)(r0 + lr) * s.ld + lp);
+      const f32x4 v0 = src[0], v1 = src[1];
+      *reinterpret_cast<f32x4*>(xs + lr * NS + lp) = v0;
+      *reinterpret_cast<f32x4*>(xs + lr * NS + lp + 4) = v1;
+    }
+    __syncthreads();
+    for (int r = 0; r < nr; ++r) {
+      float acc[3] = {c[0], c[1], c[2]};
+#pragma unroll
+      for (int k4 = 0; k4 < NS / 4; ++k4) {
+        const f32x4 x = *reinterpret_cast<const f32x4*>(xs + r * NS + 4 * k4);
+#pragma unroll
+        for (int q = 0; q < 4; ++q)
+#pragma unroll
+          for (int j = 0; j < 3; ++j) acc[j] = __builtin_fmaf(w[j][4 * k4 + q], x[q], acc[j]);
+      }
+#pragma unroll
+      for (int j = 0; j < 3; ++j)
+        if (out[j]) out[j][(size_t)(r0 + r) * P_LD] = acc[j];
+    }
+  }
+}
+
+void launch_row_terms(const RowTermArgs& a0, hipStream_t st) {
+  RowTermArgs a = a0;
+  long rows = 0;
+  for (int i = 0; i < a.n_set; ++i) rows += a.s[i].n_rows;
+  const int slots = std::max(2 * dbfr_current_cu_count() - a.n_set, 1);
+  a.rows_per_blk = (int)std::max(16L, (rows + slots - 1) / slots);
+  int nb = 0;
+  for (int i = 0; i < a.n_set; ++i) { a.s[i].blk0 = nb; nb += (a.s[i].n_rows + a.rows_per_blk - 1) / a.rows_per_blk; }
+  if (nb > 0) hipLaunchKernelGGL(k_row_terms, dim3(nb), dim3(192), 0, st, a);
+}
diff --git a/diffbindfr_amd/csrc/convz.hip b/diffbindfr_amd/csrc/convz.hip
--- a/diffbindfr_amd/csrc/convz.hip
+++ b/diffbindfr_amd/csrc/convz.hip
@@ -623,7 +623,10 @@
   static int abl = getenv("DBFR_CONVZ_ABL") ? atoi(getenv("DBFR_CONVZ_ABL")) : 0;
   if (abl == 1) V(1) if (abl == 2) V(2) if (abl == 4) V(4) if (abl == 8) V(8) if (abl == 16) V(16) if (abl == 32) V(32) if (abl == 12) V(12) if (abl == 5) V(5) if (abl == 64) V(64) if (abl == 128) V(128)
 #endif
-  if (a.executed) hipLaunchKernelGGL(k_convz_useful, dim3(64), dim3(256), 0, st, a);
   V(0)
 #undef V
 }
+
+void launch_convz_useful(const ConvZArgs& a, hipStream_t st) {
+  if (a.executed) hipLaunchKernelGGL(k_convz_useful, dim3(64), dim3(256), 0, st, a);
+}
diff --git a/diffbindfr_amd/lib.py b/diffbindfr_amd/lib.py
--- a/diffbindfr_amd/lib.py
+++ b/diffbindfr_amd/lib.py
@@ -162,7 +162,7 @@
 
 SYMBOLS = ["dbfr_model_create", "dbfr_model_destroy", "dbfr_model_set_edge_log", "dbfr_model_set_tie_log", "dbfr_model_fallback_convs", "dbfr_model_rowscaled_convs", "dbfr_model_set_gemm", "dbfr_model_get_gemm", "dbfr_workspace_bytes", "dbfr_score", "dbfr_sample",
            "dbfr_sample_range", "dbfr_capacity_report",
-           "dbfr_init_poses", "dbfr_extract_templates", "dbfr_status_sync", "dbfr_abi_version", "dbfr_build_id", "dbfr_last_error", "dbfr_wigner3j", "dbfr_conv_paths", "dbfr_test_pack_f16_tiles", "dbfr_test_pack_f16_rows", "dbfr_test_chunk_table", "dbfr_test_pack_f16_depth", "dbfr_probe_mfma_f16",
+           "dbfr_init_poses", "dbfr_extract_templates", "dbfr_status_sync", "dbfr_abi_version", "dbfr_build_id", "dbfr_last_error", "dbfr_wigner3j", "dbfr_conv_paths", "dbfr_test_pack_f16_tiles", "dbfr_test_pack_f16_rows", "dbfr_test_pack_w1_factored", "dbfr_test_chunk_table", "dbfr_test_pack_f16_depth", "dbfr_probe_mfma_f16",
            "dbfr_profile_enable", "dbfr_profile_read", "dbfr_profile_fused_bytes", "dbfr_profile_executed_flops", "dbfr_profile_useful_flops", "dbfr_workspace_layout", "dbfr_test_conv", "dbfr_test_conv2", "dbfr_test_reduce_ln", "dbfr_test_reduce_ln2", "dbfr_test_sde_step",
            "dbfr_pose_metrics", "dbfr_pdb_format", "dbfr_pdb_write_files", "dbfr_select_pocket", "dbfr_sdf_format",
            "dbfr_sdf_write_files", "dbfr_mdn_model_create", "dbfr_mdn_model_destroy", "dbfr_mdn_workspace_bytes", "dbfr_mdn_forward", "dbfr_mdn_pocket_features",
@@ -213,6 +213,7 @@
     lib.dbfr_test_pack_f16_tiles.argtypes = [vp, vp, i32, vp, C.POINTER(i32)]
     lib.dbfr_test_pack_f16_depth.argtypes = [vp, vp, i32, C.POINTER(i32), C.POINTER(i32)]
     lib.dbfr_test_pack_f16_rows.argtypes = [vp, vp, i32, vp, C.POINTER(i32), vp, C.POINTER(i32)]
+    lib.dbfr_test_pack_w1_factored.argtypes = [vp, i32, vp, C.POINTER(i32), vp, vp, vp, C.POINTER(i32)]
     lib.dbfr_test_chunk_table.argtypes = [vp, vp, i32, i32, vp, i32, vp, vp, vp]
     lib.dbfr_probe_mfma_f16.argtypes = [C.c_double, C.POINTER(C.c_double), vp]
     lib.dbfr_profile_enable.argtypes = [vp, i32]
diff --git a/include/dbfr.h b/include/dbfr.h
--- a/include/dbfr.h
+++ b/include/dbfr.h
@@ -463,6 +463,8 @@
                           int32_t* chunk_es, int32_t* chunk_gl, void* hip_stream);
 int dbfr_test_pack_f16_tiles(const float* frag, const float* bias, int32_t n_tiles, void* out, int32_t* k_out);
 int dbfr_test_pack_f16_rows(const float* frag, const float* bias, int32_t n_tiles, void* out, int32_t* k_out, float* rinv_out, int32_t* depth_out);
+int dbfr_test_pack_w1_factored(const float* W1, int32_t per_row, void* w1a_out, int32_t* k1a_out, float* rinv_out, float* w1bt_out, float* w1ct_out,
+                               int32_t* depth_out);
 int dbfr_test_pack_f16_depth(const float* frag, const float* bias, int32_t n_tiles, int32_t* depth_out, int32_t* depth_ok_out);
 int dbfr_profile_enable(dbfr_model* m, int32_t on);
 int dbfr_profile_read(dbfr_model* m, double* conv_ms, int64_t* conv_launches, double* conv_flops,
```

After: 495.1 (median of 3 runs). Within noise of the previous version (+0.3%).
